# HKUST-Aerial-Robotics/MIND

Hardware: AMD Instinct MI355X
Metric: sim steps/sec (whole node) + scenario-tree nodes expanded/sec, AV2 demo scenes (higher is better)
Workload: dtype f32-class (bf16 hi+mid+lo split operands = 24 significand bits, six products, fp32 accumulate) pair kernel + ActorNet, f32 elsewhere in the predictor, f64 iLQR

## Files before the change

include/mind_hip.h:

```cpp
#ifndef MIND_HIP_H
#define MIND_HIP_H

#include <stddef.h>
#include <stdint.h>

#ifdef __cplusplus
extern "C" {
#endif

#define MIND_OK 0
#define MIND_EINVAL (-1)
#define MIND_ENOMEM (-2)
#define MIND_EHIP (-3)
#define MIND_ESTATE (-4)
#define MIND_ENOTFOUND (-5)

typedef struct mind_ctx mind_ctx;

int mind_ctx_create(int device, void *stream, mind_ctx **out);
int mind_ctx_destroy(mind_ctx *ctx);
const char *mind_last_error_string(mind_ctx *ctx);
int mind_ctx_synchronize(mind_ctx *ctx);

typedef struct {
  const char *name;
  const float *data;
  int64_t numel;
} mind_tensor_desc;

int mind_weights_load(mind_ctx *ctx, const mind_tensor_desc *tensors, int n_tensors);

typedef struct {
  int n_scenes;
  const int32_t *actor_off;
  const int32_t *lane_off;
  const float *actors;
  const float *lanes;
  const float *lane_feat;
  const float *actor_ctrs;
  const float *actor_vecs;
  const float *lane_ctrs;
  const float *lane_vecs;
  const float *const *rpe;
  const float *tgt_nodes;
  const float *tgt_rpe;
} mind_scene_batch;

typedef struct {
  float *cls;
  float *reg;
  float *vel;
  float *lane_feat;
  float *actor_emb;
  float *cls_emb;
} mind_pred_out;

int mind_predict_batch(mind_ctx *ctx, const mind_scene_batch *in, mind_pred_out *out);

int mind_last_fusion_stats(mind_ctx *ctx, int *n_launches, float *total_ms, double *pairs_processed);
int mind_last_actor_stats(mind_ctx *ctx, int *layerwise, int *n_launches, int *n_chunks, float *total_ms);
int mind_last_token_stats(mind_ctx *ctx, int *layerwise, int *n_launches, int *n_chunks, float *total_ms);
int mind_last_token_stage_ms(mind_ctx *ctx, float *out_ms, int cap);
int mind_last_ilqr_stats(mind_ctx *ctx, float *kernel_ms, int *n_trees, int *workgroups_per_tree);
int mind_last_ilqr_profile(mind_ctx *ctx, double *out9);
int mind_last_ilqr_trace(mind_ctx *ctx, int tree, int phase, double *out, int cap_rows, int *n_rows);
int mind_set_profiling(mind_ctx *ctx, int enable);

#define MIND_PAIR_F32 0
#define MIND_PAIR_BF16X3 1
#define MIND_PAIR_BF16 2
#define MIND_PAIR_BF16X6 3
int mind_set_pair_precision(mind_ctx *ctx, int mode);

int mind_set_tuning(mind_ctx *ctx, const char *name, int value);
int mind_get_pair_precision(mind_ctx *ctx);
int mind_debug_pack_bfrag(const float *w, int row_stride, uint32_t *out);

int mind_debug_pair_schedule(const int *scene_tokens, const int *scene_actors, int n_scenes, int n_cu, int last_layer, int *out_jobs, int cap,
                             int *out_info);

int mind_debug_predict_choice(const char *const *knob_names, const int *knob_values, int n_knobs, int pair_prec, int n_cu, int have_side,
                              const int *scene_actors, const int *scene_lanes, int n_scenes, long long *out, int cap);

int mind_debug_ilqr_plan(const char *const *knob_names, const int *knob_values, int n_knobs, int n_cu, int mode, int n_trees, const int *n_nodes,
                         const int32_t *parents, long long *out, int cap, int *bad);

int mind_debug_aime_book(int pred_len, int max_depth, int max_rounds, int n_agents, int world, int rank, int force, int n_rounds, const int *dec_len,
                         const float *dec, int n_tokens, int bytes_per_pair, int plan_chunk_mb, int per_scene, long long *out, int cap, char *msg,
                         int msg_cap);

int mind_debug_actor_lw_plan(int n_actors, int np, int chunk, long long *out_launches, int cap, long long *out_info);

int mind_debug_token_lw_plan(int n_tokens, int mode, int chunk, long long *out_launches, int cap, long long *out_info);

int mind_debug_pack_conv_frag(const float *w, int co, int ci, int ksz, uint32_t *out, size_t cap);

int mind_debug_trig(mind_ctx *ctx, const double *x, int n, double *out);

int mind_debug_set_layers(mind_ctx *ctx, int n);
int64_t mind_debug_read(mind_ctx *ctx, const char *name, float *host, int64_t max_floats);

typedef struct {
  int n_nodes;
  const int32_t *parent;
  const float *prob;
  int n_agents;
  const float *agent_mean;
  const float *agent_cov;
  const double *field;
  const double *node_w;
} mind_cost_tree;

typedef struct {
  double dt, wheelbase;
  double w_des_state[6];
  double w_state_con[6];
  double state_lower[6], state_upper[6];
  double w_ctrl[2];
  double w_tgt, w_ego, w_ego_cov_offset, w_exo, w_exo_cov_offset, w_exo_cost_offset;
  double grid_res; int grid_w, grid_h;
  int max_iter;
} mind_ilqr_cfg;

typedef struct { int iterations; int converged; double J; double mu; } mind_ilqr_stats;

int mind_ilqr_solve_trees(mind_ctx *ctx, const mind_ilqr_cfg *cfg, const mind_cost_tree *trees,
                          int n_trees, const double *x0, const double *target_lane, int n_lane_pts,
                          double target_vel, int use_exo, const double *us_init, double *xs,
                          double *us, mind_ilqr_stats *stats);

int mind_ilqr_contingency(mind_ctx *ctx, const mind_ilqr_cfg *cfg_warm, const mind_ilqr_cfg *cfg_full,
                          const mind_cost_tree *trees, int n_trees, const double *x0,
                          const double *target_lane, int n_lane_pts, double target_vel, double *xs,
                          double *us, mind_ilqr_stats *stats_warm, mind_ilqr_stats *stats_full);
int mind_ilqr_contingency_begin(mind_ctx *ctx, const mind_ilqr_cfg *cfg_warm, const mind_ilqr_cfg *cfg_full,
                                const mind_cost_tree *trees, int n_trees, const double *x0,
                                const double *target_lane, int n_lane_pts, double target_vel, double *xs,
                                double *us, mind_ilqr_stats *stats_warm, mind_ilqr_stats *stats_full);
int mind_ilqr_contingency_begin_plan(mind_ctx *ctx, const mind_ilqr_cfg *cfg_warm, const mind_ilqr_cfg *cfg_full, const double *x0,
                                     const double *target_lane, int n_lane_pts, double target_vel, double *xs, double *us,
                                     mind_ilqr_stats *stats_warm, mind_ilqr_stats *stats_full);
int mind_ilqr_finish(mind_ctx *ctx);

typedef struct {
  int n_scenes;
  const int32_t *actor_off;
  const float *reg, *vel;
  const float *actor_ctrs, *actor_vecs;
  const float *rot, *orig;
  const float *cov_last;
  const int32_t *last;
  const float *target_lane;
  int n_lane_pts;
  const float *cls;
  const float *scen_prob;
  int lane_check;
  float dist_thres;
} mind_world_in;

typedef struct {
  float *world;
  float *topo;
  float *ego_end;
  float *sel, *sel_prob;
} mind_world_out;

int mind_aime_world(mind_ctx *ctx, const mind_world_in *in, const mind_world_out *out);

typedef struct {
  int n_scenes, n_agents, n_lanes;
  const float *pos, *ang, *vel;
  const float *types;
  const float *pad;
  const float *lane_ctrs, *lane_vecs;
  const float *target_lane;
  const float *target_lane_info;
  int n_lane_pts;
  float time_ahead, min_vel;
  const float *rows_dev;
  const int32_t *parent_slot;
  const int32_t *row0;
  const int32_t *dur;
  int prev_gen;
} mind_rebase_in;

typedef struct {
  float *actors;
  float *actor_ctrs, *actor_vecs;
  float *lane_ctrs, *lane_vecs;
  float *tgt_nodes, *tgt_rpe;
  float *frames;
  int32_t *gen;
} mind_rebase_out;

int mind_aime_rebase(mind_ctx *ctx, const mind_rebase_in *in, const mind_rebase_out *out);

typedef struct {
  int n_agents, n_lanes, n_lane_pts;
  const float *actors;
  const float *actor_ctrs, *actor_vecs;
  const float *lanes;
  const float *lane_ctrs, *lane_vecs;
  const float *tgt_nodes, *tgt_rpe;
  const float *rot, *orig, *tgt_pts;
  const float *hist;
  const float *types;
  const float *target_lane;
  const float *target_lane_info;
  float time_ahead, min_vel, dist_thres;
  int max_depth;
  int max_rounds;
  int pred_len;
  const float *raw_pos, *raw_ang, *raw_vel;
  const float *raw_pad;
  const double *lane_pts;
  const int32_t *lane_flags;
  float travel0;
  const float *script_cls, *script_reg, *script_vel;
  float prob_floor;
  const mind_ilqr_cfg *solve_cfg_warm, *solve_cfg_full;
  const double *solve_x0, *solve_lane;
  int solve_n_lane_pts;
  double solve_target_vel;
} mind_aime_plan_in;

#define MIND_AIME_BRANCH 1
#define MIND_AIME_END 2
#define MIND_AIME_TERMINATE 4
typedef struct {
  int round, scene, mode;
  int parent;
  float prob;
  int cur_t, end_t;
  int flags;
  int dur;
  int64_t row_off;
  float tgt_pts[22];
} mind_aime_node;

typedef struct {
  const mind_aime_node *nodes;
  int n_nodes;
  const float *rows;
  int64_t n_row_floats;
  int n_expanded, n_rounds;
  int root_flags;
  int round_scenes[32];
  float pair_ms;
  int pair_launches;
  int n_trees;
// ... 145 lines not shown
```

mind_amd/_lib.py:

```python
import ctypes as C
import os

_HERE = os.path.dirname(os.path.abspath(__file__))
LIB_PATH = os.environ.get("MIND_HIP_LIB", os.path.join(_HERE, "libmind_hip.so"))

MIND_OK = 0
MIND_EINVAL, MIND_ENOMEM, MIND_EHIP, MIND_ESTATE, MIND_ENOTFOUND = -1, -2, -3, -4, -5


class TensorDesc(C.Structure):
    _fields_ = [("name", C.c_char_p), ("data", C.POINTER(C.c_float)), ("numel", C.c_int64)]


class SceneBatch(C.Structure):
    _fields_ = [("n_scenes", C.c_int), ("actor_off", C.POINTER(C.c_int32)), ("lane_off", C.POINTER(C.c_int32)),
                ("actors", C.c_void_p), ("lanes", C.c_void_p), ("lane_feat", C.c_void_p),
                ("actor_ctrs", C.c_void_p), ("actor_vecs", C.c_void_p), ("lane_ctrs", C.c_void_p),
                ("lane_vecs", C.c_void_p), ("rpe", C.POINTER(C.c_void_p)), ("tgt_nodes", C.c_void_p),
                ("tgt_rpe", C.c_void_p)]


class PredOut(C.Structure):
    _fields_ = [("cls", C.c_void_p), ("reg", C.c_void_p), ("vel", C.c_void_p), ("lane_feat", C.c_void_p),
                ("actor_emb", C.c_void_p), ("cls_emb", C.c_void_p)]


class CostTree(C.Structure):
    _fields_ = [("n_nodes", C.c_int), ("parent", C.POINTER(C.c_int32)), ("prob", C.POINTER(C.c_float)),
                ("n_agents", C.c_int), ("agent_mean", C.POINTER(C.c_float)), ("agent_cov", C.POINTER(C.c_float)),
                ("field", C.POINTER(C.c_double)), ("node_w", C.POINTER(C.c_double))]


class FieldGrid(C.Structure):
    _fields_ = [("W", C.c_int), ("H", C.c_int), ("res", C.c_double), ("off_x", C.c_double), ("off_y", C.c_double),
                ("gx", C.POINTER(C.c_double)), ("gy", C.POINTER(C.c_double))]


class WorldIn(C.Structure):
    _fields_ = [("n_scenes", C.c_int), ("actor_off", C.POINTER(C.c_int32)), ("reg", C.c_void_p), ("vel", C.c_void_p),
                ("actor_ctrs", C.c_void_p), ("actor_vecs", C.c_void_p), ("rot", C.POINTER(C.c_float)),
                ("orig", C.POINTER(C.c_float)), ("cov_last", C.POINTER(C.c_float)), ("last", C.POINTER(C.c_int32)),
                ("target_lane", C.POINTER(C.c_float)), ("n_lane_pts", C.c_int), ("cls", C.c_void_p),
                ("scen_prob", C.POINTER(C.c_float)), ("lane_check", C.c_int), ("dist_thres", C.c_float)]


class WorldOut(C.Structure):
    _fields_ = [("world", C.c_void_p), ("topo", C.c_void_p), ("ego_end", C.c_void_p), ("sel", C.c_void_p), ("sel_prob", C.c_void_p)]


class RebaseIn(C.Structure):
    _fields_ = [("n_scenes", C.c_int), ("n_agents", C.c_int), ("n_lanes", C.c_int), ("pos", C.POINTER(C.c_float)),
                ("ang", C.POINTER(C.c_float)), ("vel", C.POINTER(C.c_float)), ("types", C.POINTER(C.c_float)),
                ("pad", C.POINTER(C.c_float)), ("lane_ctrs", C.POINTER(C.c_float)), ("lane_vecs", C.POINTER(C.c_float)),
                ("target_lane", C.POINTER(C.c_float)), ("target_lane_info", C.POINTER(C.c_float)), ("n_lane_pts", C.c_int),
                ("time_ahead", C.c_float), ("min_vel", C.c_float), ("rows_dev", C.c_void_p), ("parent_slot", C.POINTER(C.c_int32)),
                ("row0", C.POINTER(C.c_int32)), ("dur", C.POINTER(C.c_int32)), ("prev_gen", C.c_int)]


class RebaseOut(C.Structure):
    _fields_ = [("actors", C.c_void_p), ("actor_ctrs", C.c_void_p), ("actor_vecs", C.c_void_p), ("lane_ctrs", C.c_void_p),
                ("lane_vecs", C.c_void_p), ("tgt_nodes", C.c_void_p), ("tgt_rpe", C.c_void_p), ("frames", C.c_void_p),
                ("gen", C.POINTER(C.c_int32))]


class AimePlanIn(C.Structure):
    _fields_ = [("n_agents", C.c_int), ("n_lanes", C.c_int), ("n_lane_pts", C.c_int)] + \
               [(k, C.POINTER(C.c_float)) for k in ("actors", "actor_ctrs", "actor_vecs", "lanes", "lane_ctrs", "lane_vecs", "tgt_nodes", "tgt_rpe",
                                                    "rot", "orig", "tgt_pts", "hist", "types", "target_lane", "target_lane_info")] + \
               [("time_ahead", C.c_float), ("min_vel", C.c_float), ("dist_thres", C.c_float), ("max_depth", C.c_int), ("max_rounds", C.c_int), ("pred_len", C.c_int),
                ("raw_pos", C.POINTER(C.c_float)), ("raw_ang", C.POINTER(C.c_float)), ("raw_vel", C.POINTER(C.c_float)), ("raw_pad", C.POINTER(C.c_float)),
                ("lane_pts", C.POINTER(C.c_double)), ("lane_flags", C.POINTER(C.c_int32)), ("travel0", C.c_float),
                ("script_cls", C.c_void_p), ("script_reg", C.c_void_p), ("script_vel", C.c_void_p), ("prob_floor", C.c_float),
                ("solve_cfg_warm", C.c_void_p), ("solve_cfg_full", C.c_void_p), ("solve_x0", C.c_void_p), ("solve_lane", C.c_void_p),
                ("solve_n_lane_pts", C.c_int), ("solve_target_vel", C.c_double)]


class AimeNode(C.Structure):
    _fields_ = [("round", C.c_int), ("scene", C.c_int), ("mode", C.c_int), ("parent", C.c_int), ("prob", C.c_float),
                ("cur_t", C.c_int), ("end_t", C.c_int), ("flags", C.c_int), ("dur", C.c_int), ("row_off", C.c_int64),
                ("tgt_pts", C.c_float * 22)]


class AimePlanOut(C.Structure):
    _fields_ = [("nodes", C.POINTER(AimeNode)), ("n_nodes", C.c_int), ("rows", C.POINTER(C.c_float)), ("n_row_floats", C.c_int64),
                ("n_expanded", C.c_int), ("n_rounds", C.c_int), ("root_flags", C.c_int), ("round_scenes", C.c_int * 32),
                ("pair_ms", C.c_float), ("pair_launches", C.c_int), ("n_trees", C.c_int), ("tree_top", C.POINTER(C.c_int32)),
                ("tree_off", C.POINTER(C.c_int32)), ("flat_parent", C.POINTER(C.c_int32)), ("flat_prob", C.POINTER(C.c_float)),
                ("flat_mean", C.POINTER(C.c_float)), ("flat_cov", C.POINTER(C.c_float)), ("solves_begun", C.c_int)]


class IlqrCfg(C.Structure):
    _fields_ = [("dt", C.c_double), ("wheelbase", C.c_double), ("w_des_state", C.c_double * 6),
                ("w_state_con", C.c_double * 6), ("state_lower", C.c_double * 6), ("state_upper", C.c_double * 6),
                ("w_ctrl", C.c_double * 2), ("w_tgt", C.c_double), ("w_ego", C.c_double),
                ("w_ego_cov_offset", C.c_double), ("w_exo", C.c_double), ("w_exo_cov_offset", C.c_double),
                ("w_exo_cost_offset", C.c_double), ("grid_res", C.c_double), ("grid_w", C.c_int), ("grid_h", C.c_int),
                ("max_iter", C.c_int)]


class IlqrStats(C.Structure):
    _fields_ = [("iterations", C.c_int), ("converged", C.c_int), ("J", C.c_double), ("mu", C.c_double)]


LOOP_TAN_FN = C.CFUNCTYPE(C.c_double, C.c_double)
LOOP_SINCOS_FN = C.CFUNCTYPE(None, C.c_double, C.POINTER(C.c_double))


class LoopDesc(C.Structure):
    _fields_ = [("n_tracks", C.c_int), ("n_steps", C.c_int), ("clamp_last", C.c_int), ("ego_state", C.c_void_p), ("ego_state_is_f32", C.c_int), ("ego_obs", C.c_void_p), ("ego_trig32", C.c_void_p),
                ("tan_fn", C.c_void_p), ("sincos_fn", C.c_void_p), ("exo_obs", C.c_void_p),
                ("exo_valid", C.c_void_p), ("timestep", C.c_void_p), ("type_slot", C.c_void_p),
                ("sim_step", C.c_double), ("plan_step", C.c_double), ("enable_time", C.c_double),
                ("wheelbase", C.c_double), ("max_speed", C.c_double), ("max_steer", C.c_double), ("max_acc", C.c_double), ("max_dec", C.c_double),
                ("n_lanes", C.c_int), ("lane_pts", C.c_void_p), ("lane_flags", C.c_void_p),
                ("n_lane_pts", C.c_int), ("target_lane", C.c_void_p), ("target_lane_info", C.c_void_p),
                ("time_ahead", C.c_double), ("min_vel", C.c_float), ("dist_thres", C.c_float), ("max_depth", C.c_int), ("max_rounds", C.c_int),
                ("pred_len", C.c_int), ("prob_floor", C.c_float),
                ("cfg_warm", C.c_void_p), ("cfg_full", C.c_void_p), ("solve_n_lane_pts", C.c_int), ("solve_lane", C.c_void_p), ("target_vel", C.c_double),
                ("eval_n_lane_pts", C.c_int), ("eval_lane_is_f32", C.c_int), ("eval_lane", C.c_void_p), ("speculative", C.c_int)]


class LoopTotals(C.Structure):
    _fields_ = [("plans", C.c_longlong), ("expansions", C.c_longlong), ("scen_trees", C.c_longlong), ("rounds", C.c_longlong),
                ("aime_s", C.c_double), ("ilqr_s", C.c_double), ("total_s", C.c_double),
                ("iterations", C.c_longlong), ("node_iterations", C.c_longlong), ("node_iterations_exo", C.c_longlong),
                ("warm_speculated", C.c_longlong), ("warm_hits", C.c_longlong),
                ("pair_ms", C.c_double), ("pair_launches", C.c_longlong), ("scene_n2", C.c_double), ("scene_n_a1", C.c_double),
                ("ilqr_ms", C.c_double), ("ilqr_launches", C.c_longlong), ("ilqr_trees", C.c_longlong), ("ilqr_workgroups_per_tree", C.c_int),
                ("ilqr_prof", C.c_double * 9), ("ilqr_node_steps", C.c_double)]


class LoopOut(C.Structure):
    _fields_ = [("planned", C.c_int), ("enabled", C.c_int), ("n_steps", C.c_longlong), ("n_plans", C.c_longlong), ("episode_steps", C.c_longlong),
                ("sim_time", C.c_double), ("last_trigger", C.c_double), ("state", C.c_double * 4), ("ctrl", C.c_double * 2),
                ("n_agents", C.c_int), ("n_trees", C.c_int), ("best", C.c_int), ("n_expanded", C.c_int), ("n_rounds", C.c_int), ("n_traj_nodes", C.c_int),
                ("costs", C.POINTER(C.c_double)), ("aime_s", C.c_double), ("ilqr_s", C.c_double), ("total_s", C.c_double),
                ("tot", LoopTotals)]


PLANNER_EGO_KEY = -(1 << 63)


class PlannerDesc(C.Structure):
    _fields_ = [("time_ahead", C.c_double), ("min_vel", C.c_float), ("dist_thres", C.c_float), ("max_depth", C.c_int), ("max_rounds", C.c_int),
                ("pred_len", C.c_int), ("prob_floor", C.c_float), ("cfg_warm", C.c_void_p), ("cfg_full", C.c_void_p), ("speculative", C.c_int),
                ("ego_type_slot", C.c_int)]


class PlannerOut(C.Structure):
    _fields_ = [("n_plans", C.c_longlong),
                ("n_agents", C.c_int), ("n_trees", C.c_int), ("best", C.c_int), ("n_expanded", C.c_int), ("n_rounds", C.c_int), ("n_traj_nodes", C.c_int),
                ("costs", C.POINTER(C.c_double)), ("ctrl", C.c_double * 2), ("aime_s", C.c_double), ("ilqr_s", C.c_double), ("total_s", C.c_double),
                ("tot", LoopTotals)]


EXPORTS = ["mind_ctx_create", "mind_ctx_destroy", "mind_last_error_string", "mind_ctx_synchronize",
           "mind_weights_load", "mind_predict_batch", "mind_last_fusion_stats", "mind_last_actor_stats", "mind_debug_actor_lw_plan", "mind_last_token_stats", "mind_last_token_stage_ms", "mind_debug_token_lw_plan", "mind_set_profiling",
           "mind_ilqr_solve_trees", "mind_ilqr_contingency", "mind_ilqr_solve_fields", "mind_cost_eval", "mind_lane_dist_field", "mind_aime_world", "mind_aime_rebase", "mind_debug_set_layers",
           "mind_debug_read", "mind_set_pair_precision", "mind_get_pair_precision", "mind_debug_pack_bfrag", "mind_debug_pack_conv_frag", "mind_debug_pair_schedule", "mind_debug_predict_choice", "mind_debug_ilqr_plan", "mind_debug_aime_book", "mind_set_tuning", "mind_last_ilqr_stats", "mind_aime_plan", "mind_last_ilqr_profile", "mind_eval_traj_trees", "mind_last_ilqr_trace", "mind_ilqr_contingency_begin", "mind_ilqr_finish", "mind_fill_tracks", "mind_ilqr_contingency_begin_plan", "mind_debug_trig", "mind_aime_plan_begin", "mind_aime_plan_poll", "mind_aime_plan_finish", "mind_ctx_busy", "mind_ilqr_finish_plan",
           "mind_set_exchange", "mind_last_exchange_stats",
           "mind_loop_create", "mind_loop_destroy", "mind_loop_reset", "mind_loop_advance", "mind_loop_state", "mind_loop_last_plan", "mind_loop_export",
           "mind_planner_create", "mind_planner_destroy", "mind_planner_reset", "mind_planner_observe", "mind_planner_set_lanes", "mind_planner_set_target_lane",
           "mind_planner_set_solve_lane", "mind_planner_set_eval_lane", "mind_planner_plan", "mind_planner_last_plan", "mind_planner_export"]

EXCHANGE_FN = C.CFUNCTYPE(C.c_int, C.c_void_p, C.c_int, C.c_void_p, C.c_void_p, C.c_int64)
XCHG_ALLGATHER, XCHG_ALLREDUCE, XCHG_ALLTOALLV = 0, 1, 2

_lib = None


def load():
    global _lib
    if _lib is not None:
        return _lib
    if not os.path.exists(LIB_PATH):
        raise ImportError(f"{LIB_PATH} is missing: the HIP extension must be built (hipcc --offload-arch=gfx950); "
                          "there is no CPU fallback for the product path")
    lib = C.CDLL(LIB_PATH)
    lib.mind_ctx_create.argtypes = [C.c_int, C.c_void_p, C.POINTER(C.c_void_p)]
    lib.mind_ctx_destroy.argtypes = [C.c_void_p]
    lib.mind_last_error_string.argtypes = [C.c_void_p]
    lib.mind_last_error_string.restype = C.c_char_p
    lib.mind_ctx_synchronize.argtypes = [C.c_void_p]
    lib.mind_weights_load.argtypes = [C.c_void_p, C.POINTER(TensorDesc), C.c_int]
    lib.mind_predict_batch.argtypes = [C.c_void_p, C.POINTER(SceneBatch), C.POINTER(PredOut)]
    lib.mind_last_fusion_stats.argtypes = [C.c_void_p, C.POINTER(C.c_int), C.POINTER(C.c_float), C.POINTER(C.c_double)]
    lib.mind_last_actor_stats.argtypes = [C.c_void_p, C.POINTER(C.c_int), C.POINTER(C.c_int), C.POINTER(C.c_int), C.POINTER(C.c_float)]
    lib.mind_debug_actor_lw_plan.argtypes = [C.c_int, C.c_int, C.c_int, C.POINTER(C.c_longlong), C.c_int, C.POINTER(C.c_longlong)]
    lib.mind_last_token_stats.argtypes = [C.c_void_p, C.POINTER(C.c_int), C.POINTER(C.c_int), C.POINTER(C.c_int), C.POINTER(C.c_float)]
    lib.mind_last_token_stage_ms.argtypes = [C.c_void_p, C.POINTER(C.c_float), C.c_int]
    lib.mind_debug_token_lw_plan.argtypes = [C.c_int, C.c_int, C.c_int, C.POINTER(C.c_longlong), C.c_int, C.POINTER(C.c_longlong)]
    lib.mind_set_profiling.argtypes = [C.c_void_p, C.c_int]
    lib.mind_ilqr_solve_trees.argtypes = [C.c_void_p, C.POINTER(IlqrCfg), C.POINTER(CostTree), C.c_int,
                                          C.POINTER(C.c_double), C.POINTER(C.c_double), C.c_int, C.c_double, C.c_int,
                                          C.POINTER(C.c_double), C.POINTER(C.c_double), C.POINTER(C.c_double),
                                          C.POINTER(IlqrStats)]
    lib.mind_ilqr_contingency.argtypes = [C.c_void_p, C.POINTER(IlqrCfg), C.POINTER(IlqrCfg), C.POINTER(CostTree), C.c_int,
                                          C.POINTER(C.c_double), C.POINTER(C.c_double), C.c_int, C.c_double,
                                          C.POINTER(C.c_double), C.POINTER(C.c_double), C.POINTER(IlqrStats), C.POINTER(IlqrStats)]
    lib.mind_ilqr_contingency_begin.argtypes = [C.c_void_p, C.POINTER(IlqrCfg), C.POINTER(IlqrCfg), C.POINTER(CostTree), C.c_int,
                                          C.POINTER(C.c_double), C.POINTER(C.c_double), C.c_int, C.c_double,
                                          C.POINTER(C.c_double), C.POINTER(C.c_double), C.POINTER(IlqrStats), C.POINTER(IlqrStats)]
    lib.mind_ilqr_finish.argtypes = [C.c_void_p]
    lib.mind_ilqr_contingency_begin_plan.argtypes = [C.c_void_p, C.POINTER(IlqrCfg), C.POINTER(IlqrCfg), C.c_void_p, C.c_void_p, C.c_int, C.c_double,
                                                     C.c_void_p, C.c_void_p, C.c_void_p, C.c_void_p]
    lib.mind_fill_tracks.argtypes = [C.c_void_p, C.c_int, C.c_int, C.c_void_p, C.c_void_p, C.c_void_p, C.c_void_p, C.c_void_p, C.c_void_p]
    lib.mind_ilqr_solve_fields.argtypes = [C.c_void_p, C.POINTER(IlqrCfg), C.POINTER(FieldGrid), C.POINTER(CostTree), C.c_int,
                                           C.POINTER(C.c_double), C.POINTER(C.c_double), C.POINTER(C.c_double),
                                           C.POINTER(C.c_double), C.POINTER(IlqrStats)]
    lib.mind_cost_eval.argtypes = [C.c_void_p, C.POINTER(IlqrCfg), C.POINTER(FieldGrid), C.POINTER(CostTree),
                                   C.POINTER(C.c_double), C.POINTER(C.c_double), C.c_int, C.c_double, C.c_int, C.c_int,
                                   C.POINTER(C.c_int32), C.POINTER(C.c_double), C.POINTER(C.c_double), C.POINTER(C.c_double)]
    lib.mind_lane_dist_field.argtypes = [C.c_void_p, C.POINTER(C.c_double), C.POINTER(C.c_double), C.c_int, C.c_int, C.c_int,
                                         C.c_double] + [C.POINTER(C.c_double)] * 4
    lib.mind_aime_world.argtypes = [C.c_void_p, C.POINTER(WorldIn), C.POINTER(WorldOut)]
    lib.mind_aime_rebase.argtypes = [C.c_void_p, C.POINTER(RebaseIn), C.POINTER(RebaseOut)]
    lib.mind_aime_plan.argtypes = [C.c_void_p, C.POINTER(AimePlanIn), C.POINTER(AimePlanOut)]
    lib.mind_aime_plan_begin.argtypes = [C.c_void_p, C.POINTER(AimePlanIn)]
    lib.mind_aime_plan_poll.argtypes = [C.c_void_p]
    lib.mind_aime_plan_finish.argtypes = [C.c_void_p, C.POINTER(AimePlanOut)]
    lib.mind_ctx_busy.argtypes = [C.c_void_p]
    lib.mind_ilqr_finish_plan.argtypes = [C.c_void_p, C.c_int, C.c_int, C.c_void_p, C.c_void_p, C.c_void_p, C.c_void_p]
    lib.mind_set_pair_precision.argtypes = [C.c_void_p, C.c_int]
    lib.mind_set_tuning.argtypes = [C.c_void_p, C.c_char_p, C.c_int]
    lib.mind_last_ilqr_stats.argtypes = [C.c_void_p, C.POINTER(C.c_float), C.POINTER(C.c_int), C.POINTER(C.c_int)]
    lib.mind_last_ilqr_profile.argtypes = [C.c_void_p, C.POINTER(C.c_double)]
    lib.mind_last_ilqr_trace.argtypes = [C.c_void_p, C.c_int, C.c_int, C.POINTER(C.c_double), C.c_int, C.POINTER(C.c_int)]
    lib.mind_eval_traj_trees.argtypes = [C.POINTER(C.c_double), C.POINTER(C.c_double), C.POINTER(C.c_int32), C.c_int, C.c_void_p, C.c_int, C.c_int,
                                         C.c_double, C.POINTER(C.c_double)]
    lib.mind_get_pair_precision.argtypes = [C.c_void_p]
    lib.mind_debug_pack_bfrag.argtypes = [C.POINTER(C.c_float), C.c_int, C.POINTER(C.c_uint32)]
    lib.mind_debug_pair_schedule.argtypes = [C.POINTER(C.c_int), C.POINTER(C.c_int), C.c_int, C.c_int, C.c_int, C.POINTER(C.c_int), C.c_int, C.POINTER(C.c_int)]
    lib.mind_debug_predict_choice.argtypes = [C.POINTER(C.c_char_p), C.POINTER(C.c_int), C.c_int, C.c_int, C.c_int, C.c_int, C.POINTER(C.c_int), C.POINTER(C.c_int),
                                              C.c_int, C.POINTER(C.c_longlong), C.c_int]
    lib.mind_debug_ilqr_plan.argtypes = [C.POINTER(C.c_char_p), C.POINTER(C.c_int), C.c_int, C.c_int, C.c_int, C.c_int, C.POINTER(C.c_int), C.POINTER(C.c_int32),
                                         C.POINTER(C.c_longlong), C.c_int, C.POINTER(C.c_int)]
    lib.mind_debug_aime_book.argtypes = [C.c_int] * 8 + [C.POINTER(C.c_int), C.POINTER(C.c_float)] + [C.c_int] * 4 + [C.POINTER(C.c_longlong), C.c_int, C.c_char_p, C.c_int]
    lib.mind_debug_trig.argtypes = [C.c_void_p, C.POINTER(C.c_double), C.c_int, C.POINTER(C.c_double)]
    lib.mind_debug_pack_conv_frag.argtypes = [C.POINTER(C.c_float), C.c_int, C.c_int, C.c_int, C.POINTER(C.c_uint32), C.c_size_t]
    lib.mind_debug_set_layers.argtypes = [C.c_void_p, C.c_int]
    lib.mind_debug_read.argtypes = [C.c_void_p, C.c_char_p, C.POINTER(C.c_float), C.c_int64]
    lib.mind_set_exchange.argtypes = [C.c_void_p, C.c_int, C.c_int, EXCHANGE_FN, C.c_void_p, C.c_int]
    lib.mind_last_exchange_stats.argtypes = [C.c_void_p, C.POINTER(C.c_longlong), C.POINTER(C.c_longlong)]
    lib.mind_loop_create.argtypes = [C.c_void_p, C.POINTER(LoopDesc), C.POINTER(C.c_void_p)]
    lib.mind_loop_destroy.argtypes = [C.c_void_p]
    lib.mind_loop_reset.argtypes = [C.c_void_p]
    lib.mind_loop_advance.argtypes = [C.c_void_p, C.c_int, C.c_double, C.c_longlong, C.POINTER(LoopOut)]
    lib.mind_loop_state.argtypes = [C.c_void_p, C.POINTER(LoopOut)]
    lib.mind_loop_last_plan.argtypes = [C.c_void_p, C.POINTER(AimePlanOut)] + [C.POINTER(C.c_void_p)] * 6 + [C.c_void_p]
    lib.mind_loop_export.argtypes = [C.c_void_p, C.c_int, C.POINTER(C.c_int), C.c_void_p, C.c_void_p, C.c_void_p]
    lib.mind_planner_create.argtypes = [C.c_void_p, C.POINTER(PlannerDesc), C.POINTER(C.c_void_p)]
    lib.mind_planner_destroy.argtypes = [C.c_void_p]
    lib.mind_planner_reset.argtypes = [C.c_void_p]
    lib.mind_planner_observe.argtypes = [C.c_void_p, C.c_int, C.c_void_p, C.c_int, C.c_void_p, C.c_void_p, C.c_void_p]
    lib.mind_planner_set_lanes.argtypes = [C.c_void_p, C.c_int, C.c_void_p, C.c_void_p]
    lib.mind_planner_set_target_lane.argtypes = [C.c_void_p, C.c_int, C.c_void_p, C.c_void_p]
    lib.mind_planner_set_solve_lane.argtypes = [C.c_void_p, C.c_int, C.c_void_p, C.c_double]
    lib.mind_planner_set_eval_lane.argtypes = [C.c_void_p, C.c_int, C.c_void_p, C.c_int]
    lib.mind_planner_plan.argtypes = [C.c_void_p, C.c_void_p, C.c_void_p, C.POINTER(PlannerOut)]
    lib.mind_planner_last_plan.argtypes = [C.c_void_p, C.POINTER(AimePlanOut)] + [C.POINTER(C.c_void_p)] * 6 + [C.c_void_p]
    lib.mind_planner_export.argtypes = [C.c_void_p, C.c_int, C.POINTER(C.c_int), C.c_void_p, C.c_void_p, C.c_void_p]
    for n in EXPORTS:
        getattr(lib, n)
        if n not in ("mind_last_error_string", "mind_debug_read"):
            getattr(lib, n).restype = C.c_int
    lib.mind_debug_read.restype = C.c_int64
    _lib = lib
    return lib


PRED_CHOICE_FIELDS = ("header", "n_runs", "np", "actor_form", "actor_arg", "actor_grid", "actor_chunk", "actor_chunks", "actor_launches", "qsplit", "qk_stride",
                      "tiled", "edge_bf16", "edge_pair_bytes", "tok_chunk", "tok_lw", "tok_chunks", "pair_family", "pair_np", "l5_jobs5", "xcd_lanes",
                      "xcd_lanes5", "dec_actor", "dec_np", "fp32_dec", "split_dec", "want_mw", "mw_blocks", "cls_on_side", "tgt_wait_first")
PAIR_PREC = ("f32", "bf16x3", "bf16", "bf16x6")


def predict_choice(knobs, prec, scenes, n_cu=256, have_side=True):
    lib = load()
    names = (C.c_char_p * max(1, len(knobs)))(*[k.encode() for k in knobs])
    vals = (C.c_int * max(1, len(knobs)))(*[int(v) for v in knobs.values()])
    sa = (C.c_int * len(scenes))(*[a for a, _ in scenes])
    sl = (C.c_int * len(scenes))(*[l for _, l in scenes])
    cap = 32 + 6 * len(scenes)
    out = (C.c_longlong * cap)()
    n = lib.mind_debug_predict_choice(names, vals, len(knobs), PAIR_PREC.index(prec) if isinstance(prec, str) else prec, n_cu, int(have_side),
                                      sa, sl, len(scenes), out, cap)
    if n == MIND_EINVAL:
        return None
    assert 0 < n <= cap and out[0] == 32 and n == 32 + 6 * out[1], n
    d = dict(zip(PRED_CHOICE_FIELDS, out[:30]))
    d["runs"] = [tuple(out[32 + 6 * i:38 + 6 * i]) for i in range(out[1])]
    return d


ILQR_PLAN_FIELDS = ("header", "n_trees", "form", "G", "GS", "spec", "nslot", "grid", "workgroups_per_tree", "host_out", "early", "starve_followers")
ILQR_TREE_FIELDS = ("M", "nl", "nseg", "nsl", "maxls", "nfs")
ILQR_TREE_TABLES = ("level_start", "level_nodes", "child_start", "child_list", "seg_start", "seg_nodes", "slevel_start", "slevel_segs", "seg_rec",
                    "fstep_start", "fstep_items", "fstep_q1", "fstep_nstart", "fstep_nodes")


def ilqr_plan(knobs, parents, n_cu=256, generic=False, evaluate=False, two_fits=False):
    lib = load()
    names = (C.c_char_p * max(1, len(knobs)))(*[k.encode() for k in knobs])
    vals = (C.c_int * max(1, len(knobs)))(*[int(v) for v in knobs.values()])
    nn = (C.c_int * len(parents))(*[len(p) for p in parents])
    flat = [int(v) for p in parents for v in p]
    par = (C.c_int32 * max(1, len(flat)))(*flat)
    bad = (C.c_int * 2)()
    mode = int(generic) | int(evaluate) << 1 | int(two_fits) << 2
    n = lib.mind_debug_ilqr_plan(names, vals, len(knobs), n_cu, mode, len(parents), nn, par, None, 0, bad)
    if n == MIND_EINVAL:
        return {"bad": (bad[0], bad[1])} if bad[0] >= 0 else None
    out = (C.c_longlong * n)()
    assert lib.mind_debug_ilqr_plan(names, vals, len(knobs), n_cu, mode, len(parents), nn, par, out, n, bad) == n and out[0] == 16
    d = dict(zip(ILQR_PLAN_FIELDS, out[:12]))
    d["trees"], o = [], 16
    for _ in parents:
        tr = dict(zip(ILQR_TREE_FIELDS, out[o:o + 6]))
        lens, o = out[o + 6:o + 20], o + 20
        for name, ln in zip(ILQR_TREE_TABLES, lens):
            tr[name], o = list(out[o:o + ln]), o + ln
        d["trees"].append(tr)
    assert o == n
    return d


AIME_ROUND_FIELDS = ("B", "lo", "hi", "Bmax", "chunk", "S", "s0", "Sm", "any")
AIME_NODE_FIELDS = ("round", "scene", "mode", "parent", "prob", "cur_t", "end_t", "flags", "dur", "row_off", "owner", "lscene")


def aime_book(pred_len, max_depth, n_agents, rounds, world=1, rank=0, force=False, max_rounds=32, n_tokens=0, bytes_per_pair=512, plan_chunk_mb=96 * 1024,
              per_scene=1):
    import numpy as np
    lib = load()
    arrs = [np.ascontiguousarray(r, np.float32).ravel() for r in rounds]
    lens = (C.c_int * max(1, len(arrs)))(*[a.size for a in arrs])
    dec = np.concatenate(arrs + [np.zeros(1, np.float32)])
    msg = C.create_string_buffer(256)
    args = [pred_len, max_depth, max_rounds, n_agents, world, rank, int(force), len(arrs), lens, dec.ctypes.data_as(C.POINTER(C.c_float)), n_tokens,
            bytes_per_pair, plan_chunk_mb, per_scene]
    n = lib.mind_debug_aime_book(*args, None, 0, msg, 256)
    if n == MIND_EINVAL:
        return None
    out = (C.c_longlong * n)()
    assert lib.mind_debug_aime_book(*args, out, n, msg, 256) == n and out[0] == 16
    o, take = [16], lambda k: (list(out[o[0]:o[0] + k]), o.__setitem__(0, o[0] + k))[0]
    d = dict(code=out[1], error=msg.value.decode() if out[1] else None, args=(out[2], out[3]), n_rows=out[8], root_flags=out[9], rounds=[])
    for _ in range(out[4]):
        r = dict(zip(AIME_ROUND_FIELDS, take(9)))
        for k, ln in (("todo", r["S"]), ("cnt_r", world), ("s0_r", world + 1), ("win", 3 * r["Sm"]), ("tab", 2 * world), ("snd", 2 * world), ("rcv", 2 * world)):
            r[k] = take(ln)
        d["rounds"].append(r)
    if not out[1]:
        d["nodes"] = [dict(zip(AIME_NODE_FIELDS, take(12))) for _ in range(out[5])]
        for name in ("gather", "flat"):
            nj, nb, nbytes = take(3)
            d[name] = dict(jobs=[tuple(take(5)) for _ in range(nj)], job_of_block=take(nb), agent_of_block=take(nb), bytes=nbytes)
        d["tree_top"], d["tree_off"], d["flat_parent"], d["flat_prob"] = take(out[6]), take(out[6] + 1), take(out[7]), take(out[7])
    assert o[0] == n
    return d


class MindError(RuntimeError):
    pass


def check(lib, ctx, rc, what):
    if rc != MIND_OK:
        msg = lib.mind_last_error_string(ctx) if ctx else b""
        raise MindError(f"{what} failed with code {rc}: {msg.decode() if msg else ''}")
```

mind_amd/csrc/encdec_kernels.hip:

```cpp
#include <hip/hip_runtime.h>
#include <stdint.h>

typedef float f32x4 __attribute__((ext_vector_type(4)));

#define NT 256

__device__ __forceinline__ float wave_sum(float v) {
  v += __shfl_xor(v, 32, 64);
  v += __shfl_xor(v, 16, 64);
  v += __shfl_xor(v, 8, 64);
  v += __shfl_xor(v, 4, 64);
  v += __shfl_xor(v, 2, 64);
  v += __shfl_xor(v, 1, 64);
  return v;
}

__device__ __forceinline__ float block_sum(float v, float *red) {
  v = wave_sum(v);
  __syncthreads();
  if ((threadIdx.x & 63) == 0) red[threadIdx.x >> 6] = v;
  __syncthreads();
  return red[0] + red[1] + red[2] + red[3];
}

#ifndef DB
#define DB 16
#endif
#define DENSE_ROW_FENCE() __builtin_amdgcn_sched_barrier(0)
#define DBQ 8
template <int R>
__device__ __forceinline__ void dense_quads(const float *in, int ldi, int K, const float *__restrict__ WT,
                                            const float *__restrict__ b, int NOUT, float *out, int ldo,
                                            float *part, int part_floats) {
  const int nthr = blockDim.x;
  const int NQ = NOUT >> 2;
  int KP = 1;
  while (KP * 2 * NQ <= nthr && KP * 2 * R * NOUT <= part_floats && KP * 2 <= (K >> 2)) KP *= 2;
  const int Kc = ((K / 4 + KP - 1) / KP) * 4;
  for (int item = threadIdx.x; item < KP * NQ; item += nthr) {
    const int kp = item / NQ, o = (item % NQ) * 4;
    float acc[R][4];
#pragma unroll
    for (int r = 0; r < R; ++r)
#pragma unroll
      for (int c = 0; c < 4; ++c) acc[r][c] = (KP == 1 && b) ? b[o + c] : 0.f;
    const int k0 = kp * Kc, k1 = min(K, k0 + Kc);
    int k = k0;
    for (; k + DBQ <= k1; k += DBQ) {
      f32x4 w[DBQ];
#pragma unroll
      for (int q = 0; q < DBQ; ++q) w[q] = *(const f32x4 *)(WT + (size_t)(k + q) * NOUT + o);
#pragma unroll
      for (int r = 0; r < R; ++r) {
#pragma unroll
        for (int q4 = 0; q4 < DBQ / 4; ++q4) {
          const f32x4 x = *(const f32x4 *)(in + r * ldi + k + 4 * q4);
#pragma unroll
          for (int j = 0; j < 4; ++j)
#pragma unroll
            for (int c = 0; c < 4; ++c) acc[r][c] = fmaf(w[4 * q4 + j][c], x[j], acc[r][c]);
        }
        DENSE_ROW_FENCE();
      }
    }
    for (; k < k1; k += 4) {
#pragma unroll
      for (int j = 0; j < 4; ++j) {
        const f32x4 w = *(const f32x4 *)(WT + (size_t)(k + j) * NOUT + o);
#pragma unroll
        for (int r = 0; r < R; ++r) {
          const float x = in[r * ldi + k + j];
#pragma unroll
          for (int c = 0; c < 4; ++c) acc[r][c] = fmaf(w[c], x, acc[r][c]);
        }
      }
    }
#pragma unroll
    for (int r = 0; r < R; ++r)
#pragma unroll
      for (int c = 0; c < 4; ++c) {
        if (KP == 1) out[r * ldo + o + c] = acc[r][c];
        else part[(kp * R + r) * NOUT + o + c] = acc[r][c];
      }
  }
  if (KP == 1) return;
  __syncthreads();
  for (int i = threadIdx.x; i < R * NOUT; i += nthr) {
    const int r = i / NOUT, oo = i % NOUT;
    float v = b ? b[oo] : 0.f;
    for (int q = 0; q < KP; ++q) v += part[(q * R + r) * NOUT + oo];
    out[r * ldo + oo] = v;
  }
}

#ifndef DT
#define DT 1024
#endif
template <int R>
__device__ __forceinline__ void dense_quads_part(const float *in, int ldi, int K, const float *__restrict__ WT, const float *__restrict__ b, int NOUT,
                                                 float *out, int ldo, float *part, int part_floats, int wg, int G) {
  const int nthr = blockDim.x;
  const int NQ = NOUT >> 2;
  int KP = 1;
  while (KP * 2 * NQ <= DT && KP * 2 * R * NOUT <= part_floats && KP * 2 <= (K >> 2)) KP *= 2;
  const int Kc = ((K / 4 + KP - 1) / KP) * 4;
  const int q_lo = NQ * wg / G, q_hi = NQ * (wg + 1) / G, NQg = q_hi - q_lo;
  for (int item = threadIdx.x; item < KP * NQg; item += nthr) {
    const int kp = item / NQg, o = (q_lo + item % NQg) * 4;
    float acc[R][4];
#pragma unroll
    for (int r = 0; r < R; ++r)
#pragma unroll
      for (int c = 0; c < 4; ++c) acc[r][c] = (KP == 1 && b) ? b[o + c] : 0.f;
    const int k0 = kp * Kc, k1 = min(K, k0 + Kc);
    int k = k0;
    for (; k + DBQ <= k1; k += DBQ) {
      f32x4 w[DBQ];
#pragma unroll
      for (int q = 0; q < DBQ; ++q) w[q] = *(const f32x4 *)(WT + (size_t)(k + q) * NOUT + o);
#pragma unroll
      for (int r = 0; r < R; ++r) {
#pragma unroll
        for (int q4 = 0; q4 < DBQ / 4; ++q4) {
          const f32x4 x = *(const f32x4 *)(in + r * ldi + k + 4 * q4);
#pragma unroll
          for (int j = 0; j < 4; ++j)
#pragma unroll
            for (int c = 0; c < 4; ++c) acc[r][c] = fmaf(w[4 * q4 + j][c], x[j], acc[r][c]);
        }
        DENSE_ROW_FENCE();
      }
    }
    for (; k < k1; k += 4) {
#pragma unroll
      for (int j = 0; j < 4; ++j) {
        const f32x4 w = *(const f32x4 *)(WT + (size_t)(k + j) * NOUT + o);
#pragma unroll
        for (int r = 0; r < R; ++r) {
          const float x = in[r * ldi + k + j];
#pragma unroll
          for (int c = 0; c < 4; ++c) acc[r][c] = fmaf(w[c], x, acc[r][c]);
        }
      }
    }
#pragma unroll
    for (int r = 0; r < R; ++r)
#pragma unroll
      for (int c = 0; c < 4; ++c) {
        if (KP == 1) out[r * ldo + o + c] = acc[r][c];
        else part[(kp * R + r) * NOUT + o + c] = acc[r][c];
      }
  }
  if (KP == 1) return;
  __syncthreads();
  const int o_lo = q_lo * 4, no = NQg * 4;
  for (int i = threadIdx.x; i < R * no; i += nthr) {
    const int r = i / no, oo = o_lo + i % no;
    float v = b ? b[oo] : 0.f;
    for (int q = 0; q < KP; ++q) v += part[(q * R + r) * NOUT + oo];
    out[r * ldo + oo] = v;
  }
}

#define DEC_SYNC_SPINS (1u << 22)
__device__ __forceinline__ bool dec_grid_sync(unsigned *bar, int G, unsigned *abort_word) {
  __shared__ int sh_ab;
  __syncthreads();
  if (threadIdx.x == 0) {
// ... 558 lines not shown
  const int PF = DEC_SCENE_PART;
  const int tid = threadIdx.x;
  int xstage = 0;
  float *xb0 = xbuf, *xb1 = xbuf + 6 * 1536;
#ifdef MIND_DEC_TRACE
  if (blockIdx.x == 0 && tid == 0) dec_trn_ = 0;
#endif
  DEC_MARK();
  if (PART == 2) {
    for (int i = tid; i < 768; i += blockDim.x) C[i / 128][i % 128] = Cout[(size_t)b * 768 + i];
    __syncthreads();
  }
  if (PART != 2) {
  if (tid < 128) v0[0][tid] = x[(size_t)cls_row[b] * 128 + tid];
  __syncthreads();
  dense<1>(&v0[0][0], 256, 128, W.c0W, W.c0b, 384, &v1[0][0], 768, part, PF);
  DEC_MARK();
  __syncthreads();
  ln_rows(&v1[0][0], 768, 1, 384, W.c0g, W.c0be, true);
  DEC_MARK();
  __syncthreads();
  if (MW) {
    dense_quads_part<1>(&v1[0][0], 768, 384, W.c3W, W.c3b, 768, &ff[0][0], 1536, part, PF, wg, G);
    if (dec_exchange<1>(&ff[0][0], 1536, 768, wg, G, (xstage++ & 1) ? xb1 : xb0, bar, abort_word)) return;
  } else
    dense<1>(&v1[0][0], 768, 384, W.c3W, W.c3b, 768, &ff[0][0], 1536, part, PF);
  DEC_MARK();
  __syncthreads();
  ln_rows(&ff[0][0], 1536, 1, 768, W.c3g, W.c3be, true);
  DEC_MARK();
  __syncthreads();
  for (int i = tid; i < 768; i += blockDim.x) C[i / 128][i % 128] = ff[0][i];
  __syncthreads();
  for (int L = 0; L < 2; ++L) {
    dense<6>(&C[0][0], 128, 128, W.inW[L], W.inb[L], 384, &qkv[0][0], 384, part, PF);
  DEC_MARK();
    __syncthreads();
    if (tid < 4 * 36) {
      const int hd = tid / 36, s = (tid % 36) / 6, t = tid % 6;
      float d = 0.f;
      for (int k = 0; k < 32; ++k) d = fmaf(qkv[s][hd * 32 + k], qkv[t][128 + hd * 32 + k], d);
      sc[hd][s][t] = d / sqrtf(32.0f);
    }
    __syncthreads();
    if (tid < 24) {
      const int hd = tid / 6, s = tid % 6;
      float m = -INFINITY;
      for (int t = 0; t < 6; ++t) m = fmaxf(m, sc[hd][s][t]);
      float e[6], sum = 0.f;
      for (int t = 0; t < 6; ++t) { e[t] = expf(sc[hd][s][t] - m); sum += e[t]; }
      for (int t = 0; t < 6; ++t) sc[hd][s][t] = e[t] / sum;
    }
    __syncthreads();
    for (int i = tid; i < 6 * 128; i += blockDim.x) {
      const int s = i / 128, c = i % 128, hd = c / 32;
      float o = 0.f;
      for (int t = 0; t < 6; ++t) o = fmaf(sc[hd][s][t], qkv[t][256 + c], o);
      att[s][c] = o;
    }
    __syncthreads();
    dense<6>(&att[0][0], 128, 128, W.outW[L], W.outb[L], 128, &t2[0][0], 128, part, PF);
  DEC_MARK();
    __syncthreads();
    for (int i = tid; i < 768; i += blockDim.x) C[i / 128][i % 128] += t2[i / 128][i % 128];
    __syncthreads();
    ln_rows(&C[0][0], 128, 6, 128, W.n1g[L], W.n1b[L], false);
  DEC_MARK();
    __syncthreads();
    if (MW) {
      dense_quads_part<6>(&C[0][0], 128, 128, W.l1W[L], W.l1b[L], 1536, &ff[0][0], 1536, part, PF, wg, G);
      if (dec_exchange<6>(&ff[0][0], 1536, 1536, wg, G, (xstage++ & 1) ? xb1 : xb0, bar, abort_word)) return;
    } else
      dense<6>(&C[0][0], 128, 128, W.l1W[L], W.l1b[L], 1536, &ff[0][0], 1536, part, PF);
  DEC_MARK();
    __syncthreads();
    for (int i = tid; i < 6 * 1536; i += blockDim.x) ff[i / 1536][i % 1536] = fmaxf(ff[i / 1536][i % 1536], 0.f);
    __syncthreads();
    if (MW) {
      dense_quads_part<6>(&ff[0][0], 1536, 1536, W.l2W[L], W.l2b[L], 128, &t2[0][0], 128, part, PF, wg, G);
      if (dec_exchange<6>(&t2[0][0], 128, 128, wg, G, (xstage++ & 1) ? xb1 : xb0, bar, abort_word)) return;
    } else
      dense<6>(&ff[0][0], 1536, 1536, W.l2W[L], W.l2b[L], 128, &t2[0][0], 128, part, PF);
  DEC_MARK();
    __syncthreads();
    for (int i = tid; i < 768; i += blockDim.x) C[i / 128][i % 128] += t2[i / 128][i % 128];
    __syncthreads();
    ln_rows(&C[0][0], 128, 6, 128, W.n2g[L], W.n2b[L], false);
  DEC_MARK();
    __syncthreads();
  }
  if (!MW || wg == 0)
    for (int i = tid; i < 768; i += blockDim.x) Cout[(size_t)b * 768 + i] = C[i / 128][i % 128];
  }
  if (PART == 1) return;
  dense<6>(&C[0][0], 128, 128, W.k0W, W.k0b, 128, &att[0][0], 128, part, PF);
  DEC_MARK();
  __syncthreads();
  ln_rows(&att[0][0], 128, 6, 128, W.k0g, W.k0be, true);
  DEC_MARK();
  __syncthreads();
  dense<6>(&att[0][0], 128, 128, W.k3W, W.k3b, 128, &t2[0][0], 128, part, PF);
  DEC_MARK();
  __syncthreads();
  ln_rows(&t2[0][0], 128, 6, 128, W.k3g, W.k3be, true);
  DEC_MARK();
  __syncthreads();
  for (int k = tid >> 6; k < 6; k += (int)(blockDim.x >> 6)) {
    const int lane = tid & 63;
    float s = t2[k][lane] * W.k6W[lane] + t2[k][lane + 64] * W.k6W[lane + 64];
    s = wave_sum(s);
    if (lane == 0) sc[0][0][k] = s + W.k6b[0];
  }
  __syncthreads();
  if (tid == 0 && (!MW || wg == 0)) {
    float m = -INFINITY;
    for (int k = 0; k < 6; ++k) m = fmaxf(m, sc[0][0][k]);
    float e[6], sum = 0.f;
    for (int k = 0; k < 6; ++k) { e[k] = expf(sc[0][0][k] - m); sum += e[k]; }
    for (int k = 0; k < 6; ++k) cls_out[(size_t)b * 6 + k] = e[k] / sum;
  }
  DEC_MARK();
#ifdef MIND_DEC_TRACE
  if (blockIdx.x == 0 && tid == 0) {
    printf("[k_dec_scene] cycles between marks (dense / LayerNorm stages in program order):");
    for (int q = 1; q < dec_trn_ && q < 64; ++q) printf(" %lld", dec_tr_[q] - dec_tr_[q - 1]);
    printf("\n");
  }
#endif
}

__global__ __launch_bounds__(DT) void k_dec_scene(const float *__restrict__ x, const int *__restrict__ cls_row, float *__restrict__ Cout,
                                                  float *__restrict__ cls_out, DecW W) {
  k_dec_scene_body<false>(x, cls_row, Cout, cls_out, W, (int)blockIdx.x, 0, 1, nullptr, nullptr, nullptr);
}
__global__ __launch_bounds__(DT) void k_dec_scene_c(const float *__restrict__ x, const int *__restrict__ cls_row, float *__restrict__ Cout, DecW W) {
  k_dec_scene_body<false, 1>(x, cls_row, Cout, nullptr, W, (int)blockIdx.x, 0, 1, nullptr, nullptr, nullptr);
}
__global__ __launch_bounds__(DT) void k_dec_cls(float *__restrict__ Cout, float *__restrict__ cls_out, DecW W) {
  k_dec_scene_body<false, 2>(nullptr, nullptr, Cout, cls_out, W, (int)blockIdx.x, 0, 1, nullptr, nullptr, nullptr);
}
#define DEC_MW_G 8
__global__ __launch_bounds__(DT) void k_dec_scene_mw(const float *__restrict__ x, const int *__restrict__ cls_row, float *__restrict__ Cout,
                                                     float *__restrict__ cls_out, DecW W, int n_scenes, float *__restrict__ xbuf,
                                                     unsigned *__restrict__ bars, unsigned *abort_word) {
  const int r = (int)blockIdx.x % (8 * DEC_MW_G);
  const int b = 8 * ((int)blockIdx.x / (8 * DEC_MW_G)) + (r & 7), wg = r >> 3;
  if (b >= n_scenes) return;
  k_dec_scene_body<true>(x, cls_row, Cout, cls_out, W, b, wg, DEC_MW_G, xbuf + (size_t)b * 2 * 6 * 1536, bars + 4 * (size_t)b, abort_word);
}

#define RA 4
#define DEC_ACTOR_LDS_FLOATS (512 + 1536 + 3072 + 3072 + 3072 + 960 + 6144)
template <int PART>
__global__ __launch_bounds__(DT) void k_dec_actor(const float *__restrict__ x ,
                                                  const int *__restrict__ actor_row ,
                                                  const int *__restrict__ actor_scene , int n_actors,
                                                  const float *__restrict__ Cmode ,
                                                  const float *__restrict__ tgt ,
                                                  float *__restrict__ reg, float *__restrict__ vel, DecW W, float *__restrict__ h2g) {
  extern __shared__ __attribute__((aligned(16))) float dsm[];
  float (*xin)[128] = (float (*)[128])(dsm);
  float (*h1)[384] = (float (*)[384])(dsm + 512);
  float (*h2)[768] = (float (*)[768])(dsm + 2048);
  float (*E)[128] = (float (*)[128])(dsm + 5120);
  float (*t1)[128] = (float (*)[128])(dsm + 8192);
  float (*prm)[40] = (float (*)[40])(dsm + 11264);
  float *part = dsm + 12224;
  const int PF = 6144;
  const int tid = threadIdx.x;
  const int a0 = blockIdx.x * RA;
  if (PART != 2) {
    for (int i = tid; i < RA * 128; i += blockDim.x) {
      const int r = i / 128, a = a0 + r;
      xin[r][i % 128] = a < n_actors ? x[(size_t)actor_row[a] * 128 + i % 128] : 0.f;
    }
    __syncthreads();
    dense<RA>(&xin[0][0], 128, 128, W.a0W, W.a0b, 384, &h1[0][0], 384, part, PF);
    __syncthreads();
    ln_rows(&h1[0][0], 384, RA, 384, W.a0g, W.a0be, true);
    __syncthreads();
    dense<RA>(&h1[0][0], 384, 384, W.a3W, W.a3b, 768, &h2[0][0], 768, part, PF);
    __syncthreads();
    ln_rows(&h2[0][0], 768, RA, 768, W.a3g, W.a3be, true);
    __syncthreads();
    if (PART == 1) {
      for (int i = tid; i < RA * 768; i += blockDim.x) {
        const int r = i / 768, a = a0 + r;
        if (a < n_actors) h2g[(size_t)a * 768 + i % 768] = h2[r][i % 768];
      }
      return;
    }
  } else {
    for (int i = tid; i < RA * 768; i += blockDim.x) {
      const int r = i / 768, a = a0 + r;
      h2[r][i % 768] = a < n_actors ? h2g[(size_t)a * 768 + i % 768] : 0.f;
    }
    __syncthreads();
  }
  for (int i = tid; i < RA * 768; i += blockDim.x) {
    const int r = i / 768, k = (i % 768) / 128, c = i % 128;
    const int a = a0 + r;
    float v = 0.f;
    if (a < n_actors) {
      const int sc = actor_scene[a];
      v = h2[r][k * 128 + c] + Cmode[((size_t)sc * 6 + k) * 128 + c];
      if (k == 0) v += tgt[(size_t)sc * 128 + c];
    }
    E[r * 6 + k][c] = v;
  }
  __syncthreads();
  dense<RA * 6>(&E[0][0], 128, 128, W.r0W, W.r0b, 128, &t1[0][0], 128, part, PF);
  __syncthreads();
  ln_rows(&t1[0][0], 128, RA * 6, 128, W.r0g, W.r0be, true);
  __syncthreads();
  dense<RA * 6>(&t1[0][0], 128, 128, W.r3W, W.r3b, 128, &E[0][0], 128, part, PF);
  __syncthreads();
  ln_rows(&E[0][0], 128, RA * 6, 128, W.r3g, W.r3be, true);
  __syncthreads();
  for (int i = tid; i < RA * 6 * 40; i += blockDim.x) {
    const int r = i / 40, o = i % 40;
    float acc = W.r6b[o];
    for (int k = 0; k < 128; ++k) acc = fmaf(W.r6W[k * 40 + o], E[r][k], acc);
    prm[r][o] = acc;
  }
  __syncthreads();
  for (int i = tid; i < RA * 6 * 60; i += blockDim.x) {
    const int r = i / 60, t = i % 60;
    const int a = a0 + r / 6, k = r % 6;
    if (a >= n_actors) continue;
    float o5[5] = {0.f, 0.f, 0.f, 0.f, 0.f};
    for (int c = 0; c < 8; ++c) {
      const float tv = W.T[t * 8 + c];
#pragma unroll
      for (int d = 0; d < 5; ++d) o5[d] = fmaf(tv, prm[r][c * 5 + d], o5[d]);
    }
    float v2[2] = {0.f, 0.f};
    for (int c = 0; c < 7; ++c) {
      const float tv = W.Tp[t * 7 + c];
      v2[0] = fmaf(tv, prm[r][(c + 1) * 5 + 0] - prm[r][c * 5 + 0], v2[0]);
      v2[1] = fmaf(tv, prm[r][(c + 1) * 5 + 1] - prm[r][c * 5 + 1], v2[1]);
    }
    float *ro = reg + (((size_t)a * 6 + k) * 60 + t) * 5;
    ro[0] = o5[0]; ro[1] = o5[1]; ro[2] = expf(o5[2]); ro[3] = expf(o5[3]); ro[4] = expf(o5[4]);
    float *vo = vel + (((size_t)a * 6 + k) * 60 + t) * 2;
    vo[0] = v2[0] / 6.0f; vo[1] = v2[1] / 6.0f;
  }
}

extern "C" size_t mind_dec_scene_lds_bytes() { return (size_t)DEC_SCENE_LDS_FLOATS * sizeof(float); }
extern "C" size_t mind_dec_actor_lds_bytes() { return (size_t)DEC_ACTOR_LDS_FLOATS * sizeof(float); }
```

mind_amd/csrc/fusion_kernels.hip:

```cpp
#include <hip/hip_runtime.h>
#include <stdint.h>

typedef float f32x4 __attribute__((ext_vector_type(4)));
typedef float f32x16 __attribute__((ext_vector_type(16)));

typedef unsigned int u32;
typedef u32 u32x4 __attribute__((ext_vector_type(4)));
typedef __bf16 bf16x8 __attribute__((ext_vector_type(8)));
typedef __bf16 bf16x2_t __attribute__((ext_vector_type(2)));
typedef float f32x2_t __attribute__((ext_vector_type(2)));

__device__ __forceinline__ u32 pk_bf16(float a, float b) {
  f32x2_t v = {a, b};
  return __builtin_bit_cast(u32, __builtin_convertvector(v, bf16x2_t));
}
__device__ __forceinline__ float bf_lo_f32(u32 pk) { return __builtin_bit_cast(float, pk << 16); }
__device__ __forceinline__ float bf_hi_f32(u32 pk) { return __builtin_bit_cast(float, pk & 0xffff0000u); }

#define D_ 128
#define PART_STRIDE 1040

struct PairJob {
  long long edge_base;
  int N;
  int j;
  int t0, t1;
  int tok_base;
  int slot;
  int flags;
  int scene;
  long long edge_base_t;
};

#define VT_GM 0
#define VT_BM 128
#define VT_BP 256
#define VT_GP 384
#define VT_BEP 512
#define VT_GE 640
#define VT_BE 768
#define VT_SIZE 896

#define PAIR_WAVES 8
#define PAIR_THREADS (PAIR_WAVES * 64)
#define STAGE_FLOATS 512
#define LDS_WAE 0
#define LDS_WAP 16384
#define LDS_STAGE 32768
#define LDS_PTAB (LDS_STAGE + PAIR_WAVES * STAGE_FLOATS)
#define LDS_SVEC (LDS_PTAB + PAIR_WAVES * 128)
#define LDS_VT (LDS_SVEC + PAIR_WAVES * 136)
#define LDS_RT (LDS_VT + VT_SIZE)
#define LDS_TOTAL (LDS_RT + 1024)

#define LDS_FENCE() asm volatile("s_waitcnt lgkmcnt(0)" ::: "memory")
#define SCHED_FENCE() __builtin_amdgcn_sched_barrier(0)
#define OPAQUE(x) asm volatile("" : "+v"(x))

typedef f32x4 frag8[8];

__device__ __forceinline__ float red_quad(float v) {
  v += __shfl_xor(v, 16, 64);
  v += __shfl_xor(v, 32, 64);
  return v;
}
__device__ __forceinline__ float red_max16(float v) {
  v = fmaxf(v, __shfl_xor(v, 8, 64));
  v = fmaxf(v, __shfl_xor(v, 4, 64));
  v = fmaxf(v, __shfl_xor(v, 2, 64));
  v = fmaxf(v, __shfl_xor(v, 1, 64));
  return v;
}
__device__ __forceinline__ float red_sum16(float v) {
  v += __shfl_xor(v, 8, 64);
  v += __shfl_xor(v, 4, 64);
  v += __shfl_xor(v, 2, 64);
  v += __shfl_xor(v, 1, 64);
  return v;
}

__device__ __forceinline__ void ln_pairs(frag8 &a, const float *vtq, int off_g, int off_b, bool relu) {
  float s = 0.f;
#pragma unroll
  for (int b = 0; b < 8; ++b)
#pragma unroll
    for (int w = 0; w < 4; ++w) s += a[b][w];
  s = red_quad(s);
  const float mean = s * (1.0f / 128.0f);
  float v = 0.f;
#pragma unroll
  for (int b = 0; b < 8; ++b)
#pragma unroll
    for (int w = 0; w < 4; ++w) {
      const float d = a[b][w] - mean;
      v = fmaf(d, d, v);
    }
  v = red_quad(v);
  const float rstd = 1.0f / sqrtf(v * (1.0f / 128.0f) + 1e-5f);
#pragma unroll
  for (int b = 0; b < 8; ++b) {
    const f32x4 gm = *(const f32x4 *)(vtq + off_g + 16 * b);
    const f32x4 bt = *(const f32x4 *)(vtq + off_b + 16 * b);
#pragma unroll
    for (int w = 0; w < 4; ++w) {
      float y = (a[b][w] - mean) * rstd * gm[w] + bt[w];
      if (relu) y = fmaxf(y, 0.f);
      a[b][w] = y;
    }
    if (b & 1) SCHED_FENCE();
  }
}

__device__ __forceinline__ void gemm128(frag8 &acc, const float *wa, const frag8 &bsrc, int lane) {
  int lo = lane * 4;
  OPAQUE(lo);
  const float *wl = wa + lo;
  f32x4 c0 = *(const f32x4 *)(wl + (0 * 8 + 0) * 256);
  f32x4 c1 = *(const f32x4 *)(wl + (1 * 8 + 0) * 256);
#pragma unroll
  for (int st = 0; st < 32; ++st) {
    const int s4 = st >> 2, ob = (st & 3) * 2;
    f32x4 n0 = c0, n1 = c1;
    if (st < 31) {
      const int s4n = (st + 1) >> 2, obn = ((st + 1) & 3) * 2;
      n0 = *(const f32x4 *)(wl + (obn * 8 + s4n) * 256);
      n1 = *(const f32x4 *)(wl + ((obn + 1) * 8 + s4n) * 256);
    }
#pragma unroll
    for (int w = 0; w < 4; ++w) {
      const float bv = bsrc[s4][w];
      acc[ob] = __builtin_amdgcn_mfma_f32_16x16x4f32(c0[w], bv, acc[ob], 0, 0, 0);
      acc[ob + 1] = __builtin_amdgcn_mfma_f32_16x16x4f32(c1[w], bv, acc[ob + 1], 0, 0, 0);
    }
    c0 = n0; c1 = n1;
    SCHED_FENCE();
  }
}

__device__ __forceinline__ int sw_pos(int r, int c) { return (r * 8 + (c ^ ((r >> 1) & 7))) * 4; }

#ifdef MIND_PAIR_TRACE
#define PT_DECL long long pt_[12] = {0, 0, 0, 0, 0, 0, 0, 0, 0, 0, 0, 0}; long long pt_t = clock64();
#define PT_DRAIN() asm volatile("s_waitcnt vmcnt(0)" ::: "memory")
#define PT(i) do { long long n_ = clock64(); pt_[i] += n_ - pt_t; pt_t = n_; } while (0)
#else
#define PT_DECL
#define PT_DRAIN()
#define PT(i)
#endif

template <int MODE>
__global__ __launch_bounds__(PAIR_THREADS, 1) void k_pair(const PairJob *__restrict__ jobs, int n_jobs,
                                                 float *__restrict__ edge, const float *__restrict__ ST,
                                                 const float *__restrict__ QK, float *__restrict__ part,
// ... 262 lines not shown
        LDS_FENCE();
        const bool mine = (ll >> 5) == (qt & 1);
        const int fq = ll & 31;
#pragma unroll
        for (int t = 0; t < 16; ++t) {
          float val = stage[sw_pos(t, fq >> 2) + (fq & 3)];
          val = mine ? val : 0.f;
          const f32x4 pa = *(const f32x4 *)(ptab + t * 8);
          const f32x4 pb = *(const f32x4 *)(ptab + t * 8 + 4);
#pragma unroll
          for (int k = 0; k < 4; ++k) {
            mbar[hf][k] = fmaf(pa[k], val, mbar[hf][k]);
            mbar[hf][k + 4] = fmaf(pb[k], val, mbar[hf][k + 4]);
          }
          if ((t & 3) == 3) SCHED_FENCE();
        }
        LDS_FENCE();
      }

      PT(7);
    }

    float *po = part + (size_t)J.slot * PART_STRIDE;
#pragma unroll
    for (int r = 0; r < 4; ++r) {
      const float l = red_sum16(l_part[r]);
      if (p == 0 && q < 2) { po[4 * q + r] = m_run[r]; po[8 + 4 * q + r] = l; }
    }
#pragma unroll
    for (int hf = 0; hf < 2; ++hf)
#pragma unroll
      for (int hd = 0; hd < 8; ++hd) po[16 + hd * 128 + hf * 64 + lane] = mbar[hf][hd];
  }
#ifdef MIND_PAIR_TRACE
  if (blockIdx.x == 0 && tid == 0)
    printf("[k_pair<%d> um=%d] cycles: load %lld gemm1 %lld T+LN1 %lld scores %lld softmax %lld mbar %lld gemm2 %lld LN23+store %lld\n", MODE,
           update_mode, pt_[0], pt_[1], pt_[2], pt_[3], pt_[4], pt_[5], pt_[6], pt_[7]);
#endif
}

template __global__ void k_pair<0>(const PairJob *, int, float *, const float *, const float *, float *,
                                   const float *, const float *, const float *, const float *,
                                   const float *, const float *const *, int);
template __global__ void k_pair<1>(const PairJob *, int, float *, const float *, const float *, float *,
                                   const float *, const float *, const float *, const float *,
                                   const float *, const float *const *, int);

extern "C" size_t mind_pair_lds_bytes() { return (size_t)LDS_TOTAL * sizeof(float); }

#define TOK_TPW_BIG 8
#define TOK_TPW_SMALL 4

struct TokMeta {
  int type;
  int src;
  int slot0;
  int nsplit;
  int flags;
  int pad0, pad1, pad2;
};

struct TokWeights {
  const float *WvT, *bv, *WoT, *bo, *g2, *b2, *W1T, *b1, *W2T, *bb2, *g3, *b3;
  const float *WsT, *WtT, *bm, *WqT, *bq, *Wk;
  const float *WpaT, *bpa, *gpa, *bepa, *WplT, *bpl, *gpl, *bepl;
};

#define TKG 4
#define TT_THREADS (TKG * 128)

template <int K, int TP>
__device__ __forceinline__ void matvec_part(float (&acc)[TP], const float *__restrict__ WT, int ldo, int col,
                                            const float *xin, int ldx, int kg) {
  constexpr int KQ = K / TKG;
  const int k0 = kg * KQ;
  float w[KQ];
#pragma unroll
  for (int k = 0; k < KQ; ++k) w[k] = WT[(size_t)(k0 + k) * ldo + col];
#pragma unroll
  for (int t = 0; t < TP; ++t) acc[t] = 0.f;
#pragma unroll
  for (int k = 0; k < KQ; k += 4)
#pragma unroll
    for (int t = 0; t < TP; ++t) {
      const float4 xv = *reinterpret_cast<const float4 *>(xin + t * ldx + k0 + k);
      acc[t] = fmaf(w[k], xv.x, acc[t]);
      acc[t] = fmaf(w[k + 1], xv.y, acc[t]);
      acc[t] = fmaf(w[k + 2], xv.z, acc[t]);
      acc[t] = fmaf(w[k + 3], xv.w, acc[t]);
    }
}

template <int K>
__device__ __forceinline__ void mv_load(float (&w)[K / TKG], const float *__restrict__ WT, int ldo, int col, int kg) {
  constexpr int KQ = K / TKG;
  const int k0 = kg * KQ;
#pragma unroll
  for (int k = 0; k < KQ; ++k) w[k] = WT[(size_t)(k0 + k) * ldo + col];
}
template <int K, int TP>
__device__ __forceinline__ void mv_fma(float (&acc)[TP], const float (&w)[K / TKG], const float *xin, int ldx, int kg) {
  constexpr int KQ = K / TKG;
  const int k0 = kg * KQ;
#pragma unroll
  for (int t = 0; t < TP; ++t) acc[t] = 0.f;
#pragma unroll
  for (int k = 0; k < KQ; k += 4)
#pragma unroll
    for (int t = 0; t < TP; ++t) {
      const float4 xv = *reinterpret_cast<const float4 *>(xin + t * ldx + k0 + k);
      acc[t] = fmaf(w[k], xv.x, acc[t]);
      acc[t] = fmaf(w[k + 1], xv.y, acc[t]);
      acc[t] = fmaf(w[k + 2], xv.z, acc[t]);
      acc[t] = fmaf(w[k + 3], xv.w, acc[t]);
    }
}
template <int TP, int N>
__device__ __forceinline__ void ksum_n(const float (&acc)[N][TP], const float (&bias)[N], float *rk, int kg, int col, float (&r0)[N], float (&r1)[N]) {
  constexpr int TPW = TP, ST = TKG * TP * 128;
  __syncthreads();
#pragma unroll
  for (int n = 0; n < N; ++n)
#pragma unroll
    for (int t = 0; t < TPW; ++t) rk[n * ST + (kg * TPW + t) * 128 + col] = acc[n][t];
  __syncthreads();
  const int t0 = (TP / TKG) * kg;
#pragma unroll
  for (int n = 0; n < N; ++n) {
    const float *q = rk + n * ST;
    r0[n] = ((q[(0 * TPW + t0) * 128 + col] + q[(1 * TPW + t0) * 128 + col]) + (q[(2 * TPW + t0) * 128 + col] + q[(3 * TPW + t0) * 128 + col])) + bias[n];
    r1[n] = 0.f;
    if (TP / TKG == 2)
      r1[n] = ((q[(0 * TPW + t0 + 1) * 128 + col] + q[(1 * TPW + t0 + 1) * 128 + col]) + (q[(2 * TPW + t0 + 1) * 128 + col] + q[(3 * TPW + t0 + 1) * 128 + col])) + bias[n];
  }
}

template <int TP>
__device__ __forceinline__ void ksum(const float (&acc)[TP], float bias, float *rk, int kg, int col, float &r0, float &r1) {
  constexpr int TPW = TP;
  __syncthreads();
#pragma unroll
  for (int t = 0; t < TPW; ++t) rk[(kg * TPW + t) * 128 + col] = acc[t];
  __syncthreads();
  const int t0 = (TP / TKG) * kg;
  r0 = ((rk[(0 * TPW + t0) * 128 + col] + rk[(1 * TPW + t0) * 128 + col]) +
        (rk[(2 * TPW + t0) * 128 + col] + rk[(3 * TPW + t0) * 128 + col])) + bias;
  r1 = 0.f;
  if (TP / TKG == 2)
    r1 = ((rk[(0 * TPW + t0 + 1) * 128 + col] + rk[(1 * TPW + t0 + 1) * 128 + col]) +
          (rk[(2 * TPW + t0 + 1) * 128 + col] + rk[(3 * TPW + t0 + 1) * 128 + col])) + bias;
}

__device__ __forceinline__ void gsum2(float &a, float &b, float *rd, int kg, int tid) {
#pragma unroll
  for (int o = 32; o > 0; o >>= 1) { a += __shfl_xor(a, o, 64); b += __shfl_xor(b, o, 64); }
  const int wv = (tid >> 6) & 1;
  __syncthreads();
  if ((tid & 63) == 0) { rd[(kg * 2 + wv) * 2] = a; rd[(kg * 2 + wv) * 2 + 1] = b; }
  __syncthreads();
  a = rd[(kg * 2) * 2] + rd[(kg * 2 + 1) * 2];
  b = rd[(kg * 2) * 2 + 1] + rd[(kg * 2 + 1) * 2 + 1];
}

__device__ __forceinline__ void ln2tok(float &p0, float &p1, float g, float be, float *rd, int kg, int tid) {
  float s0 = p0, s1 = p1;
  gsum2(s0, s1, rd, kg, tid);
  const float d0 = p0 - s0 * (1.0f / 128.0f), d1 = p1 - s1 * (1.0f / 128.0f);
  s0 = d0 * d0; s1 = d1 * d1;
  gsum2(s0, s1, rd, kg, tid);
  p0 = d0 * (1.0f / sqrtf(s0 * (1.0f / 128.0f) + 1e-5f)) * g + be;
  p1 = d1 * (1.0f / sqrtf(s1 * (1.0f / 128.0f) + 1e-5f)) * g + be;
}

template <int TPW, bool MG>
__device__ __forceinline__ void k_token_body(const TokMeta *__restrict__ meta, int n_tok, int mode,
                                             const float *__restrict__ actor_feat,
                                             const float *__restrict__ lane_feat, float *__restrict__ x,
                                             const float *__restrict__ part, float *__restrict__ ST,
                                             float *__restrict__ QK, const TokWeights &W) {
  __shared__ __attribute__((aligned(16))) float xs[TPW][132];
  __shared__ __attribute__((aligned(16))) float tmp[TPW][260];
  __shared__ __attribute__((aligned(16))) float mb[TPW][8][132];
  __shared__ float rk[(MG ? 3 : 1) * TKG * TPW * 128];
  __shared__ float rd[TKG * 2 * 2];
  __shared__ float cw[TPW][8][8];
  const int tid = threadIdx.x, kg = tid >> 7, col = tid & 127;
  const int tok0 = blockIdx.x * TPW;
  const int nt = min(TPW, n_tok - tok0);
  constexpr bool TWO = TPW / TKG == 2;
  const int ta = (TPW / TKG) * kg, tb = TWO ? ta + 1 : ta;
  const bool va = ta < nt, vb = TWO && tb < nt;
#ifdef MIND_TOKEN_TRACE
  long long tt_[10] = {0, 0, 0, 0, 0, 0, 0, 0, 0, 0}, tq_ = clock64();
#define TT(i) do { const long long n_ = clock64(); tt_[i] += n_ - tq_; tq_ = n_; } while (0)
#else
#define TT(i) do {} while (0)
#endif

  if (mode & 1) {
    int tya = 2, tyb = 2;
    float fa = 0.f, fb = 0.f;
    if (va) {
      const TokMeta m = meta[tok0 + ta];
      tya = m.type;
      if (m.type == 0) fa = actor_feat[(size_t)m.src * 128 + col];
      else if (m.type == 1) fa = lane_feat[(size_t)m.src * 128 + col];
    }
    if (vb) {
      const TokMeta m = meta[tok0 + tb];
      tyb = m.type;
      if (m.type == 0) fb = actor_feat[(size_t)m.src * 128 + col];
      else if (m.type == 1) fb = lane_feat[(size_t)m.src * 128 + col];
    }
    tmp[ta][col] = fa; if (TWO) tmp[tb][col] = fb;
    __syncthreads();
    float acc[TPW], a0, a1, l0, l1;
    matvec_part<128, TPW>(acc, W.WpaT, 128, col, &tmp[0][0], 260, kg);
    ksum<TPW>(acc, W.bpa[col], rk, kg, col, a0, a1);
    matvec_part<128, TPW>(acc, W.WplT, 128, col, &tmp[0][0], 260, kg);
    ksum<TPW>(acc, W.bpl[col], rk, kg, col, l0, l1);
    float p0 = tya == 0 ? a0 : l0, p1 = tyb == 0 ? a1 : l1;
    {
      float s0 = p0, s1 = p1;
      gsum2(s0, s1, rd, kg, tid);
      const float d0 = p0 - s0 * (1.0f / 128.0f), d1 = p1 - s1 * (1.0f / 128.0f);
      s0 = d0 * d0; s1 = d1 * d1;
      gsum2(s0, s1, rd, kg, tid);
      const float ga = W.gpa[col], gl = W.gpl[col], ba = W.bepa[col], bl = W.bepl[col];
      p0 = fmaxf(d0 * (1.0f / sqrtf(s0 * (1.0f / 128.0f) + 1e-5f)) * (tya == 0 ? ga : gl) + (tya == 0 ? ba : bl), 0.f);
      p1 = fmaxf(d1 * (1.0f / sqrtf(s1 * (1.0f / 128.0f) + 1e-5f)) * (tyb == 0 ? ga : gl) + (tyb == 0 ? ba : bl), 0.f);
      if (tya == 2) p0 = 0.f;
      if (tyb == 2) p1 = 0.f;
    }
    xs[ta][col] = p0; if (TWO) xs[tb][col] = p1;
    __syncthreads();
  } else {
    xs[ta][col] = va ? x[(size_t)(tok0 + ta) * 128 + col] : 0.f;
    if (TWO) xs[tb][col] = vb ? x[(size_t)(tok0 + tb) * 128 + col] : 0.f;
    __syncthreads();
  }
  TT(0);
  if (mode & 2) {
    if (tid < TPW * 8) {
      const int t = tid >> 3, hd = tid & 7;
      float wgt[8];
#pragma unroll
      for (int s = 0; s < 8; ++s) wgt[s] = 0.f;
      if (t < nt) {
        const TokMeta m = meta[tok0 + t];
        if (!((mode & 8) && !(m.flags & 1))) {
          float M = -INFINITY;
          for (int s = 0; s < m.nsplit; ++s) M = fmaxf(M, part[(size_t)(m.slot0 + s) * PART_STRIDE + hd]);
          float L = 0.f;
          for (int s = 0; s < m.nsplit; ++s) {
            const float *ps = part + (size_t)(m.slot0 + s) * PART_STRIDE;
            const float e = expf(ps[hd] - M);
            wgt[s] = e;
            L += e * ps[8 + hd];
          }
          const float inv = 1.0f / L;
          for (int s = 0; s < m.nsplit; ++s) wgt[s] *= inv;
        }
      }
#pragma unroll
      for (int s = 0; s < 8; ++s) cw[t][hd][s] = wgt[s];
    }
    __syncthreads();
    TT(1);
#pragma unroll
    for (int q = 0; q < TPW / TKG; ++q) {
      const int t = ta + q;
      int ns = 0, slot0 = 0;
      if (t < nt) {
        const TokMeta m = meta[tok0 + t];
        ns = ((mode & 8) && !(m.flags & 1)) ? 0 : m.nsplit;
        slot0 = m.slot0;
      }
      float v[8];
#pragma unroll
      for (int hd = 0; hd < 8; ++hd) v[hd] = 0.f;
      int s = 0;
      for (; s + 2 <= ns; s += 2) {
        const float *ps = part + (size_t)(slot0 + s) * PART_STRIDE + 16 + col;
        float pv[8], pw[8];
#pragma unroll
        for (int hd = 0; hd < 8; ++hd) { pv[hd] = ps[hd * 128]; pw[hd] = ps[PART_STRIDE + hd * 128]; }
#pragma unroll
        for (int hd = 0; hd < 8; ++hd) v[hd] = fmaf(cw[t][hd][s], pv[hd], v[hd]);
#pragma unroll
        for (int hd = 0; hd < 8; ++hd) v[hd] = fmaf(cw[t][hd][s + 1], pw[hd], v[hd]);
      }
      if (s < ns) {
        const float *ps = part + (size_t)(slot0 + s) * PART_STRIDE + 16 + col;
        float pv[8];
#pragma unroll
        for (int hd = 0; hd < 8; ++hd) pv[hd] = ps[hd * 128];
#pragma unroll
        for (int hd = 0; hd < 8; ++hd) v[hd] = fmaf(cw[t][hd][s], pv[hd], v[hd]);
      }
#pragma unroll
      for (int hd = 0; hd < 8; ++hd) mb[t][hd][col] = v[hd];
    }
    __syncthreads();
    TT(2);
    {
      float acc[TPW], o0, o1;
      matvec_part<128, TPW>(acc, W.WvT, 128, col, &mb[0][col >> 4][0], 8 * 132, kg);
      ksum<TPW>(acc, W.bv[col], rk, kg, col, o0, o1);
// ... 141 lines not shown
```

mind_amd/csrc/mind_hip.hip:

```cpp
#include <hip/hip_runtime.h>

#include <cmath>
#include <cstdarg>
#include <cstdio>
#include <cstdlib>
#include <algorithm>
#include <cstring>
#include <map>
#include <string>
#include <thread>
#include <atomic>
#include <functional>
#include <vector>

#include "../../include/mind_hip.h"
#include "encdec_kernels.hip"
#include "fusion_kernels.hip"
#include "pair_bf16_kernels.hip"
#include "pair_tile_kernels.hip"
#include "pair_tile6_kernels.hip"
#include "token_mfma_kernels.hip"
#include "actor_mfma_kernels.hip"
#include "actor_lw_kernels.hip"
#include "token_lw_kernels.hip"
// ... 121 lines not shown
  std::atomic<int> pa_state{0};
  mind_aime_plan_in pa_in;
  mind_aime_plan_out pa_out;
  int pa_rc = 0;
  struct Plan {
    AimeBook book;
    int agents = 0;
    long long gen = 0;
    const float *rows_p = nullptr, *fmean_p = nullptr, *fcov_p = nullptr;
    const float *dev_fmean = nullptr, *dev_fcov = nullptr;
  } plan;
  DevBuf pl_flat;
  DevBuf dec_xbuf, dec_bars;
  unsigned *dec_abort = nullptr;
  int rb_cur = 0, rb_gen = 0;
  size_t rb_S = 0, rb_a = 0;
  bool profiling = false;
  hipEvent_t ev_il0 = nullptr, ev_il1 = nullptr;
  float ilqr_ms = 0.f;
  int ilqr_multi = 0, ilqr_trees = 0;
  std::function<int()> il_finish;
  bool il_finish_owned = false;
  hipEvent_t ev_rows = nullptr;
  std::vector<const double *> il_trace_dev;
  std::vector<int> il_trace_its;
  int il_trace_cap = 0, il_trace_phases = 0;
  double il_prof[9] = {0, 0, 0, 0, 0, 0, 0, 0, 0};
  long long n_ilqr_fallbacks = 0;
  int n_pair_launch = 0;
  float pair_ms = 0.f;
  double pairs_done = 0.0;
  std::vector<hipEvent_t> ev;
  bool ev_defer = false;
  std::vector<hipEvent_t> ev_pool;
  size_t ev_pool_used = 0;
  std::vector<size_t> ev_pending;
  int n_cu = 256;
  int debug_layers = 6;
  int last_ntok = 0;
  size_t il_dbg[6] = {0, 0, 0, 0, 0, 0};
  long long last_edge_pairs = 0;
  int last_slots = 0, last_A = 0, last_B = 0;
};

static int fail(mind_ctx *c, int code, const char *fmt, ...) {
  char buf[512];
  va_list ap;
  va_start(ap, fmt);
  vsnprintf(buf, sizeof(buf), fmt, ap);
  va_end(ap);
  if (c) c->err = buf;
  return code;
}

#define HIPCHK(c, call)                                                                        \
  do {                                                                                         \
    hipError_t e_ = (call);                                                                    \
    if (e_ != hipSuccess)                                                                      \
      return fail(c, MIND_EHIP, "%s failed: %s (%s:%d)", #call, hipGetErrorString(e_), __FILE__, __LINE__); \
  } while (0)

static int ensure(mind_ctx *c, DevBuf &b, size_t bytes) {
  if (bytes <= b.cap) return MIND_OK;
  if (b.p) (void)hipFree(b.p);
  b.p = nullptr;
  b.cap = 0;
  size_t want = bytes < ((size_t)64 << 20) ? std::max<size_t>(2 * bytes, (size_t)1 << 20) : bytes + bytes / 4 + 4096;
  hipError_t e = hipMalloc(&b.p, want);
  if (e != hipSuccess) {
    e = hipMalloc(&b.p, bytes);
    want = bytes;
    if (e != hipSuccess) return fail(c, MIND_ENOMEM, "hipMalloc(%zu) failed: %s", bytes, hipGetErrorString(e));
  }
  b.cap = want;
  return MIND_OK;
}

static int ensure_exact(mind_ctx *c, DevBuf &b, size_t bytes, const char *what) {
  if (bytes <= b.cap) return MIND_OK;
  HIPCHK(c, hipStreamSynchronize(c->stream));
  if (b.p) (void)hipFree(b.p);
  b.p = nullptr;
  b.cap = 0;
  if (hipMalloc(&b.p, bytes) != hipSuccess) return fail(c, MIND_ENOMEM, "hipMalloc(%zu) for %s failed", bytes, what);
  b.cap = bytes;
  return MIND_OK;
}

extern "C" int mind_ctx_create(int device, void *stream, mind_ctx **out) {
  if (!out) return MIND_EINVAL;
  *out = nullptr;
  int n = 0;
  if (hipGetDeviceCount(&n) != hipSuccess || n <= 0) return MIND_EHIP;
  if (device < 0 || device >= n) return MIND_EINVAL;
  mind_ctx *c = new mind_ctx();
  c->device = device;
  if (hipSetDevice(device) != hipSuccess) { delete c; return MIND_EHIP; }
  c->stream = (hipStream_t)stream;
  if (hipStreamCreateWithFlags(&c->side, hipStreamNonBlocking) != hipSuccess) c->side = nullptr;
  if (c->side && hipEventCreateWithFlags(&c->ev_side, hipEventDisableTiming) != hipSuccess) { (void)hipStreamDestroy(c->side); c->side = nullptr; }
  if (c->side && hipEventCreateWithFlags(&c->ev_main, hipEventDisableTiming) != hipSuccess) { (void)hipStreamDestroy(c->side); c->side = nullptr; }
  if (c->side && hipEventCreateWithFlags(&c->ev_tgt, hipEventDisableTiming) != hipSuccess) { (void)hipStreamDestroy(c->side); c->side = nullptr; }
  if (hipEventCreateWithFlags(&c->ev_stage, hipEventDisableTiming) != hipSuccess) { *out = nullptr; delete c; return MIND_EHIP; }
  hipDeviceProp_t prop;
  if (hipGetDeviceProperties(&prop, device) == hipSuccess) c->n_cu = prop.multiProcessorCount;
  (void)hipFuncSetAttribute((const void *)k_pair<0>, hipFuncAttributeMaxDynamicSharedMemorySize, (int)mind_pair_lds_bytes());
  (void)hipFuncSetAttribute((const void *)k_pair<1>, hipFuncAttributeMaxDynamicSharedMemorySize, (int)mind_pair_lds_bytes());
  (void)hipFuncSetAttribute((const void *)k_pair_bf<0, 3>, hipFuncAttributeMaxDynamicSharedMemorySize, (int)mind_pair_bf_lds_bytes());
  (void)hipFuncSetAttribute((const void *)k_pair_bf<1, 3>, hipFuncAttributeMaxDynamicSharedMemorySize, (int)mind_pair_bf_lds_bytes());
  (void)hipFuncSetAttribute((const void *)k_pair_bf<0, 1>, hipFuncAttributeMaxDynamicSharedMemorySize, (int)mind_pair_bf_lds_bytes());
  (void)hipFuncSetAttribute((const void *)k_pair_bf<1, 1>, hipFuncAttributeMaxDynamicSharedMemorySize, (int)mind_pair_bf_lds_bytes());
  (void)hipFuncSetAttribute((const void *)k_pair_t<0, 3>, hipFuncAttributeMaxDynamicSharedMemorySize, (int)mind_pair_bf_lds_bytes());
  (void)hipFuncSetAttribute((const void *)k_pair_t<1, 3>, hipFuncAttributeMaxDynamicSharedMemorySize, (int)mind_pair_bf_lds_bytes());
  (void)hipFuncSetAttribute((const void *)k_pair_t<0, 1>, hipFuncAttributeMaxDynamicSharedMemorySize, (int)mind_pair_bf_lds_bytes());
  (void)hipFuncSetAttribute((const void *)k_pair_t<1, 1>, hipFuncAttributeMaxDynamicSharedMemorySize, (int)mind_pair_bf_lds_bytes());
  (void)hipFuncSetAttribute((const void *)k_pair_t6<0>, hipFuncAttributeMaxDynamicSharedMemorySize, (int)mind_pair_bf_lds_bytes());
  (void)hipFuncSetAttribute((const void *)k_pair_t6<1>, hipFuncAttributeMaxDynamicSharedMemorySize, (int)mind_pair_bf_lds_bytes());
  if (const char *te = getenv("MIND_PAIR_TILE")) c->pt.pair_tile = !(te[0] == '0');
  if (const char *xe = getenv("MIND_XCD_ORDER")) c->pt.xcd_order = !(xe[0] == '0');

  if (const char *pe = getenv("MIND_PAIR_PREC")) {
    const std::string v = pe;
    if (v == "f32" || v == "0") c->pair_prec = 0;
    else if (v == "bf16x3" || v == "1") c->pair_prec = 1;
    else if (v == "bf16" || v == "2") c->pair_prec = 2;
    else if (v == "bf16x6" || v == "3") c->pair_prec = 3;
  }
  (void)hipFuncSetAttribute((const void *)k_actor_net, hipFuncAttributeMaxDynamicSharedMemorySize, (int)mind_actor_lds_bytes());
  (void)hipFuncSetAttribute((const void *)k_actor_mfma<3>, hipFuncAttributeMaxDynamicSharedMemorySize, (int)mind_actor_mfma_lds_bytes());
  (void)hipFuncSetAttribute((const void *)k_actor_mfma<6>, hipFuncAttributeMaxDynamicSharedMemorySize, (int)mind_actor_mfma_lds_bytes());
  (void)hipFuncSetAttribute((const void *)k_dec_actor_mfma<1>, hipFuncAttributeMaxDynamicSharedMemorySize, (int)mind_dec_actor_mfma_lds_bytes());
  (void)hipFuncSetAttribute((const void *)k_dec_actor_mfma<3>, hipFuncAttributeMaxDynamicSharedMemorySize, (int)mind_dec_actor_mfma_lds_bytes());
  (void)hipFuncSetAttribute((const void *)k_dec_actor_mfma<6>, hipFuncAttributeMaxDynamicSharedMemorySize, (int)mind_dec_actor_mfma_lds_bytes());
  if (const char *se = getenv("MIND_ACTOR_SPLIT")) c->pt.actor_np = atoi(se) == 3 ? 3 : 6;
  (void)hipFuncSetAttribute((const void *)k_actor_mfma<1>, hipFuncAttributeMaxDynamicSharedMemorySize, (int)mind_actor_mfma_lds_bytes());
  if (const char *me = getenv("MIND_ENC_MFMA")) c->pt.enc_mfma = !(me[0] == '0');
  if (const char *me = getenv("MIND_ACTOR_F32")) c->pt.actor_f32 = !(me[0] == '0');
  if (const char *me = getenv("MIND_ACTOR_F32_MIN")) c->pt.actor_f32_min = atoi(me);
  if (const char *me = getenv("MIND_ACTOR_LW_MIN")) c->pt.actor_lw_min = atoi(me);
  lw_set_attributes();
  (void)hipFuncSetAttribute((const void *)k_actor_f32<1>, hipFuncAttributeMaxDynamicSharedMemorySize, (int)mind_actor_f32_lds_bytes(1));
  (void)hipFuncSetAttribute((const void *)k_actor_f32<2>, hipFuncAttributeMaxDynamicSharedMemorySize, (int)mind_actor_f32_lds_bytes(2));
  if (const char *de = getenv("MIND_DEC_MFMA_MIN")) c->pt.dec_mfma_min = atoi(de);
  if (const char *oe = getenv("MIND_DEC_OVERLAP")) c->pt.dec_overlap = !(oe[0] == '0');
  (void)hipFuncSetAttribute((const void *)k_ilqr<true, 0>, hipFuncAttributeMaxDynamicSharedMemorySize, (int)il_lds_bytes(0));
  (void)hipFuncSetAttribute((const void *)k_ilqr<false, 1>, hipFuncAttributeMaxDynamicSharedMemorySize, (int)il_lds_bytes(0));
  (void)hipFuncSetAttribute((const void *)k_ilqr<false, 0>, hipFuncAttributeMaxDynamicSharedMemorySize, (int)il_lds_bytes(0));
  (void)hipFuncSetAttribute((const void *)k_ilqr<false, 2>, hipFuncAttributeMaxDynamicSharedMemorySize, (int)il_lds_bytes(0));
  if (const char *te = getenv("MIND_TOK_MFMA")) c->pt.tok_mfma = !(te[0] == '0');
  if (const char *te = getenv("MIND_TOK_SMALL_MAX")) c->pt.tok_small_max = atoi(te);
  if (const char *te = getenv("MIND_TOK_MERGE")) c->pt.tok_merge = !(te[0] == '0');
  if (const char *te = getenv("MIND_DEC_MW")) c->pt.dec_mw = !(te[0] == '0');
  if (const char *te = getenv("MIND_DEC_CLS_SIDE")) c->pt.dec_cls_side = !(te[0] == '0');
  if (const char *te = getenv("MIND_TOK_BF_MIN_N")) c->pt.tok_bf_min_n = atoi(te);
  if (const char *te = getenv("MIND_TOK_LW_MIN_N")) c->pt.tok_lw_min_n = atoi(te);
  if (const char *te = getenv("MIND_TOK_LW_MIN")) c->pt.tok_lw_min = atoi(te);
  if (const char *te = getenv("MIND_TGT_SIDE")) c->pt.tgt_side = !(te[0] == '0');
  if (const char *te = getenv("MIND_PL_TAB_SIDE")) c->pl_tab_side = !(te[0] == '0');
  (void)hipFuncSetAttribute((const void *)k_token_mfma<0>, hipFuncAttributeMaxDynamicSharedMemorySize, (int)mind_token_mfma_lds_bytes());
  (void)hipFuncSetAttribute((const void *)k_token_mfma<1>, hipFuncAttributeMaxDynamicSharedMemorySize, (int)mind_token_mfma_lds_bytes());
  if (const char *ce = getenv("MIND_PLAN_CHUNK_MB")) { const long v = atol(ce); if (v > 0) c->plan_chunk_mb = v; }
  if (const char *we = getenv("MIND_TAB_SMALL")) c->tab_small = atoi(we) != 0;
  if (const char *we = getenv("MIND_TAB_HOST_MAX")) c->tab_host_max = std::max(0, atoi(we));
  if (const char *we = getenv("MIND_EARLY_EVAL")) c->early_eval = atoi(we) != 0;
  if (const char *we = getenv("MIND_GLUE_FUSED")) c->glue_fused = atoi(we) != 0;
  if (const char *we = getenv("MIND_DEC_MIRROR")) c->dec_mirror = atoi(we) != 0;
  if (const char *we = getenv("MIND_UPLOAD_KERNEL_MAX")) c->upload_kernel_max = std::max(0, atoi(we));
  const char *const il_env[][2] = {{"MIND_ILQR_CHUNK", "ilqr_chunk"}, {"MIND_ILQR_WGS", "ilqr_wgs"}, {"MIND_ILQR_SPEC_DERIV", "ilqr_spec_deriv"},
                                   {"MIND_ILQR_HOST_OUT_MAX", "ilqr_host_out_max"}, {"MIND_ILQR_SLOTS", "ilqr_slots"}};
  for (const auto &e : il_env)
    if (const char *we = getenv(e[0])) (void)ilqr_tuning_set(c->it, e[1], atoi(we));
  (void)hipFuncSetAttribute((const void *)k_dec_scene, hipFuncAttributeMaxDynamicSharedMemorySize, (int)mind_dec_scene_lds_bytes());
  (void)hipFuncSetAttribute((const void *)k_dec_scene_mw, hipFuncAttributeMaxDynamicSharedMemorySize, (int)mind_dec_scene_lds_bytes());
  (void)hipFuncSetAttribute((const void *)k_dec_scene_c, hipFuncAttributeMaxDynamicSharedMemorySize, (int)mind_dec_scene_lds_bytes());
  (void)hipFuncSetAttribute((const void *)k_dec_cls, hipFuncAttributeMaxDynamicSharedMemorySize, (int)mind_dec_scene_lds_bytes());
  (void)hipFuncSetAttribute((const void *)k_dec_tgt, hipFuncAttributeMaxDynamicSharedMemorySize, (int)mind_dec_scene_lds_bytes());
  (void)hipFuncSetAttribute((const void *)k_dec_actor<0>, hipFuncAttributeMaxDynamicSharedMemorySize, (int)mind_dec_actor_lds_bytes());
  (void)hipFuncSetAttribute((const void *)k_dec_actor<1>, hipFuncAttributeMaxDynamicSharedMemorySize, (int)mind_dec_actor_lds_bytes());
  (void)hipFuncSetAttribute((const void *)k_dec_actor<2>, hipFuncAttributeMaxDynamicSharedMemorySize, (int)mind_dec_actor_lds_bytes());
  *out = c;
  return MIND_OK;
}

extern "C" int mind_ctx_destroy(mind_ctx *c) {
  if (!c) return MIND_EINVAL;
  if (c->pa_thread.joinable()) c->pa_thread.join();
  (void)hipSetDevice(c->device);
  (void)hipStreamSynchronize(c->stream);
  DevBuf *bufs[] = {&c->edge, &c->x, &c->ST, &c->QK, &c->part, &c->tokpos, &c->meta, &c->jobs, &c->actor_feat,
                    &c->lane_feat, &c->tgt_feat, &c->cmode, &c->tgt_emb, &c->rows, &c->rpe_ptrs, &c->ilqr_dev, &c->aime_dev, &c->rebase_dev2[0], &c->rebase_dev2[1], &c->dec_h2};
  for (DevBuf *b : bufs)
    if (b->p) (void)hipFree(b->p);
  for (TableSet &t : c->tabs)
    for (DevBuf *b : {&t.meta, &t.jobs, &t.jobs5, &t.rows})
      if (b->p) (void)hipFree(b->p);
  if (c->wdev) (void)hipFree(c->wdev);
  for (DevBuf *b : {&c->dec_xbuf, &c->dec_bars})
    if (b->p) (void)hipFree(b->p);
  if (c->dec_abort) (void)hipHostFree(c->dec_abort);
  for (DevBuf *b : {&c->pl_root, &c->pl_in[0], &c->pl_in[1], &c->pl_lf, &c->pl_lrep, &c->pl_pred, &c->pl_small, &c->pl_tab[0], &c->pl_tab[1], &c->pl_win[0],
                    &c->pl_win[1], &c->pl_flat, &c->x_send, &c->x_recv, &c->x_seg})
    if (b->p) (void)hipFree(b->p);
  for (DevBuf &b : c->pl_world)
    if (b.p) (void)hipFree(b.p);
  for (void *q : c->pl_pin)
    if (q) (void)hipHostFree(q);
  if (c->ev_pl) (void)hipEventDestroy(c->ev_pl);
  if (c->ev_root) (void)hipEventDestroy(c->ev_root);
  if (c->ev_field) (void)hipEventDestroy(c->ev_field);
  if (c->il_field.p) (void)hipFree(c->il_field.p);
  if (c->il_field_pin) (void)hipHostFree(c->il_field_pin);
  if (c->ev_tab) (void)hipEventDestroy(c->ev_tab);
  if (c->ev_rows) (void)hipEventDestroy(c->ev_rows);
  if (c->pl_copy) (void)hipStreamDestroy(c->pl_copy);
  for (hipEvent_t e : c->ev) (void)hipEventDestroy(e);
  for (hipEvent_t e : c->ev_pool) (void)hipEventDestroy(e);
  if (c->ev_side) (void)hipEventDestroy(c->ev_side);
  if (c->ev_main) (void)hipEventDestroy(c->ev_main);
  if (c->ev_tgt) (void)hipEventDestroy(c->ev_tgt);
  if (c->ev_stage) (void)hipEventDestroy(c->ev_stage);
  if (c->ev_cls) (void)hipEventDestroy(c->ev_cls);
  if (c->actor_lw_arena.p) (void)hipFree(c->actor_lw_arena.p);
  if (c->tok_lw_arena.p) (void)hipFree(c->tok_lw_arena.p);
  for (hipEvent_t e : c->ev_tok) (void)hipEventDestroy(e);
  if (c->ev_act0) (void)hipEventDestroy(c->ev_act0);
  if (c->ev_act1) (void)hipEventDestroy(c->ev_act1);
  if (c->ev_il0) (void)hipEventDestroy(c->ev_il0);
  if (c->ev_il1) (void)hipEventDestroy(c->ev_il1);
  if (c->side) { (void)hipStreamSynchronize(c->side); (void)hipStreamDestroy(c->side); }
  if (c->own_stream) (void)hipStreamDestroy(c->stream);
  delete c;
  return MIND_OK;
}

extern "C" const char *mind_last_error_string(mind_ctx *c) { return c ? c->err.c_str() : "null context"; }

extern "C" int mind_ctx_synchronize(mind_ctx *c) {
  if (!c) return MIND_EINVAL;
  HIPCHK(c, hipStreamSynchronize(c->stream));
  return MIND_OK;
}

extern "C" int mind_set_tuning(mind_ctx *c, const char *name, int value) {
  if (!c || !name) return MIND_EINVAL;
  const std::string n = name;
  if (pred_tuning_set(c->pt, name, value)) return MIND_OK;
  if (ilqr_tuning_set(c->it, name, value)) return MIND_OK;
  if (n == "plan_chunk_mb") c->plan_chunk_mb = value < 1 ? 1 : value;
  else if (n == "pl_tab_side") c->pl_tab_side = value != 0;
  else if (n == "tab_small") c->tab_small = value != 0;
  else if (n == "tab_host_max") c->tab_host_max = value < 0 ? 0 : value;
  else if (n == "early_eval") c->early_eval = value != 0;
  else if (n == "glue_fused") c->glue_fused = value != 0;
  else if (n == "dec_mirror") c->dec_mirror = value != 0;
  else if (n == "upload_kernel_max") c->upload_kernel_max = value < 0 ? 0 : value;
  else return fail(c, MIND_EINVAL, "mind_set_tuning: unknown knob '%s'", name);
  return MIND_OK;
}

extern "C" int mind_set_exchange(mind_ctx *c, int rank, int world, mind_exchange_fn fn, void *user, int force) {
  if (!c) return MIND_EINVAL;
  if (fn && (world < 1 || rank < 0 || rank >= world)) return fail(c, MIND_EINVAL, "mind_set_exchange: rank %d of %d", rank, world);
  c->xfn = fn; c->xuser = user;
  c->xr = fn ? rank : 0; c->xw = fn ? world : 1; c->xforce = fn && force != 0;
  return MIND_OK;
}

extern "C" int mind_last_exchange_stats(mind_ctx *c, long long *collectives, long long *bytes) {
  if (!c) return MIND_EINVAL;
  if (collectives) *collectives = c->x_collectives;
  if (bytes) *bytes = c->x_bytes;
  return MIND_OK;
}

extern "C" int mind_set_pair_precision(mind_ctx *c, int mode) {
  if (!c || mode < 0 || mode > 3) return MIND_EINVAL;
  c->pair_prec = mode;
  return MIND_OK;
}

extern "C" int mind_get_pair_precision(mind_ctx *c) { return c ? c->pair_prec : MIND_EINVAL; }

namespace { std::vector<float> pack_bfrag(const std::vector<float> &w, int row_stride); }
extern "C" int mind_debug_pack_bfrag(const float *w, int row_stride, uint32_t *out) {
  if (!w || !out || row_stride < 128) return MIND_EINVAL;
  std::vector<float> v(w, w + (size_t)127 * row_stride + 128);
  v.resize((size_t)128 * row_stride, 0.f);
  const std::vector<float> t = pack_bfrag(v, row_stride);
  memcpy(out, t.data(), 16384 * sizeof(uint32_t));
  return MIND_OK;
}

extern "C" int mind_set_profiling(mind_ctx *c, int enable) {
  if (!c) return MIND_EINVAL;
  c->profiling = enable != 0;
  return MIND_OK;
}

extern "C" int mind_last_ilqr_stats(mind_ctx *c, float *kernel_ms, int *n_trees, int *workgroups_per_tree) {
  if (!c) return MIND_EINVAL;
  if (kernel_ms) *kernel_ms = c->ilqr_ms;
  if (n_trees) *n_trees = c->ilqr_trees;
  if (workgroups_per_tree) *workgroups_per_tree = c->ilqr_multi;
  return MIND_OK;
}

extern "C" int mind_last_ilqr_trace(mind_ctx *c, int tree, int phase, double *out, int cap_rows, int *n_rows) {
  if (!c || !n_rows || (cap_rows > 0 && !out)) return MIND_EINVAL;
  if (tree < 0 || tree >= (int)c->il_trace_dev.size() || phase < 0 || phase >= c->il_trace_phases || !c->il_trace_dev[tree])
    return fail(c, MIND_ESTATE, "mind_last_ilqr_trace: no trace for tree %d phase %d (the last tree-iLQR call had %d trees, %d phases)", tree, phase,
                (int)c->il_trace_dev.size(), c->il_trace_phases);
  const int rows = std::min(c->il_trace_its[2 * tree + phase], c->il_trace_cap);
  *n_rows = rows;
  const int take = std::min(rows, cap_rows);
  if (take > 0) {
    HIPCHK(c, hipMemcpyAsync(out, c->il_trace_dev[tree] + (size_t)phase * c->il_trace_cap * IL_TRACE_W, (size_t)take * IL_TRACE_W * sizeof(double),
                             hipMemcpyDeviceToHost, c->stream));
    HIPCHK(c, hipStreamSynchronize(c->stream));
  }
  return MIND_OK;
}

extern "C" int mind_last_ilqr_profile(mind_ctx *c, double *out9) {
  if (!c || !out9) return MIND_EINVAL;
  memcpy(out9, c->il_prof, sizeof(c->il_prof));
  return MIND_OK;
}

static int mind_pair_events_resolve(mind_ctx *c, float *total_ms) {
  float sum = 0.f;
  for (size_t base : c->ev_pending)
    for (int L = 0; L < c->debug_layers; ++L) {
// ... 794 lines not shown
    for (i = 8; i < n - (n % 8); i += 8)
      for (int j = 0; j < 8; ++j) r[j] += a[i + j];
    double res = ((r[0] + r[1]) + (r[2] + r[3])) + ((r[4] + r[5]) + (r[6] + r[7]));
    for (; i < n; ++i) res += a[i];
    return res;
  }
  long n2 = n / 2;
  n2 -= n2 % 8;
  return np_pairwise(a, n2) + np_pairwise(a + n2, n - n2);
}
template <class T>
void eval_nodes(const double *st, const double *ct, long N, const T *lane, int P, double tv, double *per_node) {
  const int S = P - 1;
  std::vector<T> dx(S), dy(S), l2(S);
  for (int q = 0; q < S; ++q) {
    dx[q] = lane[2 * q + 2] - lane[2 * q];
    dy[q] = lane[2 * q + 3] - lane[2 * q + 1];
    l2[q] = dx[q] * dx[q] + dy[q] * dy[q];
  }
  constexpr int BS = 8;
  const int NB = (S + BS - 1) / BS;
  std::vector<double> sx_(S), sy_(S), sr_(S), bx(NB), by(NB), br(NB);
  for (int q = 0; q < S; ++q) {
    const double ax = (double)lane[2 * q], ay = (double)lane[2 * q + 1], ex = (double)lane[2 * q + 2], ey = (double)lane[2 * q + 3];
    sx_[q] = 0.5 * (ax + ex); sy_[q] = 0.5 * (ay + ey);
    sr_[q] = 0.5 * sqrt((ex - ax) * (ex - ax) + (ey - ay) * (ey - ay)) * (1.0 + 1e-9) + 1e-9;
  }
  for (int b = 0; b < NB; ++b) {
    const int q0 = b * BS, q1 = std::min(S, q0 + BS);
    double cx = 0.0, cy = 0.0;
    for (int q = q0; q < q1; ++q) { cx += sx_[q]; cy += sy_[q]; }
    cx /= (double)(q1 - q0); cy /= (double)(q1 - q0);
    double r = 0.0;
    for (int q = q0; q < q1; ++q) r = std::max(r, sqrt((sx_[q] - cx) * (sx_[q] - cx) + (sy_[q] - cy) * (sy_[q] - cy)) + sr_[q]);
    bx[b] = cx; by[b] = cy; br[b] = r * (1.0 + 1e-9) + 1e-9;
  }
  int b_prev = 0;
  for (long i = 0; i < N; ++i) {
    const double px = st[6 * i], py = st[6 * i + 1];
    double emin = INFINITY, rmin = INFINITY;
    bool saw_nan = false;
    int b_best = b_prev;
    auto price_block = [&](int b) {
      const int q0 = b * BS, q1 = std::min(S, q0 + BS);
      for (int q = q0; q < q1; ++q) {
        if (emin < INFINITY) {
          const double cxq = px - sx_[q], cyq = py - sy_[q], lim = rmin + sr_[q];
          if (cxq * cxq + cyq * cyq > lim * lim) continue;
        }
        const double sx = (double)lane[2 * q], sy = (double)lane[2 * q + 1], ddx = (double)dx[q], ddy = (double)dy[q];
        double t = ((px - sx) * ddx + (py - sy) * ddy) / (double)l2[q];
        t = t < 0.0 ? 0.0 : (t > 1.0 ? 1.0 : t);
        const double ex = px - (sx + t * ddx), ey = py - (sy + t * ddy);
        const double e = ex * ex + ey * ey;
        if (e < emin) { emin = e; rmin = sqrt(e) * (1.0 + 1e-9) + 1e-9; b_best = b; }
        else if (e != e) saw_nan = true;
      }
    };
    price_block(b_prev);
    for (int b = 0; b < NB; ++b) {
      if (b == b_prev) continue;
      if (emin < INFINITY) {
        const double cxb = px - bx[b], cyb = py - by[b], lim = rmin + br[b];
        if (cxb * cxb + cyb * cyb > lim * lim) continue;
      }
      price_block(b);
    }
    b_prev = b_best;
    const double dmin = saw_nan ? (double)NAN : sqrt(emin);
    const double c0 = ct[2 * i], c1 = ct[2 * i + 1], dv = tv - st[6 * i + 2];
    per_node[i] = ((0.1 * (c0 * c0) + 5.0 * (c1 * c1)) + 0.01 * (dv * dv)) + 0.01 * dmin;
  }
}
}

extern "C" int mind_fill_tracks(const double *raw , int a, int T, const int32_t *slot ,
                                float *pos , float *ang , float *vel , int16_t *typ ,
                                int16_t *have ) {
  if (!raw || !slot || !pos || !ang || !vel || !typ || !have || a < 0 || T <= 0) return MIND_EINVAL;
  for (int i = 0; i < a; ++i) {
    const double *r = raw + (size_t)i * T * 6;
    int first = 0;
    for (int t = 0; t < T; ++t)
      if (r[t * 6] != 0.0) { first = t; break; }
    int src = -1;
    for (int t = 0; t < T; ++t) {
      const bool h = r[t * 6] != 0.0;
      if (h) src = t;
      const int f = src < 0 ? first : src;
      const bool hf = r[f * 6] != 0.0;
      const size_t o = (size_t)i * T + t;
      pos[2 * o] = hf ? (float)r[f * 6 + 1] : 0.f;
      pos[2 * o + 1] = hf ? (float)r[f * 6 + 2] : 0.f;
      ang[o] = hf ? (float)r[f * 6 + 3] : 0.f;
      vel[2 * o] = h ? (float)r[t * 6 + 4] : 0.f;
      vel[2 * o + 1] = h ? (float)r[t * 6 + 5] : 0.f;
      have[o] = h ? 1 : 0;
      for (int k = 0; k < 7; ++k) typ[o * 7 + k] = (h && k == slot[i]) ? 1 : 0;
    }
  }
  return MIND_OK;
}

extern "C" int mind_eval_traj_trees(const double *states, const double *ctrls, const int32_t *counts, int n_trees, const void *lane,
                                    int lane_is_f32, int n_lane_pts, double target_vel, double *out) {
  if (!states || !ctrls || !counts || n_trees <= 0 || !lane || n_lane_pts < 2 || !out) return MIND_EINVAL;
  long N = 0;
  for (int t = 0; t < n_trees; ++t) { if (counts[t] <= 0) return MIND_EINVAL; N += counts[t]; }
  std::vector<double> per(N);
  auto run = [&](long lo, long hi) {
    if (lane_is_f32) eval_nodes<float>(states + 6 * lo, ctrls + 2 * lo, hi - lo, (const float *)lane, n_lane_pts, target_vel, per.data() + lo);
    else eval_nodes<double>(states + 6 * lo, ctrls + 2 * lo, hi - lo, (const double *)lane, n_lane_pts, target_vel, per.data() + lo);
  };
  const long nth = std::min<long>(std::min<long>(8, (long)std::max(1u, std::thread::hardware_concurrency())), N / 8192);
  if (nth <= 1) run(0, N);
  else {
    std::vector<std::thread> th;
    for (long k = 0; k < nth; ++k) th.emplace_back(run, N * k / nth, N * (k + 1) / nth);
    for (std::thread &t : th) t.join();
  }
  long o = 0;
  for (int t = 0; t < n_trees; ++t) {
    const long n = counts[t];
    out[t] = (n > 1 ? per[o] + np_pairwise(per.data() + o + 1, n - 1) : per[o]) / (double)n;
    o += n;
  }
  return MIND_OK;
}

__global__ void k_debug_trig(const double *__restrict__ x, int n, double *__restrict__ out) {
  const int i = blockIdx.x * blockDim.x + threadIdx.x;
  const double v = i < n ? x[i] : 0.0;
  double s, c, t, c2;
  mind_sincos(v, &s, &c);
  mind_tan_cos(v, &t, &c2);
  if (i < n) { out[4 * i] = s; out[4 * i + 1] = c; out[4 * i + 2] = t; out[4 * i + 3] = c2; }
}
extern "C" int mind_debug_trig(mind_ctx *c, const double *x, int n, double *out) {
  if (!c || !x || !out || n <= 0) return MIND_EINVAL;
  HIPCHK(c, hipSetDevice(c->device));
  double *d = nullptr;
  HIPCHK(c, hipMalloc((void **)&d, (size_t)n * 5 * sizeof(double)));
  hipError_t e = hipMemcpy(d, x, (size_t)n * sizeof(double), hipMemcpyHostToDevice);
  if (e == hipSuccess) {
    hipLaunchKernelGGL(k_debug_trig, dim3((n + 63) / 64), dim3(64), 0, c->stream, d, n, d + n);
    e = hipStreamSynchronize(c->stream);
  }
  if (e == hipSuccess) e = hipMemcpy(out, d + n, (size_t)n * 4 * sizeof(double), hipMemcpyDeviceToHost);
  (void)hipFree(d);
  if (e != hipSuccess) return fail(c, MIND_EHIP, "mind_debug_trig: %s", hipGetErrorString(e));
  return MIND_OK;
}

extern "C" int mind_debug_set_layers(mind_ctx *c, int n) {
  if (!c || n < 0 || n > 6) return MIND_EINVAL;
  c->debug_layers = n;
  return MIND_OK;
}
extern "C" int64_t mind_debug_read(mind_ctx *c, const char *name, float *host, int64_t max_floats) {
  if (!c || !name) return MIND_EINVAL;
  const void *src = nullptr;
  int64_t n = 0;
  std::string k = name;
  if (k == "x") { src = c->x.p; n = (int64_t)c->last_ntok * 128; }
  else if (k == "ST") { src = c->ST.p; n = (int64_t)c->last_ntok * 256; }
  else if (k == "QK") { src = c->QK.p; n = (int64_t)c->last_ntok * 1024; }
  else if (k == "edge") { src = c->edge.p; n = c->last_edge_pairs * 128; }
  else if (k == "part") { src = c->part.p; n = (int64_t)c->last_slots * PART_STRIDE; }
  else if (k == "actor_feat") { src = c->actor_feat.p; n = (int64_t)c->last_A * 128; }
  else if (k == "tokpos") { src = c->tokpos.p; n = (int64_t)c->last_ntok * 4; }
  else if (k == "cmode") { src = c->cmode.p; n = (int64_t)c->last_B * 768; }
  else if (k == "tgt_emb") { src = c->tgt_emb.p; n = (int64_t)c->last_B * 128; }
  else if (k == "tgt_feat") { src = c->tgt_feat.p; n = (int64_t)c->last_B * 128; }
  else if (k == "il_spec") {
    if (!host) return 2;
    if (max_floats < 2) return MIND_EINVAL;
    host[0] = (float)c->il_spec_req; host[1] = (float)c->il_spec_hit;
    return 2;
  }
  else if (k.rfind("il_", 0) == 0 && c->il_dbg[5]) {
    const size_t M = c->il_dbg[5];
    int w = -1; size_t per = 0;
    if (k == "il_L") { w = 0; per = 1; } else if (k == "il_Lx") { w = 1; per = 6; } else if (k == "il_Lxx") { w = 2; per = 36; }
    else if (k == "il_Fx") { w = 3; per = 36; } else if (k == "il_xs") { w = 4; per = 6; }
    if (w < 0) return MIND_EINVAL;
    src = (const char *)c->ilqr_dev.p + c->il_dbg[w];
    n = (int64_t)(M * per * 2);
  }
  else return MIND_EINVAL;
  if (!host) return n;
  if (n > max_floats) n = max_floats;
  if (hipStreamSynchronize(c->stream) != hipSuccess) return MIND_EHIP;
  if (k == "edge" && c->last_edge_tiled) {
    long long pt = 0;
    for (int N : c->last_scene_n) pt += (long long)N * (((N + 15) / 16) * 16);
    const bool eb = c->last_edge_bf16;
    std::vector<float> raw((size_t)pt * (eb ? 64 : 128));
    if (hipMemcpy(raw.data(), src, raw.size() * sizeof(float), hipMemcpyDeviceToHost) != hipSuccess) return MIND_EHIP;
    int64_t o = 0;
    size_t sb = 0;
    for (int N : c->last_scene_n) {
      const int rows = ((N + 15) / 16) * 16;
      for (int j = 0; j < N; ++j)
        for (int i = 0; i < N; ++i)
          for (int f = 0; f < 128 && o < n; ++f, ++o) {
            const int t = i >> 4, pp = i & 15, b = f >> 4, qq = (f >> 2) & 3, r = f & 3;
            const size_t tile0 = sb + (size_t)j * rows + (size_t)t * 16;
            if (!eb) host[o] = raw[tile0 * 128 + ((b * 64 + qq * 16 + pp) * 4 + r)];
            else {
              uint32_t w;
              memcpy(&w, &raw[tile0 * 64 + (((b >> 1) * 64 + qq * 16 + pp) * 4 + 2 * (b & 1) + (r >> 1))], 4);
              w = (r & 1) ? (w & 0xffff0000u) : (w << 16);
              memcpy(&host[o], &w, 4);
            }
          }
      sb += (size_t)N * rows;
    }
    return n;
  }
  if (hipMemcpy(host, src, (size_t)n * sizeof(float), hipMemcpyDeviceToHost) != hipSuccess) return MIND_EHIP;
  return n;
}

#include "loop.hip"
```

mind_amd/csrc/pred_choice.h:

```cpp
#pragma once
#include <cstring>
#include <vector>

struct PredTuning {
  bool pair_tile = true;
  bool xcd_order = true;
  bool enc_mfma = true;
  int actor_np = 6;
  bool actor_f32 = true;
  int actor_f32_min = 1 << 30, actor_f32_pair_min = 1 << 30;
  int actor_lw_min = 1 << 30, actor_lw_chunk = 0;
  bool tok_mfma = false;
  int tok_bf_min_n = 0;
  int tok_lw_min_n = 1 << 30, tok_lw_min = 1 << 30, tok_lw_chunk = 0;
  bool tok_merge = true;
  int tok_small_max = 2048;
  int dec_mfma_min = 1 << 30;
  bool dec_overlap = true;
  bool dec_mw = false;
  bool dec_cls_side = false;
  bool tgt_side = true;
};

static bool pred_tuning_set(PredTuning &t, const char *name, int value) {
  const auto is = [name](const char *k) { return strcmp(name, k) == 0; };
  if (is("dec_mfma_min")) t.dec_mfma_min = value;
  else if (is("enc_mfma")) t.enc_mfma = value != 0;
  else if (is("actor_f32")) t.actor_f32 = value != 0;
  else if (is("actor_f32_min")) t.actor_f32_min = value;
  else if (is("actor_f32_pair_min")) t.actor_f32_pair_min = value;
  else if (is("actor_lw_min")) t.actor_lw_min = value;
  else if (is("actor_lw_chunk")) t.actor_lw_chunk = value < 0 ? 0 : value;
  else if (is("actor_split")) t.actor_np = value == 3 ? 3 : 6;
  else if (is("xcd_order")) t.xcd_order = value != 0;
  else if (is("pair_tile")) t.pair_tile = value != 0;
  else if (is("dec_overlap")) t.dec_overlap = value != 0;
  else if (is("tok_mfma")) t.tok_mfma = value != 0;
  else if (is("tok_small_max")) t.tok_small_max = value;
  else if (is("tok_merge")) t.tok_merge = value != 0;
  else if (is("dec_mw")) t.dec_mw = value != 0;
  else if (is("dec_cls_side")) t.dec_cls_side = value != 0;
  else if (is("tok_bf_min_n")) t.tok_bf_min_n = value;
  else if (is("tok_lw_min_n")) t.tok_lw_min_n = value;
  else if (is("tok_lw_min")) t.tok_lw_min = value;
  else if (is("tok_lw_chunk")) t.tok_lw_chunk = value < 0 ? 0 : value;
  else if (is("tgt_side")) t.tgt_side = value != 0;
  else return false;
  return true;
}

static inline int pred_mfma_parts(const PredTuning &t, int pair_prec) {
  return (pair_prec == 3 || (pair_prec == 1 && t.actor_np == 6)) ? 6 : (pair_prec == 1 ? 3 : 1);
}

static inline bool pred_edge_tiled(const PredTuning &t, int pair_prec) { return pair_prec == 3 || (pair_prec != 0 && t.pair_tile); }

static inline int pred_edge_pair_bytes(const PredTuning &t, int pair_prec) { return pred_edge_tiled(t, pair_prec) && pair_prec == 2 ? 256 : 512; }

enum PredActorForm { PRED_ACTOR_VALU = 0, PRED_ACTOR_F32 = 1, PRED_ACTOR_MFMA = 2, PRED_ACTOR_LW = 3 };
enum PredPairFamily { PRED_PAIR_F32 = 0, PRED_PAIR_BF = 1, PRED_PAIR_T = 2, PRED_PAIR_T6 = 3 };
enum PredDecActor { PRED_DEC_ONE = 0, PRED_DEC_SPLIT = 1, PRED_DEC_MFMA = 2 };

struct PredTokRun {
  int t0, n, kind;
  bool layerwise;
  bool small, merged;
};

struct PredChoice {
  int np = 1;
  int actor_form = PRED_ACTOR_VALU, actor_arg = 0, actor_grid = 0, actor_chunk = 0, actor_chunks = 1, actor_launches = 1;
  int qsplit = 0, qk_stride = 1024;
  bool tiled = false, edge_bf16 = false;
  std::vector<PredTokRun> tok_runs;
  int tok_chunk = 0;
  bool tok_lw = false;
  int last_tok_chunks = 0;
  int pair_family = PRED_PAIR_F32, pair_np = 0;
  bool l5_jobs5 = false;
  int xcd_lanes = 1, xcd_lanes5 = 1;
  int dec_actor = PRED_DEC_ONE;
  bool fp32_dec = true, split_dec = false, want_mw = false, cls_side = false;
  int mw_blocks = 0;
  bool tgt_wait_first = false;
};

static PredChoice pred_choose(const PredTuning &t, int pair_prec, int n_cu, bool have_side, int n_scenes, const int *scene_actors, const int *scene_lanes) {
  PredChoice ch;
  int A = 0;
  for (int b = 0; b < n_scenes; ++b) A += scene_actors[b];
  ch.np = pred_mfma_parts(t, pair_prec);

  ch.actor_grid = A;
  if (t.actor_f32 && A >= (pair_prec == 0 ? t.actor_f32_pair_min : t.actor_f32_min)) {
    ch.actor_form = PRED_ACTOR_F32; ch.actor_arg = 2; ch.actor_grid = (A + 1) / 2;
  } else if (pair_prec == 0 && t.actor_f32 && t.enc_mfma) {
    ch.actor_form = PRED_ACTOR_F32; ch.actor_arg = 1;
  } else if (pair_prec == 0 || !t.enc_mfma) {
    ch.actor_form = PRED_ACTOR_VALU;
  } else if (A >= t.actor_lw_min) {
    ch.actor_form = PRED_ACTOR_LW; ch.actor_arg = ch.np;
    ch.actor_chunk = t.actor_lw_chunk > 0 ? t.actor_lw_chunk : LW_CHUNK;
    ch.actor_chunks = (A + ch.actor_chunk - 1) / ch.actor_chunk;
    ch.actor_grid = ch.actor_chunks;
    ch.actor_launches = ch.actor_chunks * (1 + 2 * LW_NSTAGE);
  } else {
    ch.actor_form = PRED_ACTOR_MFMA; ch.actor_arg = ch.np;
  }

  ch.qsplit = pair_prec == 3 ? 48 : pair_prec != 0 ? 16 : 0;
  ch.qk_stride = pair_prec == 3 ? P6_QK_STRIDE : 1024;
  ch.tiled = pred_edge_tiled(t, pair_prec);
  ch.edge_bf16 = pred_edge_pair_bytes(t, pair_prec) == 256;

  ch.tok_chunk = t.tok_lw_chunk > 0 ? t.tok_lw_chunk : TL_CHUNK;
  long long njobs = 0, njobs5 = 0;
  int t0 = 0;
  for (int b = 0; b < n_scenes; ++b) {
    const int N = scene_actors[b] + scene_lanes[b] + 1;
    const int kind = t.tok_mfma ? 1 : (pair_prec != 0 && pair_prec != 3 && t.tok_bf_min_n > 0 && N >= t.tok_bf_min_n) ? 2 : N >= t.tok_lw_min_n ? 1 : 0;
    if (!ch.tok_runs.empty() && ch.tok_runs.back().kind == kind) ch.tok_runs.back().n += N;
    else ch.tok_runs.push_back({t0, N, kind, false, false, false});
    t0 += N;
    njobs += (long long)N * pair_column_splits(N);
    njobs5 += (long long)(scene_actors[b] + 1) * pair_column_splits(N);
  }
  for (PredTokRun &r : ch.tok_runs) {
    r.layerwise = r.kind == 1 && r.n >= t.tok_lw_min;
    r.small = r.kind == 0 && r.n <= t.tok_small_max;
    r.merged = r.small && t.tok_merge;
    if (r.layerwise) {
      ch.tok_lw = true;
      ch.last_tok_chunks += (r.n + ch.tok_chunk - 1) / ch.tok_chunk;
    }
  }

  ch.pair_family = pair_prec == 0 ? PRED_PAIR_F32 : pair_prec == 3 ? PRED_PAIR_T6 : ch.tiled ? PRED_PAIR_T : PRED_PAIR_BF;
  ch.pair_np = (ch.pair_family == PRED_PAIR_T || ch.pair_family == PRED_PAIR_BF) ? (pair_prec == 1 ? 3 : 1) : 0;
  ch.l5_jobs5 = ch.tiled;
  ch.xcd_lanes = pair_xcd_lanes(t.xcd_order, n_scenes, pair_grid(njobs, n_cu));
  ch.xcd_lanes5 = pair_xcd_lanes(t.xcd_order, n_scenes, pair_grid(njobs5, n_cu));

  ch.fp32_dec = pair_prec == 0 || !t.enc_mfma || A < t.dec_mfma_min;
  ch.split_dec = ch.fp32_dec && have_side && t.dec_overlap;
  ch.dec_actor = ch.split_dec ? PRED_DEC_SPLIT : ch.fp32_dec ? PRED_DEC_ONE : PRED_DEC_MFMA;
  ch.mw_blocks = ((n_scenes + 7) / 8) * 8 * DEC_MW_G;
  ch.want_mw = t.dec_mw && ch.mw_blocks <= n_cu;
  ch.cls_side = ch.split_dec && t.dec_cls_side;
  ch.tgt_wait_first = have_side && !t.tgt_side;
  return ch;
}
```

mind_amd/csrc/predict.hip:

```cpp
__global__ void k_tokpos(const TokMeta *__restrict__ meta, int n_tok, const float *__restrict__ actr,
                         const float *__restrict__ avec, const float *__restrict__ lctr,
                         const float *__restrict__ lvec, float *__restrict__ tokpos) {
  const int t = blockIdx.x * blockDim.x + threadIdx.x;
  if (t >= n_tok) return;
  const TokMeta m = meta[t];
  float4 o = make_float4(0.f, 0.f, 0.f, 0.f);
  if (m.type == 0 && actr) o = make_float4(actr[m.src * 2], actr[m.src * 2 + 1], avec[m.src * 2], avec[m.src * 2 + 1]);
  if (m.type == 1 && lctr) o = make_float4(lctr[m.src * 2], lctr[m.src * 2 + 1], lvec[m.src * 2], lvec[m.src * 2 + 1]);
  ((float4 *)tokpos)[t] = o;
}

struct PairTables {
  std::vector<TokMeta> meta;
  std::vector<PairJob> jobs, jobs5;
  std::vector<int> actor_row, actor_scene, cls_row, scene_n;
  long long edge_pairs = 0, edge_pairs_t = 0;
  int ntok = 0, slot = 0;
  double pairs_full = 0, pairs_l5 = 0;
};

static void pair_tables_build(int Bn, const int *scene_actors, const int *scene_lanes, bool xcd_order, int n_cu, PairTables &T) {
  int A = 0;
  for (int b = 0; b < Bn; ++b) A += scene_actors[b];
  T.actor_row.assign(A, 0); T.actor_scene.assign(A, 0); T.cls_row.assign(Bn, 0); T.scene_n.assign(Bn, 0);
  int a0 = 0, l0 = 0;
  for (int b = 0; b < Bn; ++b) {
    const int a = scene_actors[b], l = scene_lanes[b];
    const int N = a + l + 1;
    const int tiles = (N + 15) / 16;
    const int ns = pair_column_splits(N);
    for (int j = 0; j < N; ++j) {
      TokMeta m;
      memset(&m, 0, sizeof(m));
      m.type = j < a ? 0 : (j < a + l ? 1 : 2);
      m.src = j < a ? a0 + j : (j < a + l ? l0 + (j - a) : 0);
      m.slot0 = T.slot;
      m.nsplit = ns;
      m.flags = (j < a || j == N - 1) ? 1 : 0;
      T.meta.push_back(m);
      for (int s_ = 0; s_ < ns; ++s_) {
        PairJob J;
        memset(&J, 0, sizeof(J));
        J.edge_base = T.edge_pairs;
        J.edge_base_t = T.edge_pairs_t;
        J.N = N;
        J.j = j;
        pair_job_range(tiles, ns, s_, &J.t0, &J.t1);
        J.tok_base = T.ntok;
        J.slot = T.slot++;
        J.flags = m.flags;
        J.scene = b;
        T.jobs.push_back(J);
      }
      if (j < a) { T.actor_row[a0 + j] = T.ntok + j; T.actor_scene[a0 + j] = b; }
    }
    T.cls_row[b] = T.ntok + N - 1;
    T.scene_n[b] = N;
    T.ntok += N;
    T.edge_pairs += (long long)N * N;
    T.edge_pairs_t += (long long)N * tiles * 16;
    T.pairs_full += (double)N * N;
    T.pairs_l5 += (double)N * (a + 1);
    a0 += a; l0 += l;
  }
  for (const PairJob &J : T.jobs)
    if (J.flags & 1) T.jobs5.push_back(J);
  for (std::vector<PairJob> *jl : {&T.jobs, &T.jobs5}) {
    const int grid = pair_grid((long long)jl->size(), n_cu);
    pair_jobs_deal(*jl, grid, PAIR_WAVES, pair_xcd_lanes(xcd_order, Bn, grid));
  }
}

extern "C" int mind_debug_pair_schedule(const int *scene_tokens, const int *scene_actors, int n_scenes, int n_cu, int last_layer, int *out_jobs, int cap,
                                        int *out_info) {
  if (!scene_tokens || !scene_actors || n_scenes <= 0 || n_cu <= 0 || !out_jobs || !out_info) return MIND_EINVAL;
  std::vector<int> lanes(n_scenes);
  for (int b = 0; b < n_scenes; ++b) {
    const int N = scene_tokens[b], a = scene_actors[b];
    if (N <= 0 || a < 0 || a >= N) return MIND_EINVAL;
    lanes[b] = N - a - 1;
  }
  PairTables T;
  pair_tables_build(n_scenes, scene_actors, lanes.data(), true, n_cu, T);
  const std::vector<PairJob> &jl = last_layer ? T.jobs5 : T.jobs;
  const int grid = pair_grid((long long)jl.size(), n_cu);
  const int stride = grid * PAIR_WAVES;
  int n = 0;
  for (size_t i = 0; i < jl.size(); ++i) {
    const PairJob &J = jl[i];
    if (J.t1 <= J.t0) continue;
    if (n < cap) {
      int *o = out_jobs + (size_t)6 * n;
      o[0] = J.scene; o[1] = J.j; o[2] = J.t0; o[3] = J.t1; o[4] = J.slot; o[5] = (int)(i % stride);
    }
    ++n;
  }
  out_info[0] = pair_column_splits(scene_tokens[0]); out_info[1] = grid; out_info[2] = (int)jl.size(); out_info[3] = n;
  return n;
}

#define PRED_CHOICE_HEADER 32
extern "C" int mind_debug_predict_choice(const char *const *knob_names, const int *knob_values, int n_knobs, int pair_prec, int n_cu, int have_side,
                                         const int *scene_actors, const int *scene_lanes, int n_scenes, long long *out, int cap) {
  if (n_knobs < 0 || (n_knobs > 0 && (!knob_names || !knob_values)) || pair_prec < 0 || pair_prec > 3 || n_cu <= 0 || !scene_actors || !scene_lanes ||
      n_scenes <= 0 || cap < 0 || (cap > 0 && !out))
    return MIND_EINVAL;
  PredTuning t;
  for (int k = 0; k < n_knobs; ++k)
    if (!knob_names[k] || !pred_tuning_set(t, knob_names[k], knob_values[k])) return MIND_EINVAL;
  for (int b = 0; b < n_scenes; ++b)
    if (scene_actors[b] <= 0 || scene_lanes[b] < 0) return MIND_EINVAL;
  const PredChoice ch = pred_choose(t, pair_prec, n_cu, have_side != 0, n_scenes, scene_actors, scene_lanes);
  const bool mfma_dec = ch.dec_actor == PRED_DEC_MFMA;
  const long long head[PRED_CHOICE_HEADER] = {
      PRED_CHOICE_HEADER, (long long)ch.tok_runs.size(), ch.np, ch.actor_form, ch.actor_arg, ch.actor_grid, ch.actor_chunk, ch.actor_chunks,
      ch.actor_launches, ch.qsplit, ch.qk_stride, ch.tiled, ch.edge_bf16, pred_edge_pair_bytes(t, pair_prec), ch.tok_chunk, ch.tok_lw,
      ch.last_tok_chunks, ch.pair_family, ch.pair_np, ch.l5_jobs5, ch.xcd_lanes, ch.xcd_lanes5, ch.dec_actor, mfma_dec ? ch.np : 0,
      ch.fp32_dec, ch.split_dec, ch.want_mw, ch.mw_blocks, ch.cls_side && !ch.want_mw, ch.tgt_wait_first, 0, 0};
  std::vector<long long> rec(head, head + PRED_CHOICE_HEADER);
  for (const PredTokRun &r : ch.tok_runs) rec.insert(rec.end(), {r.t0, r.n, r.kind, r.layerwise, r.small, r.merged});
  for (size_t i = 0; i < rec.size() && (int)i < cap; ++i) out[i] = rec[i];
  return (int)rec.size();
}

struct PredCall {
  mind_ctx *c;
  const mind_scene_batch *in;
  mind_pred_out *out;
  const PredChoice &ch;
  int Bn, A, Ltot;
  hipStream_t st, ss;
  TableSet *ts = nullptr;
  const float *lane_feat = nullptr;
  const float *const *rpe_dev = nullptr;
  hipEvent_t *evs = nullptr;
  bool tok_timed = false;
  size_t ev_tok_used = 0;
  float *x() const { return (float *)c->x.p; }
  const int *rows() const { return (const int *)ts->rows.p; }
};

static int pred_tables(PredCall &p, const int *scene_actors, const int *scene_lanes) {
  mind_ctx *c = p.c;
  const int Bn = p.Bn, A = p.A;
  std::vector<int> key;
  key.reserve(2 * Bn + 3);
  key.push_back(Bn);
  for (int b = 0; b <= Bn; ++b) key.push_back(p.in->actor_off[b]);
  for (int b = 0; b <= Bn; ++b) key.push_back(p.in->lane_off[b]);
  TableSet *ts = nullptr;
  for (TableSet &t : c->tabs)
    if (t.key == key) ts = &t;
  const bool tab_hit = ts != nullptr;
  if (!ts) {
    ts = &c->tabs[0];
    for (TableSet &t : c->tabs)
      if (t.stamp < ts->stamp) ts = &t;
  }
  ts->stamp = ++c->tab_clock;
  p.ts = ts;
  if (tab_hit) {
    c->n_table_hits++;
    return MIND_OK;
  }
  PairTables T;
  pair_tables_build(Bn, scene_actors, scene_lanes, c->pt.xcd_order, c->n_cu, T);
  int rc;
  ts->key.clear();
  if ((rc = ensure(c, ts->meta, T.meta.size() * sizeof(TokMeta)))) return rc;
  if ((rc = ensure(c, ts->jobs, T.jobs.size() * sizeof(PairJob)))) return rc;
  if ((rc = ensure(c, ts->jobs5, T.jobs5.size() * sizeof(PairJob)))) return rc;
  if ((rc = ensure(c, ts->rows, (size_t)(2 * A + Bn) * sizeof(int)))) return rc;
  HIPCHK(c, hipMemcpyAsync(ts->meta.p, T.meta.data(), T.meta.size() * sizeof(TokMeta), hipMemcpyHostToDevice, p.st));
  HIPCHK(c, hipMemcpyAsync(ts->jobs.p, T.jobs.data(), T.jobs.size() * sizeof(PairJob), hipMemcpyHostToDevice, p.st));
  HIPCHK(c, hipMemcpyAsync(ts->jobs5.p, T.jobs5.data(), T.jobs5.size() * sizeof(PairJob), hipMemcpyHostToDevice, p.st));
  std::vector<int> rows(2 * A + Bn);
  memcpy(rows.data(), T.actor_row.data(), A * sizeof(int));
  memcpy(rows.data() + A, T.actor_scene.data(), A * sizeof(int));
  memcpy(rows.data() + 2 * A, T.cls_row.data(), Bn * sizeof(int));
  HIPCHK(c, hipMemcpyAsync(ts->rows.p, rows.data(), rows.size() * sizeof(int), hipMemcpyHostToDevice, p.st));
  HIPCHK(c, hipStreamSynchronize(p.st));
  ts->actor_row.swap(T.actor_row);
  ts->cls_row.swap(T.cls_row);
  ts->scene_n.swap(T.scene_n);
  ts->edge_pairs = T.edge_pairs; ts->edge_pairs_t = T.edge_pairs_t; ts->ntok = T.ntok; ts->slot = T.slot; ts->njobs = (int)T.jobs.size();
  ts->njobs5 = (int)T.jobs5.size();
  ts->pairs_full = T.pairs_full; ts->pairs_l5 = T.pairs_l5;
  ts->key.swap(key);
  return MIND_OK;
}

static int pred_workspaces(PredCall &p) {
  mind_ctx *c = p.c;
  const TableSet *ts = p.ts;
  const int ntok = ts->ntok, Bn = p.Bn;
  int rc;
  if ((rc = ensure(c, c->edge, (size_t)(p.ch.tiled ? ts->edge_pairs_t : ts->edge_pairs) * 128 * sizeof(float)))) return rc;
  if ((rc = ensure(c, c->x, (size_t)ntok * 128 * sizeof(float)))) return rc;
  if ((rc = ensure(c, c->ST, (size_t)ntok * 256 * sizeof(float)))) return rc;
  if ((rc = ensure(c, c->QK, (size_t)(ntok + 1) * p.ch.qk_stride * sizeof(float)))) return rc;
  if ((rc = ensure(c, c->part, (size_t)ts->slot * PART_STRIDE * sizeof(float)))) return rc;
  if ((rc = ensure(c, c->tokpos, (size_t)ntok * 4 * sizeof(float)))) return rc;
  if ((rc = ensure(c, c->actor_feat, (size_t)p.A * 128 * sizeof(float)))) return rc;
  if ((rc = ensure(c, c->lane_feat, (size_t)(p.Ltot > 0 ? p.Ltot : 1) * 128 * sizeof(float)))) return rc;
  if ((rc = ensure(c, c->tgt_feat, (size_t)Bn * 128 * sizeof(float)))) return rc;
  if ((rc = ensure(c, c->cmode, (size_t)Bn * 768 * sizeof(float)))) return rc;
  if ((rc = ensure(c, c->tgt_emb, (size_t)Bn * 128 * sizeof(float)))) return rc;
  if (p.in->rpe) {
    if ((rc = ensure(c, c->rpe_ptrs, (size_t)Bn * sizeof(float *)))) return rc;
    HIPCHK(c, hipMemcpyAsync(c->rpe_ptrs.p, p.in->rpe, (size_t)Bn * sizeof(float *), hipMemcpyHostToDevice, p.st));
    HIPCHK(c, hipStreamSynchronize(p.st));
    p.rpe_dev = (const float *const *)c->rpe_ptrs.p;
  }
  return MIND_OK;
}

static int pred_actor_net(PredCall &p) {
  mind_ctx *c = p.c;
  const PredChoice &ch = p.ch;
  const float *actors = p.in->actors;
  float *actor_feat = (float *)c->actor_feat.p;
  const int A = p.A;
  const dim3 grid(ch.actor_grid);
  switch (ch.actor_form) {
  case PRED_ACTOR_F32:
    if (ch.actor_arg == 2) hipLaunchKernelGGL(k_actor_f32<2>, grid, dim3(AF_T), mind_actor_f32_lds_bytes(2), p.st, actors, A, actor_feat, c->actorFW);
    else hipLaunchKernelGGL(k_actor_f32<1>, grid, dim3(AF_T), mind_actor_f32_lds_bytes(1), p.st, actors, A, actor_feat, c->actorFW);
    break;
  case PRED_ACTOR_VALU:
    hipLaunchKernelGGL(k_actor_net, grid, dim3(AT), mind_actor_lds_bytes(), p.st, actors, A, actor_feat, c->actorW);
    break;
  case PRED_ACTOR_LW: {
    int rc;
    if ((rc = ensure_exact(c, c->actor_lw_arena, lw_arena_bytes(ch.actor_chunk), "the layer-wise ActorNet's arena"))) return rc;
    lw_build_plan(A, ch.actor_chunk, c->actor_lw_plan);
    u32 *arena = (u32 *)c->actor_lw_arena.p;
    const int nl = ch.np == 6 ? lw_run<6>(c->actor_lw_plan, p.st, arena, actors, actor_feat, c->actorBW)
                 : ch.np == 3 ? lw_run<3>(c->actor_lw_plan, p.st, arena, actors, actor_feat, c->actorBW)
                              : lw_run<1>(c->actor_lw_plan, p.st, arena, actors, actor_feat, c->actorBW);
    if (nl < 0) return fail(c, MIND_ESTATE, "layer-wise ActorNet: a stage has no kernel");
    c->last_actor_lw = 1; c->last_actor_launches = nl; c->last_actor_chunks = ch.actor_chunks;
    break;
  }
  default:
    if (ch.np == 6) hipLaunchKernelGGL(k_actor_mfma<6>, grid, dim3(AM_T), mind_actor_mfma_lds_bytes(), p.st, actors, A, actor_feat, c->actorBW);
    else if (ch.np == 3) hipLaunchKernelGGL(k_actor_mfma<3>, grid, dim3(AM_T), mind_actor_mfma_lds_bytes(), p.st, actors, A, actor_feat, c->actorBW);
    else hipLaunchKernelGGL(k_actor_mfma<1>, grid, dim3(AM_T), mind_actor_mfma_lds_bytes(), p.st, actors, A, actor_feat, c->actorBW);
  }
  return MIND_OK;
}

static int pred_encoders(PredCall &p) {
  mind_ctx *c = p.c;
  const mind_scene_batch *in = p.in;
  hipStream_t st = p.st, ss = p.ss;
  const int Bn = p.Bn, Ltot = p.Ltot, ntok = p.ts->ntok;
  if (c->side) {
    HIPCHK(c, hipEventRecord(c->ev_main, st));
    HIPCHK(c, hipStreamWaitEvent(c->side, c->ev_main, 0));
  }
  const bool act_timed = c->profiling && !c->ev_defer;
  if (act_timed && !c->ev_act0) {
    HIPCHK(c, hipEventCreate(&c->ev_act0));
    HIPCHK(c, hipEventCreate(&c->ev_act1));
  }
  c->last_actor_lw = 0; c->last_actor_launches = 1; c->last_actor_chunks = 1; c->actor_ms = 0.f;
  if (act_timed) HIPCHK(c, hipEventRecord(c->ev_act0, st));
  int rc;
  if ((rc = pred_actor_net(p))) return rc;
  if (act_timed) HIPCHK(c, hipEventRecord(c->ev_act1, st));
  p.lane_feat = in->lane_feat;
// ... 14 lines not shown
  hipLaunchKernelGGL(k_lane_net, dim3((Bn + PL - 1) / PL), dim3(DT), 0, ss, in->tgt_nodes, Bn, (float *)c->tgt_feat.p, c->laneW);
  hipLaunchKernelGGL(k_dec_tgt, dim3(Bn), dim3(DT), mind_dec_scene_lds_bytes(), ss, (const float *)c->tgt_feat.p, in->tgt_rpe, (float *)c->tgt_emb.p,
                     c->decW);
  if (c->side) HIPCHK(c, hipEventRecord(c->ev_tgt, c->side));
  if (p.ch.tgt_wait_first) HIPCHK(c, hipStreamWaitEvent(st, c->ev_tgt, 0));
  return MIND_OK;
}

static hipError_t pred_tok_mark(PredCall &p, int tag) {
  mind_ctx *c = p.c;
  if (!p.tok_timed) return hipSuccess;
  if (p.ev_tok_used == c->ev_tok.size()) {
    hipEvent_t e;
    const hipError_t rc_ = hipEventCreate(&e);
    if (rc_ != hipSuccess) return rc_;
    c->ev_tok.push_back(e);
    c->ev_tok_tag.push_back(0);
  }
  c->ev_tok_tag[p.ev_tok_used] = tag;
  return hipEventRecord(c->ev_tok[p.ev_tok_used++], p.st);
}

static int pred_token_step(PredCall &p, int mode, int Lw) {
  mind_ctx *c = p.c;
  hipStream_t st = p.st;
  const size_t qk_stride = p.ch.qk_stride, tokm_lds = mind_token_mfma_lds_bytes();
  const float *actor_feat = (const float *)c->actor_feat.p, *lane_feat = p.lane_feat;
  float *part = (float *)c->part.p;
  HIPCHK(c, pred_tok_mark(p, -1));
  for (const PredTokRun &r : p.ch.tok_runs) {
    const TokMeta *m_ = (const TokMeta *)p.ts->meta.p + r.t0;
    float *x_ = p.x() + (size_t)r.t0 * 128, *ST_ = (float *)c->ST.p + (size_t)r.t0 * 256, *QK_ = (float *)c->QK.p + (size_t)r.t0 * qk_stride;
    if (r.layerwise) {
      tl_build_plan(r.n, mode, p.ch.tok_chunk, c->n_cu, c->tok_lw_plan);
      for (const TlLaunch &L : c->tok_lw_plan) {
        if (tl_launch(L, st, mode, m_, actor_feat, lane_feat, x_, part, ST_, QK_, qk_stride, c->tokW[Lw], c->tokWM[Lw], (float *)c->tok_lw_arena.p, p.ch.tok_chunk))
          return fail(c, MIND_ESTATE, "layer-wise token stage: a stage has no kernel");
        HIPCHK(c, pred_tok_mark(p, L.stage));
      }
      c->last_tok_launches += (int)c->tok_lw_plan.size();
      continue;
    }
    c->last_tok_launches++;
    if (r.kind == 0) {
      const int tpw = r.small ? TOK_TPW_SMALL : TOK_TPW_BIG;
      hipLaunchKernelGGL(r.small ? (r.merged ? k_token_m : k_token<TOK_TPW_SMALL>) : k_token<TOK_TPW_BIG>, dim3((r.n + tpw - 1) / tpw), dim3(TT_THREADS), 0,
                         st, m_, r.n, mode, actor_feat, lane_feat, x_, part, ST_, QK_, c->tokW[Lw]);
    } else if (r.kind == 1) {
      hipLaunchKernelGGL(k_token_mfma<0>, dim3((r.n + TM_TOK - 1) / TM_TOK), dim3(TM_THREADS), tokm_lds, st, m_, r.n, mode, actor_feat, lane_feat, x_,
                         part, ST_, QK_, c->tokW[Lw], c->tokWM[Lw]);
    } else {
      hipLaunchKernelGGL(k_token_mfma<1>, dim3((r.n + TM_TOK - 1) / TM_TOK), dim3(TM_THREADS), tokm_lds, st, m_, r.n, mode, actor_feat, lane_feat, x_,
                         part, ST_, QK_, c->tokW[Lw], c->tokWB[Lw]);
    }
    HIPCHK(c, pred_tok_mark(p, TL_NSTAGE));
  }
  return MIND_OK;
}

static int pred_pair_layer(PredCall &p, int L) {
  mind_ctx *c = p.c;
  const PredChoice &ch = p.ch;
  const TableSet *ts = p.ts;
  const bool last = L == 5, own5 = last && ch.l5_jobs5;
  const int um = L < 4 ? 0 : (L == 4 ? 1 : 2);
  const PairJob *jl = (const PairJob *)(own5 ? ts->jobs5.p : ts->jobs.p);
  const int nj = own5 ? ts->njobs5 : ts->njobs;
  const dim3 grid(pair_grid(nj, c->n_cu)), block(PAIR_THREADS);
  float *edge = (float *)c->edge.p, *ST = (float *)c->ST.p, *QK = (float *)c->QK.p, *part = (float *)c->part.p, *tokpos = (float *)c->tokpos.p;
  const size_t ldsb = mind_pair_bf_lds_bytes();
  const u32 *we = c->WBe[L], *wp = last ? c->WBe[L] : c->WBp[L];
  if (c->profiling) HIPCHK(c, hipEventRecord(p.evs[2 * L], p.st));
#define PAIR_GO(K0, K1, LDS, ...)                                                                                                             \
  do {                                                                                                                                        \
    if (L == 0) hipLaunchKernelGGL(K0, grid, block, LDS, p.st, jl, nj, edge, ST, QK, part, __VA_ARGS__, c->vtab[L], c->rtab, tokpos, p.rpe_dev, um); \
    else hipLaunchKernelGGL(K1, grid, block, LDS, p.st, jl, nj, edge, ST, QK, part, __VA_ARGS__, c->vtab[L], c->rtab, tokpos, p.rpe_dev, um);        \
  } while (0)
  switch (ch.pair_family) {
  case PRED_PAIR_F32: PAIR_GO((k_pair<0>), (k_pair<1>), mind_pair_lds_bytes(), c->WAe[L], last ? c->WAe[L] : c->WAp[L]); break;
  case PRED_PAIR_T6: PAIR_GO((k_pair_t6<0>), (k_pair_t6<1>), ldsb, we, wp, c->WLe[L], last ? c->WLe[L] : c->WLp[L]); break;
  case PRED_PAIR_T:
    if (ch.pair_np == 3) PAIR_GO((k_pair_t<0, 3>), (k_pair_t<1, 3>), ldsb, we, wp);
    else PAIR_GO((k_pair_t<0, 1>), (k_pair_t<1, 1>), ldsb, we, wp);
    break;
  default:
    if (ch.pair_np == 3) PAIR_GO((k_pair_bf<0, 3>), (k_pair_bf<1, 3>), ldsb, we, wp);
    else PAIR_GO((k_pair_bf<0, 1>), (k_pair_bf<1, 1>), ldsb, we, wp);
  }
#undef PAIR_GO
  if (c->profiling) HIPCHK(c, hipEventRecord(p.evs[2 * L + 1], p.st));
  c->n_pair_launch++;
  c->pairs_done += last ? ts->pairs_l5 : ts->pairs_full;
  return MIND_OK;
}

static int pred_fusion(PredCall &p) {
  mind_ctx *c = p.c;
  const PredChoice &ch = p.ch;
  const TableSet *ts = p.ts;
  int rc;
  c->last_tok_lw = ch.tok_lw; c->last_tok_launches = 0; c->last_tok_chunks = ch.last_tok_chunks; c->tok_ms = 0.f;
  for (float &v : c->tok_stage_ms) v = 0.f;
  if (ch.tok_lw && (rc = ensure_exact(c, c->tok_lw_arena, tl_arena_bytes(ch.tok_chunk), "the layer-wise token stage's arena"))) return rc;
  p.tok_timed = c->profiling && !c->ev_defer;
  if ((rc = pred_token_step(p, 1 | 4 | ch.qsplit, 0))) return rc;
  c->n_pair_launch = 0;
  c->pairs_done = 0;
  if (c->profiling && c->ev.size() < 12) {
    while (c->ev.size() < 12) {
      hipEvent_t e;
      HIPCHK(c, hipEventCreate(&e));
      c->ev.push_back(e);
    }
  }
  p.evs = c->ev.data();
  if (c->profiling && c->ev_defer) {
    while (c->ev_pool.size() < c->ev_pool_used + 12) {
      hipEvent_t e;
      HIPCHK(c, hipEventCreate(&e));
      c->ev_pool.push_back(e);
    }
    p.evs = c->ev_pool.data() + c->ev_pool_used;
    c->ev_pending.push_back(c->ev_pool_used);
    c->ev_pool_used += 12;
  }
  c->last_ntok = ts->ntok; c->last_edge_pairs = ts->edge_pairs; c->last_slots = ts->slot; c->last_A = p.A; c->last_B = p.Bn;
  c->last_scene_n = ts->scene_n; c->last_edge_tiled = ch.tiled; c->last_edge_bf16 = ch.edge_bf16;
  for (int L = 0; L < c->debug_layers; ++L) {
    if ((rc = pred_pair_layer(p, L))) return rc;
    if ((rc = pred_token_step(p, 2 | (L < 5 ? 4 : 8) | ch.qsplit, L + 1))) return rc;
  }
  return MIND_OK;
}

static int pred_decoder(PredCall &p) {
  mind_ctx *c = p.c;
  const PredChoice &ch = p.ch;
  mind_pred_out *out = p.out;
  hipStream_t st = p.st;
  const int A = p.A, Bn = p.Bn;
  const float *x = p.x();
  const int *d_actor_row = p.rows(), *d_actor_scene = d_actor_row + A, *d_cls_row = d_actor_row + 2 * A;
  const float *cmode = (const float *)c->cmode.p, *tgt_emb = (const float *)c->tgt_emb.p;
  const dim3 agrid((A + RA - 1) / RA), mgrid((A + DM_RA - 1) / DM_RA);
  int rc;
  if (ch.split_dec) {
    if ((rc = ensure(c, c->dec_h2, (size_t)A * 768 * sizeof(float)))) return rc;
    HIPCHK(c, hipEventRecord(c->ev_main, st));
    HIPCHK(c, hipStreamWaitEvent(c->side, c->ev_main, 0));
    hipLaunchKernelGGL(k_dec_actor<1>, agrid, dim3(DT), mind_dec_actor_lds_bytes(), c->side, x, d_actor_row, d_actor_scene, A,
                       (const float *)nullptr, (const float *)nullptr, (float *)nullptr, (float *)nullptr, c->decW, (float *)c->dec_h2.p);
    HIPCHK(c, hipEventRecord(c->ev_side, c->side));
  }
  bool cls_on_side = false;
  bool mw = ch.want_mw;
  if (mw) {
    if (c->dec_abort && *(volatile unsigned *)c->dec_abort) return fail(c, MIND_EHIP, "k_dec_scene_mw: a barrier of an earlier launch timed out (launch not resident)");
    if (!c->dec_abort) {
      if (hipHostMalloc((void **)&c->dec_abort, 64, hipHostMallocMapped) != hipSuccess) { c->dec_abort = nullptr; mw = false; }
      else *c->dec_abort = 0u;
    }
    const size_t need_x = (size_t)(c->n_cu / DEC_MW_G) * 2 * 6 * 1536 * sizeof(float), need_b = (size_t)(c->n_cu / DEC_MW_G) * 4 * sizeof(unsigned);
    if (mw && c->dec_xbuf.cap < need_x) {
      if ((rc = ensure(c, c->dec_xbuf, need_x))) return rc;
    }
    if (mw && c->dec_bars.cap < need_b) {
      if ((rc = ensure(c, c->dec_bars, need_b))) return rc;
      HIPCHK(c, hipMemsetAsync(c->dec_bars.p, 0, c->dec_bars.cap, st));
    }
  }
  if (mw)
    hipLaunchKernelGGL(k_dec_scene_mw, dim3(ch.mw_blocks), dim3(DT), mind_dec_scene_lds_bytes(), st, x, d_cls_row, (float *)c->cmode.p, out->cls, c->decW, Bn,
                       (float *)c->dec_xbuf.p, (unsigned *)c->dec_bars.p, c->dec_abort);
  else if (ch.cls_side) {
    hipLaunchKernelGGL(k_dec_scene_c, dim3(Bn), dim3(DT), mind_dec_scene_lds_bytes(), st, x, d_cls_row, (float *)c->cmode.p, c->decW);
    HIPCHK(c, hipEventRecord(c->ev_main, st));
    HIPCHK(c, hipStreamWaitEvent(c->side, c->ev_main, 0));
    hipLaunchKernelGGL(k_dec_cls, dim3(Bn), dim3(DT), mind_dec_scene_lds_bytes(), c->side, (float *)c->cmode.p, out->cls, c->decW);
    if (!c->ev_cls) HIPCHK(c, hipEventCreateWithFlags(&c->ev_cls, hipEventDisableTiming));
    HIPCHK(c, hipEventRecord(c->ev_cls, c->side));
    cls_on_side = true;
  } else
    hipLaunchKernelGGL(k_dec_scene, dim3(Bn), dim3(DT), mind_dec_scene_lds_bytes(), st, x, d_cls_row, (float *)c->cmode.p, out->cls, c->decW);
  if (c->side) HIPCHK(c, hipStreamWaitEvent(st, c->ev_tgt, 0));
  switch (ch.dec_actor) {
  case PRED_DEC_SPLIT:
    HIPCHK(c, hipStreamWaitEvent(st, c->ev_side, 0));
    hipLaunchKernelGGL(k_dec_actor<2>, agrid, dim3(DT), mind_dec_actor_lds_bytes(), st, x, d_actor_row, d_actor_scene, A, cmode, tgt_emb, out->reg,
                       out->vel, c->decW, (float *)c->dec_h2.p);
    break;
  case PRED_DEC_ONE:
    hipLaunchKernelGGL(k_dec_actor<0>, agrid, dim3(DT), mind_dec_actor_lds_bytes(), st, x, d_actor_row, d_actor_scene, A, cmode, tgt_emb, out->reg,
                       out->vel, c->decW, (float *)nullptr);
    break;
  default: {
#define DEC_MFMA(NPV)                                                                                                                     \
  hipLaunchKernelGGL(k_dec_actor_mfma<NPV>, mgrid, dim3(DM_T), mind_dec_actor_mfma_lds_bytes(), st, x, d_actor_row, d_actor_scene, A, cmode, \
                     tgt_emb, out->reg, out->vel, c->decBW)
    if (ch.np == 6) DEC_MFMA(6);
    else if (ch.np == 3) DEC_MFMA(3);
    else DEC_MFMA(1);
#undef DEC_MFMA
  }
  }
  if (cls_on_side) HIPCHK(c, hipStreamWaitEvent(st, c->ev_cls, 0));
  return MIND_OK;
}

static int pred_finish(PredCall &p) {
  mind_ctx *c = p.c;
  mind_pred_out *out = p.out;
  const float *x = p.x();
  for (int a = 0; a < p.A && out->actor_emb; ++a)
    HIPCHK(c, hipMemcpyAsync(out->actor_emb + (size_t)a * 128, x + (size_t)p.ts->actor_row[a] * 128, 128 * sizeof(float), hipMemcpyDeviceToDevice, p.st));
  for (int b = 0; b < p.Bn && out->cls_emb; ++b)
    HIPCHK(c, hipMemcpyAsync(out->cls_emb + (size_t)b * 128, x + (size_t)p.ts->cls_row[b] * 128, 128 * sizeof(float), hipMemcpyDeviceToDevice, p.st));
  HIPCHK(c, hipGetLastError());
  if (c->profiling && c->ev_defer) {
    c->pair_ms = 0.f;
  } else if (c->profiling) {
    HIPCHK(c, hipStreamSynchronize(p.st));
    c->pair_ms = 0.f;
    for (int L = 0; L < c->debug_layers; ++L) {
      float ms = 0.f;
      HIPCHK(c, hipEventElapsedTime(&ms, c->ev[2 * L], c->ev[2 * L + 1]));
      c->pair_ms += ms;
    }
    if (c->ev_act0) HIPCHK(c, hipEventElapsedTime(&c->actor_ms, c->ev_act0, c->ev_act1));
    for (size_t i = 1; i < p.ev_tok_used; ++i) {
      if (c->ev_tok_tag[i] < 0) continue;
      float ms = 0.f;
      HIPCHK(c, hipEventElapsedTime(&ms, c->ev_tok[i - 1], c->ev_tok[i]));
      c->tok_stage_ms[c->ev_tok_tag[i]] += ms;
      c->tok_ms += ms;
    }
  }
  return MIND_OK;
}

extern "C" int mind_predict_batch(mind_ctx *c, const mind_scene_batch *in, mind_pred_out *out) {
  if (!c || !in || !out) return MIND_EINVAL;
  if (!c->have_weights) return fail(c, MIND_ESTATE, "weights not loaded");
  const int Bn = in->n_scenes;
  if (Bn <= 0 || !in->actor_off || !in->lane_off || !in->actors || !in->tgt_nodes || !in->tgt_rpe || !out->cls ||
      !out->reg || !out->vel)
    return fail(c, MIND_EINVAL, "null input/output pointer");
  if (!in->lanes && !in->lane_feat) return fail(c, MIND_EINVAL, "need lanes or lane_feat");
  if (!in->rpe && !(in->actor_ctrs && in->actor_vecs && in->lane_ctrs && in->lane_vecs))
    return fail(c, MIND_EINVAL, "need rpe or ctrs/vecs");
  HIPCHK(c, hipSetDevice(c->device));
  const int A = in->actor_off[Bn], Ltot = in->lane_off[Bn];
  if (A <= 0 || Ltot < 0) return fail(c, MIND_EINVAL, "empty batch");
  std::vector<int> sa(Bn), sl(Bn);
  for (int b = 0; b < Bn; ++b) {
    sa[b] = in->actor_off[b + 1] - in->actor_off[b]; sl[b] = in->lane_off[b + 1] - in->lane_off[b];
    if (sa[b] <= 0 || sl[b] < 0) return fail(c, MIND_EINVAL, "scene %d has %d agents, %d lanes", b, sa[b], sl[b]);
  }
  const PredChoice ch = pred_choose(c->pt, c->pair_prec, c->n_cu, c->side != nullptr, Bn, sa.data(), sl.data());
  PredCall p{c, in, out, ch, Bn, A, Ltot, c->stream, c->side ? c->side : c->stream};
  int rc;
  if ((rc = pred_tables(p, sa.data(), sl.data()))) return rc;
  if ((rc = pred_workspaces(p))) return rc;
  if ((rc = pred_encoders(p))) return rc;
  if ((rc = pred_fusion(p))) return rc;
  if ((rc = pred_decoder(p))) return rc;
  return pred_finish(p);
}
```

mind_amd/csrc/token_mfma_kernels.hip:

```cpp
#define TM_TOK 16
#define TM_THREADS 256
#define TM_LDX 132
#define TM_LDT 260
#define TM_HP 8

struct TokWeightsM {
  const float *Wv, *Wo, *W1a, *W1b, *W2a, *W2b;
  const float *Ws, *Wt, *Wq, *Wkf;
  const float *Wpa, *Wpl;
};

typedef float tm_f4 __attribute__((ext_vector_type(4)));

struct TmFrag { tm_f4 a0[8], a1[8]; };
__device__ __forceinline__ void tm_load(TmFrag &F, const float *__restrict__ Wf, int ob0, int lane) {
  const tm_f4 *A = reinterpret_cast<const tm_f4 *>(Wf) + (size_t)ob0 * 8 * 64 + lane;
#pragma unroll
  for (int s4 = 0; s4 < 8; ++s4) { F.a0[s4] = A[s4 * 64]; F.a1[s4] = A[(8 + s4) * 64]; }
}
template <int BF>
__device__ __forceinline__ void tm_mma(tm_f4 (&acc)[2], const TmFrag &F, int ob0, const float *xb, int ob_stride, int lane) {
  if (BF) {
    const float *b0p = xb + 8 * (lane >> 4) + (size_t)ob0 * ob_stride;
    const float *b1p = b0p + ob_stride;
#pragma unroll
    for (int g = 0; g < 4; ++g) {
      u32x4 bh[2], bl[2];
#pragma unroll
      for (int t = 0; t < 2; ++t) {
        if (t == 1 && !ob_stride) { bh[1] = bh[0]; bl[1] = bl[0]; break; }
        const float *bp = (t ? b1p : b0p) + 32 * g;
        const tm_f4 x0 = *reinterpret_cast<const tm_f4 *>(bp), x1 = *reinterpret_cast<const tm_f4 *>(bp + 4);
        const float v[8] = {x0[0], x0[1], x0[2], x0[3], x1[0], x1[1], x1[2], x1[3]};
#pragma unroll
        for (int d = 0; d < 4; ++d) {
          const u32 h = pk_bf16(v[2 * d], v[2 * d + 1]);
          bh[t][d] = h;
          bl[t][d] = pk_bf16(v[2 * d] - bf_lo_f32(h), v[2 * d + 1] - bf_hi_f32(h));
        }
      }
      const u32x4 a0h = __builtin_bit_cast(u32x4, F.a0[g]), a0l = __builtin_bit_cast(u32x4, F.a0[4 + g]);
      const u32x4 a1h = __builtin_bit_cast(u32x4, F.a1[g]), a1l = __builtin_bit_cast(u32x4, F.a1[4 + g]);
      acc[0] = MFMA_BF(a0l, bh[0], acc[0]);
      acc[1] = MFMA_BF(a1l, bh[1], acc[1]);
      acc[0] = MFMA_BF(a0h, bl[0], acc[0]);
      acc[1] = MFMA_BF(a1h, bl[1], acc[1]);
      acc[0] = MFMA_BF(a0h, bh[0], acc[0]);
      acc[1] = MFMA_BF(a1h, bh[1], acc[1]);
    }
    return;
  }
  const float *b0p = xb + 4 * (lane >> 4) + (size_t)ob0 * ob_stride;
  const float *b1p = b0p + ob_stride;
#pragma unroll
  for (int s4 = 0; s4 < 8; ++s4) {
    const tm_f4 b0 = *reinterpret_cast<const tm_f4 *>(b0p + 16 * s4);
    const tm_f4 b1 = ob_stride ? *reinterpret_cast<const tm_f4 *>(b1p + 16 * s4) : b0;
#pragma unroll
    for (int w = 0; w < 4; ++w) {
      acc[0] = __builtin_amdgcn_mfma_f32_16x16x4f32(F.a0[s4][w], b0[w], acc[0], 0, 0, 0);
      acc[1] = __builtin_amdgcn_mfma_f32_16x16x4f32(F.a1[s4][w], b1[w], acc[1], 0, 0, 0);
    }
  }
}
template <int BF>
__device__ __forceinline__ void tm_gemm(tm_f4 (&acc)[2], const float *__restrict__ Wf, int ob0, const float *xb, int ob_stride, int lane) {
  TmFrag F;
  tm_load(F, Wf, ob0, lane);
  tm_mma<BF>(acc, F, ob0, xb, ob_stride, lane);
}

#define TM_FEAT(ob, i) (16 * (ob) + 4 * (lane >> 4) + (i))

__device__ __forceinline__ void tm_layernorm(float *tile, int ld, const float *__restrict__ g, const float *__restrict__ be, bool relu, int tid) {
  const int row = tid >> 4, part = tid & 15;
  float *p = tile + row * ld + part * 8;
  float v[8], s = 0.f;
#pragma unroll
  for (int k = 0; k < 8; ++k) { v[k] = p[k]; s += v[k]; }
#pragma unroll
  for (int o = 8; o > 0; o >>= 1) s += __shfl_xor(s, o, 64);
  const float mean = s * (1.0f / 128.0f);
  float q = 0.f;
#pragma unroll
  for (int k = 0; k < 8; ++k) { v[k] -= mean; q += v[k] * v[k]; }
#pragma unroll
  for (int o = 8; o > 0; o >>= 1) q += __shfl_xor(q, o, 64);
  const float inv = 1.0f / sqrtf(q * (1.0f / 128.0f) + 1e-5f);
#pragma unroll
  for (int k = 0; k < 8; ++k) {
    float y = v[k] * inv * g[part * 8 + k] + be[part * 8 + k];
    p[k] = relu ? fmaxf(y, 0.f) : y;
  }
}

template <int BF>
__global__ __launch_bounds__(TM_THREADS) void k_token_mfma(const TokMeta *__restrict__ meta, int n_tok, int mode, const float *__restrict__ actor_feat,
                                                           const float *__restrict__ lane_feat, float *__restrict__ x, const float *__restrict__ part,
                                                           float *__restrict__ ST, float *__restrict__ QK, TokWeights W, TokWeightsM WM) {
  extern __shared__ __attribute__((aligned(16))) float tm_sm[];
  float *xs = tm_sm;
  float *tmp = xs + TM_TOK * TM_LDX;
  float *mb = tmp + TM_TOK * TM_LDT;
  float *cw = mb + TM_TOK * TM_HP * TM_LDX;
  const int tid = threadIdx.x, lane = tid & 63, wave = tid >> 6;
  const int tok0 = blockIdx.x * TM_TOK;
  const int nt = min(TM_TOK, n_tok - tok0);
  const int ob0 = 2 * wave;
  const int tk = lane & 15;
  const bool tk_ok = tk < nt;
  TmFrag Fv, Fo;
  bool pre = false;

  if (mode & 1) {
    for (int e = tid; e < TM_TOK * 128; e += TM_THREADS) {
      const int t = e >> 7, col = e & 127;
      float f = 0.f;
      if (t < nt) {
        const TokMeta m = meta[tok0 + t];
        if (m.type == 0) f = actor_feat[(size_t)m.src * 128 + col];
        else if (m.type == 1) f = lane_feat[(size_t)m.src * 128 + col];
      }
      tmp[t * TM_LDT + col] = f;
    }
    __syncthreads();
    const int ty = tk_ok ? meta[tok0 + tk].type : 2;
    tm_f4 aa[2] = {{0, 0, 0, 0}, {0, 0, 0, 0}}, al[2] = {{0, 0, 0, 0}, {0, 0, 0, 0}};
    tm_gemm<BF>(aa, WM.Wpa, ob0, tmp + tk * TM_LDT, 0, lane);
    tm_gemm<BF>(al, WM.Wpl, ob0, tmp + tk * TM_LDT, 0, lane);
#pragma unroll
    for (int t = 0; t < 2; ++t)
#pragma unroll
      for (int i = 0; i < 4; ++i) {
        const int f = TM_FEAT(ob0 + t, i);
        xs[tk * TM_LDX + f] = ty == 0 ? aa[t][i] + W.bpa[f] : al[t][i] + W.bpl[f];
      }
    __syncthreads();
    {
      const int row = tid >> 4, prt = tid & 15;
      const int tyr = row < nt ? meta[tok0 + row].type : 2;
      tm_layernorm(xs, TM_LDX, tyr == 0 ? W.gpa : W.gpl, tyr == 0 ? W.bepa : W.bepl, true, tid);
      if (tyr == 2) {
#pragma unroll
        for (int k = 0; k < 8; ++k) xs[row * TM_LDX + prt * 8 + k] = 0.f;
      }
    }
    __syncthreads();
  } else {
    for (int e = tid; e < TM_TOK * 128; e += TM_THREADS) {
      const int t = e >> 7, col = e & 127;
      xs[t * TM_LDX + col] = t < nt ? x[(size_t)(tok0 + t) * 128 + col] : 0.f;
    }
    __syncthreads();
  }
  if (mode & 2) {
    if (tid < TM_TOK * 8) {
      const int t = tid >> 3, hd = tid & 7;
      float wgt[8];
#pragma unroll
      for (int s = 0; s < 8; ++s) wgt[s] = 0.f;
      if (t < nt) {
        const TokMeta m = meta[tok0 + t];
        if (!((mode & 8) && !(m.flags & 1))) {
          float M = -INFINITY;
          for (int s = 0; s < m.nsplit; ++s) M = fmaxf(M, part[(size_t)(m.slot0 + s) * PART_STRIDE + hd]);
          float L = 0.f;
          for (int s = 0; s < m.nsplit; ++s) {
            const float *ps = part + (size_t)(m.slot0 + s) * PART_STRIDE;
            const float e = expf(ps[hd] - M);
            wgt[s] = e;
            L += e * ps[8 + hd];
          }
          const float inv = 1.0f / L;
          for (int s = 0; s < m.nsplit; ++s) wgt[s] *= inv;
        }
      }
#pragma unroll
      for (int s = 0; s < 8; ++s) cw[(t * 8 + hd) * 8 + s] = wgt[s];
    }
    __syncthreads();
    tm_load(Fv, WM.Wv, ob0, lane);
    TmFrag F1a, F1b;
    for (int h0_ = 0; h0_ < 8; h0_ += TM_HP) {
      {
        const int t = tid >> 4, c8 = (tid & 15) * 8;
        int ns = 0, slot0 = 0;
        if (t < nt) {
          const TokMeta m = meta[tok0 + t];
          ns = ((mode & 8) && !(m.flags & 1)) ? 0 : m.nsplit;
          slot0 = m.slot0;
        }
        tm_f4 v[TM_HP][2];
#pragma unroll
        for (int hd = 0; hd < TM_HP; ++hd) { v[hd][0] = tm_f4{0, 0, 0, 0}; v[hd][1] = tm_f4{0, 0, 0, 0}; }
        for (int sp = 0; sp < ns; ++sp) {
          const tm_f4 *ps = reinterpret_cast<const tm_f4 *>(part + (size_t)(slot0 + sp) * PART_STRIDE + 16 + (size_t)h0_ * 128 + c8);
          tm_f4 pv[TM_HP][2];
#pragma unroll
          for (int hd = 0; hd < TM_HP; ++hd) { pv[hd][0] = ps[hd * 32]; pv[hd][1] = ps[hd * 32 + 1]; }
#pragma unroll
          for (int hd = 0; hd < TM_HP; ++hd) {
            const float wgt = cw[(t * 8 + h0_ + hd) * 8 + sp];
#pragma unroll
            for (int k = 0; k < 4; ++k) { v[hd][0][k] = fmaf(wgt, pv[hd][0][k], v[hd][0][k]); v[hd][1][k] = fmaf(wgt, pv[hd][1][k], v[hd][1][k]); }
          }
        }
#pragma unroll
        for (int hd = 0; hd < TM_HP; ++hd) {
          *reinterpret_cast<tm_f4 *>(mb + (t * TM_HP + hd) * TM_LDX + c8) = v[hd][0];
          *reinterpret_cast<tm_f4 *>(mb + (t * TM_HP + hd) * TM_LDX + c8 + 4) = v[hd][1];
        }
      }
      __syncthreads();
      if (ob0 >= h0_ && ob0 < h0_ + TM_HP) {
        tm_f4 acc[2] = {{0, 0, 0, 0}, {0, 0, 0, 0}};
        tm_mma<BF>(acc, Fv, ob0 - h0_, mb + (size_t)tk * TM_HP * TM_LDX, TM_LDX, lane);
#pragma unroll
        for (int t = 0; t < 2; ++t)
#pragma unroll
          for (int i = 0; i < 4; ++i) { const int f = TM_FEAT(ob0 + t, i); tmp[tk * TM_LDT + f] = acc[t][i] + W.bv[f]; }
      }
      __syncthreads();
    }
    tm_load(Fo, WM.Wo, ob0, lane);
    {
      tm_f4 acc[2] = {{0, 0, 0, 0}, {0, 0, 0, 0}};
      tm_mma<BF>(acc, Fo, ob0, tmp + tk * TM_LDT, 0, lane);
      tm_load(F1a, WM.W1a, ob0, lane);
      tm_load(F1b, WM.W1b, ob0, lane);
#pragma unroll
      for (int t = 0; t < 2; ++t)
#pragma unroll
        for (int i = 0; i < 4; ++i) { const int f = TM_FEAT(ob0 + t, i); xs[tk * TM_LDX + f] += acc[t][i] + W.bo[f]; }
    }
    __syncthreads();
    tm_layernorm(xs, TM_LDX, W.g2, W.b2, false, tid);
    __syncthreads();
    {
      tm_f4 h0[2] = {{0, 0, 0, 0}, {0, 0, 0, 0}}, h1[2] = {{0, 0, 0, 0}, {0, 0, 0, 0}};
      tm_mma<BF>(h0, F1a, ob0, xs + tk * TM_LDX, 0, lane);
// ... 91 lines not shown
```

Measured before the change: 1774.

## Use DPP/permlane wave reductions and optionally fuse cls head into actor decoder

Result: faster. 1804 (median of 4 runs) (+1.7%).

```diff
diff --git a/include/mind_hip.h b/include/mind_hip.h
--- a/include/mind_hip.h
+++ b/include/mind_hip.h
@@ -96,6 +96,8 @@
 int mind_debug_pack_conv_frag(const float *w, int co, int ci, int ksz, uint32_t *out, size_t cap);
 
 int mind_debug_trig(mind_ctx *ctx, const double *x, int n, double *out);
+
+int mind_debug_xlane(mind_ctx *ctx, const float *in, int n_waves, float *out_new, float *out_old);
 
 int mind_debug_set_layers(mind_ctx *ctx, int n);
 int64_t mind_debug_read(mind_ctx *ctx, const char *name, float *host, int64_t max_floats);
diff --git a/mind_amd/_lib.py b/mind_amd/_lib.py
--- a/mind_amd/_lib.py
+++ b/mind_amd/_lib.py
@@ -157,7 +157,7 @@
 EXPORTS = ["mind_ctx_create", "mind_ctx_destroy", "mind_last_error_string", "mind_ctx_synchronize",
            "mind_weights_load", "mind_predict_batch", "mind_last_fusion_stats", "mind_last_actor_stats", "mind_debug_actor_lw_plan", "mind_last_token_stats", "mind_last_token_stage_ms", "mind_debug_token_lw_plan", "mind_set_profiling",
            "mind_ilqr_solve_trees", "mind_ilqr_contingency", "mind_ilqr_solve_fields", "mind_cost_eval", "mind_lane_dist_field", "mind_aime_world", "mind_aime_rebase", "mind_debug_set_layers",
-           "mind_debug_read", "mind_set_pair_precision", "mind_get_pair_precision", "mind_debug_pack_bfrag", "mind_debug_pack_conv_frag", "mind_debug_pair_schedule", "mind_debug_predict_choice", "mind_debug_ilqr_plan", "mind_debug_aime_book", "mind_set_tuning", "mind_last_ilqr_stats", "mind_aime_plan", "mind_last_ilqr_profile", "mind_eval_traj_trees", "mind_last_ilqr_trace", "mind_ilqr_contingency_begin", "mind_ilqr_finish", "mind_fill_tracks", "mind_ilqr_contingency_begin_plan", "mind_debug_trig", "mind_aime_plan_begin", "mind_aime_plan_poll", "mind_aime_plan_finish", "mind_ctx_busy", "mind_ilqr_finish_plan",
+           "mind_debug_read", "mind_set_pair_precision", "mind_get_pair_precision", "mind_debug_pack_bfrag", "mind_debug_pack_conv_frag", "mind_debug_pair_schedule", "mind_debug_predict_choice", "mind_debug_ilqr_plan", "mind_debug_aime_book", "mind_debug_xlane", "mind_set_tuning", "mind_last_ilqr_stats", "mind_aime_plan", "mind_last_ilqr_profile", "mind_eval_traj_trees", "mind_last_ilqr_trace", "mind_ilqr_contingency_begin", "mind_ilqr_finish", "mind_fill_tracks", "mind_ilqr_contingency_begin_plan", "mind_debug_trig", "mind_aime_plan_begin", "mind_aime_plan_poll", "mind_aime_plan_finish", "mind_ctx_busy", "mind_ilqr_finish_plan",
            "mind_set_exchange", "mind_last_exchange_stats",
            "mind_loop_create", "mind_loop_destroy", "mind_loop_reset", "mind_loop_advance", "mind_loop_state", "mind_loop_last_plan", "mind_loop_export",
            "mind_planner_create", "mind_planner_destroy", "mind_planner_reset", "mind_planner_observe", "mind_planner_set_lanes", "mind_planner_set_target_lane",
@@ -236,6 +236,7 @@
     lib.mind_debug_ilqr_plan.argtypes = [C.POINTER(C.c_char_p), C.POINTER(C.c_int), C.c_int, C.c_int, C.c_int, C.c_int, C.POINTER(C.c_int), C.POINTER(C.c_int32),
                                          C.POINTER(C.c_longlong), C.c_int, C.POINTER(C.c_int)]
     lib.mind_debug_aime_book.argtypes = [C.c_int] * 8 + [C.POINTER(C.c_int), C.POINTER(C.c_float)] + [C.c_int] * 4 + [C.POINTER(C.c_longlong), C.c_int, C.c_char_p, C.c_int]
+    lib.mind_debug_xlane.argtypes = [C.c_void_p, C.POINTER(C.c_float), C.c_int, C.POINTER(C.c_float), C.POINTER(C.c_float)]
     lib.mind_debug_trig.argtypes = [C.c_void_p, C.POINTER(C.c_double), C.c_int, C.POINTER(C.c_double)]
     lib.mind_debug_pack_conv_frag.argtypes = [C.POINTER(C.c_float), C.c_int, C.c_int, C.c_int, C.POINTER(C.c_uint32), C.c_size_t]
     lib.mind_debug_set_layers.argtypes = [C.c_void_p, C.c_int]
@@ -271,7 +272,7 @@
 
 PRED_CHOICE_FIELDS = ("header", "n_runs", "np", "actor_form", "actor_arg", "actor_grid", "actor_chunk", "actor_chunks", "actor_launches", "qsplit", "qk_stride",
                       "tiled", "edge_bf16", "edge_pair_bytes", "tok_chunk", "tok_lw", "tok_chunks", "pair_family", "pair_np", "l5_jobs5", "xcd_lanes",
-                      "xcd_lanes5", "dec_actor", "dec_np", "fp32_dec", "split_dec", "want_mw", "mw_blocks", "cls_on_side", "tgt_wait_first")
+                      "xcd_lanes5", "dec_actor", "dec_np", "fp32_dec", "split_dec", "want_mw", "mw_blocks", "cls_on_side", "tgt_wait_first", "cls_blocks")
 PAIR_PREC = ("f32", "bf16x3", "bf16", "bf16x6")
 
 
@@ -288,7 +289,7 @@
     if n == MIND_EINVAL:
         return None
     assert 0 < n <= cap and out[0] == 32 and n == 32 + 6 * out[1], n
-    d = dict(zip(PRED_CHOICE_FIELDS, out[:30]))
+    d = dict(zip(PRED_CHOICE_FIELDS, out[:31]))
     d["runs"] = [tuple(out[32 + 6 * i:38 + 6 * i]) for i in range(out[1])]
     return d
 
diff --git a/mind_amd/csrc/encdec_kernels.hip b/mind_amd/csrc/encdec_kernels.hip
--- a/mind_amd/csrc/encdec_kernels.hip
+++ b/mind_amd/csrc/encdec_kernels.hip
@@ -1,19 +1,11 @@
 #include <hip/hip_runtime.h>
 #include <stdint.h>
 
+#include "xlane.h"
+
 typedef float f32x4 __attribute__((ext_vector_type(4)));
 
 #define NT 256
-
-__device__ __forceinline__ float wave_sum(float v) {
-  v += __shfl_xor(v, 32, 64);
-  v += __shfl_xor(v, 16, 64);
-  v += __shfl_xor(v, 8, 64);
-  v += __shfl_xor(v, 4, 64);
-  v += __shfl_xor(v, 2, 64);
-  v += __shfl_xor(v, 1, 64);
-  return v;
-}
 
 __device__ __forceinline__ float block_sum(float v, float *red) {
   v = wave_sum(v);
@@ -878,12 +870,12 @@
 #define RA 4
 #define DEC_ACTOR_LDS_FLOATS (512 + 1536 + 3072 + 3072 + 3072 + 960 + 6144)
 template <int PART>
-__global__ __launch_bounds__(DT) void k_dec_actor(const float *__restrict__ x ,
-                                                  const int *__restrict__ actor_row ,
-                                                  const int *__restrict__ actor_scene , int n_actors,
-                                                  const float *__restrict__ Cmode ,
-                                                  const float *__restrict__ tgt ,
-                                                  float *__restrict__ reg, float *__restrict__ vel, DecW W, float *__restrict__ h2g) {
+__device__ __forceinline__ void k_dec_actor_body(const float *__restrict__ x ,
+                                                 const int *__restrict__ actor_row ,
+                                                 const int *__restrict__ actor_scene , int n_actors,
+                                                 const float *__restrict__ Cmode ,
+                                                 const float *__restrict__ tgt ,
+                                                 float *__restrict__ reg, float *__restrict__ vel, const DecW &W, float *__restrict__ h2g) {
   extern __shared__ __attribute__((aligned(16))) float dsm[];
   float (*xin)[128] = (float (*)[128])(dsm);
   float (*h1)[384] = (float (*)[384])(dsm + 512);
@@ -972,6 +964,26 @@
     vo[0] = v2[0] / 6.0f; vo[1] = v2[1] / 6.0f;
   }
 }
+template <int PART>
+__global__ __launch_bounds__(DT) void k_dec_actor(const float *__restrict__ x, const int *__restrict__ actor_row, const int *__restrict__ actor_scene,
+                                                  int n_actors, const float *__restrict__ Cmode, const float *__restrict__ tgt,
+                                                  float *__restrict__ reg, float *__restrict__ vel, DecW W, float *__restrict__ h2g) {
+  k_dec_actor_body<PART>(x, actor_row, actor_scene, n_actors, Cmode, tgt, reg, vel, W, h2g);
+}
+__global__ __launch_bounds__(DT) void k_dec_actor_cls(const float *__restrict__ x, const int *__restrict__ actor_row, const int *__restrict__ actor_scene,
+                                                      int n_actors, float *__restrict__ Cmode, const float *__restrict__ tgt,
+                                                      float *__restrict__ reg, float *__restrict__ vel, DecW W, float *__restrict__ h2g,
+                                                      float *__restrict__ cls_out) {
+  const int agrid = (n_actors + RA - 1) / RA;
+  if ((int)blockIdx.x >= agrid) {
+    k_dec_scene_body<false, 2>(nullptr, nullptr, Cmode, cls_out, W, (int)blockIdx.x - agrid, 0, 1, nullptr, nullptr, nullptr);
+    return;
+  }
+  k_dec_actor_body<2>(x, actor_row, actor_scene, n_actors, Cmode, tgt, reg, vel, W, h2g);
+}
 
 extern "C" size_t mind_dec_scene_lds_bytes() { return (size_t)DEC_SCENE_LDS_FLOATS * sizeof(float); }
 extern "C" size_t mind_dec_actor_lds_bytes() { return (size_t)DEC_ACTOR_LDS_FLOATS * sizeof(float); }
+static inline size_t mind_dec_actor_cls_lds_bytes() {
+  return (size_t)(DEC_SCENE_LDS_FLOATS > DEC_ACTOR_LDS_FLOATS ? DEC_SCENE_LDS_FLOATS : DEC_ACTOR_LDS_FLOATS) * sizeof(float);
+}
diff --git a/mind_amd/csrc/fusion_kernels.hip b/mind_amd/csrc/fusion_kernels.hip
--- a/mind_amd/csrc/fusion_kernels.hip
+++ b/mind_amd/csrc/fusion_kernels.hip
@@ -1,5 +1,7 @@
 #include <hip/hip_runtime.h>
 #include <stdint.h>
+
+#include "xlane.h"
 
 typedef float f32x4 __attribute__((ext_vector_type(4)));
 typedef float f32x16 __attribute__((ext_vector_type(16)));
@@ -568,8 +570,7 @@
 }
 
 __device__ __forceinline__ void gsum2(float &a, float &b, float *rd, int kg, int tid) {
-#pragma unroll
-  for (int o = 32; o > 0; o >>= 1) { a += __shfl_xor(a, o, 64); b += __shfl_xor(b, o, 64); }
+  wave_sum2_bperm(a, b);
   const int wv = (tid >> 6) & 1;
   __syncthreads();
   if ((tid & 63) == 0) { rd[(kg * 2 + wv) * 2] = a; rd[(kg * 2 + wv) * 2 + 1] = b; }
diff --git a/mind_amd/csrc/mind_hip.hip b/mind_amd/csrc/mind_hip.hip
--- a/mind_amd/csrc/mind_hip.hip
+++ b/mind_amd/csrc/mind_hip.hip
@@ -297,6 +297,7 @@
   if (const char *te = getenv("MIND_TOK_MERGE")) c->pt.tok_merge = !(te[0] == '0');
   if (const char *te = getenv("MIND_DEC_MW")) c->pt.dec_mw = !(te[0] == '0');
   if (const char *te = getenv("MIND_DEC_CLS_SIDE")) c->pt.dec_cls_side = !(te[0] == '0');
+  if (const char *te = getenv("MIND_DEC_CLS_BLOCKS")) c->pt.dec_cls_blocks = !(te[0] == '0');
   if (const char *te = getenv("MIND_TOK_BF_MIN_N")) c->pt.tok_bf_min_n = atoi(te);
   if (const char *te = getenv("MIND_TOK_LW_MIN_N")) c->pt.tok_lw_min_n = atoi(te);
   if (const char *te = getenv("MIND_TOK_LW_MIN")) c->pt.tok_lw_min = atoi(te);
@@ -323,6 +324,7 @@
   (void)hipFuncSetAttribute((const void *)k_dec_actor<0>, hipFuncAttributeMaxDynamicSharedMemorySize, (int)mind_dec_actor_lds_bytes());
   (void)hipFuncSetAttribute((const void *)k_dec_actor<1>, hipFuncAttributeMaxDynamicSharedMemorySize, (int)mind_dec_actor_lds_bytes());
   (void)hipFuncSetAttribute((const void *)k_dec_actor<2>, hipFuncAttributeMaxDynamicSharedMemorySize, (int)mind_dec_actor_lds_bytes());
+  (void)hipFuncSetAttribute((const void *)k_dec_actor_cls, hipFuncAttributeMaxDynamicSharedMemorySize, (int)mind_dec_actor_cls_lds_bytes());
   *out = c;
   return MIND_OK;
 }
@@ -1423,6 +1425,36 @@
   return MIND_OK;
 }
 
+__global__ __launch_bounds__(256) void k_debug_xlane(const float *__restrict__ in, int n_waves, float *__restrict__ out_new, float *__restrict__ out_old) {
+  const int wave = blockIdx.x * 4 + (threadIdx.x >> 6), lane = threadIdx.x & 63;
+  if (wave >= n_waves) return;
+  const size_t n = (size_t)n_waves * 64, i = (size_t)wave * 64 + lane;
+  const float a = in[i], b = in[(size_t)wave * 64 + (63 - lane)];
+  float a2 = a, b2 = b;
+  wave_sum2_dpp(a2, b2);
+  out_new[i] = wave_sum_dpp(a); out_new[n + i] = row16_sum_dpp(a); out_new[2 * n + i] = a2; out_new[3 * n + i] = b2;
+  a2 = a; b2 = b;
+  wave_sum2_bperm(a2, b2);
+  out_old[i] = wave_sum_bperm(a); out_old[n + i] = row16_sum_bperm(a); out_old[2 * n + i] = a2; out_old[3 * n + i] = b2;
+}
+extern "C" int mind_debug_xlane(mind_ctx *c, const float *in, int n_waves, float *out_new, float *out_old) {
+  if (!c || !in || !out_new || !out_old || n_waves <= 0 || n_waves > (1 << 20)) return MIND_EINVAL;
+  HIPCHK(c, hipSetDevice(c->device));
+  const size_t n = (size_t)n_waves * 64;
+  float *d = nullptr;
+  HIPCHK(c, hipMalloc((void **)&d, n * 9 * sizeof(float)));
+  hipError_t e = hipMemcpy(d, in, n * sizeof(float), hipMemcpyHostToDevice);
+  if (e == hipSuccess) {
+    hipLaunchKernelGGL(k_debug_xlane, dim3((n_waves + 3) / 4), dim3(256), 0, c->stream, d, n_waves, d + n, d + 5 * n);
+    e = hipStreamSynchronize(c->stream);
+  }
+  if (e == hipSuccess) e = hipMemcpy(out_new, d + n, n * 4 * sizeof(float), hipMemcpyDeviceToHost);
+  if (e == hipSuccess) e = hipMemcpy(out_old, d + 5 * n, n * 4 * sizeof(float), hipMemcpyDeviceToHost);
+  (void)hipFree(d);
+  if (e != hipSuccess) return fail(c, MIND_EHIP, "mind_debug_xlane: %s", hipGetErrorString(e));
+  return MIND_OK;
+}
+
 extern "C" int mind_debug_set_layers(mind_ctx *c, int n) {
   if (!c || n < 0 || n > 6) return MIND_EINVAL;
   c->debug_layers = n;
diff --git a/mind_amd/csrc/pred_choice.h b/mind_amd/csrc/pred_choice.h
--- a/mind_amd/csrc/pred_choice.h
+++ b/mind_amd/csrc/pred_choice.h
@@ -19,6 +19,7 @@
   bool dec_overlap = true;
   bool dec_mw = false;
   bool dec_cls_side = false;
+  bool dec_cls_blocks = false;
   bool tgt_side = true;
 };
 
@@ -40,6 +41,7 @@
   else if (is("tok_merge")) t.tok_merge = value != 0;
   else if (is("dec_mw")) t.dec_mw = value != 0;
   else if (is("dec_cls_side")) t.dec_cls_side = value != 0;
+  else if (is("dec_cls_blocks")) t.dec_cls_blocks = value != 0;
   else if (is("tok_bf_min_n")) t.tok_bf_min_n = value;
   else if (is("tok_lw_min_n")) t.tok_lw_min_n = value;
   else if (is("tok_lw_min")) t.tok_lw_min = value;
@@ -80,7 +82,7 @@
   bool l5_jobs5 = false;
   int xcd_lanes = 1, xcd_lanes5 = 1;
   int dec_actor = PRED_DEC_ONE;
-  bool fp32_dec = true, split_dec = false, want_mw = false, cls_side = false;
+  bool fp32_dec = true, split_dec = false, want_mw = false, cls_side = false, cls_blocks = false;
   int mw_blocks = 0;
   bool tgt_wait_first = false;
 };
@@ -146,7 +148,8 @@
   ch.dec_actor = ch.split_dec ? PRED_DEC_SPLIT : ch.fp32_dec ? PRED_DEC_ONE : PRED_DEC_MFMA;
   ch.mw_blocks = ((n_scenes + 7) / 8) * 8 * DEC_MW_G;
   ch.want_mw = t.dec_mw && ch.mw_blocks <= n_cu;
-  ch.cls_side = ch.split_dec && t.dec_cls_side;
+  ch.cls_blocks = ch.split_dec && t.dec_cls_blocks;
+  ch.cls_side = ch.split_dec && t.dec_cls_side && !ch.cls_blocks;
   ch.tgt_wait_first = have_side && !t.tgt_side;
   return ch;
 }
diff --git a/mind_amd/csrc/predict.hip b/mind_amd/csrc/predict.hip
--- a/mind_amd/csrc/predict.hip
+++ b/mind_amd/csrc/predict.hip
@@ -116,7 +116,7 @@
       PRED_CHOICE_HEADER, (long long)ch.tok_runs.size(), ch.np, ch.actor_form, ch.actor_arg, ch.actor_grid, ch.actor_chunk, ch.actor_chunks,
       ch.actor_launches, ch.qsplit, ch.qk_stride, ch.tiled, ch.edge_bf16, pred_edge_pair_bytes(t, pair_prec), ch.tok_chunk, ch.tok_lw,
       ch.last_tok_chunks, ch.pair_family, ch.pair_np, ch.l5_jobs5, ch.xcd_lanes, ch.xcd_lanes5, ch.dec_actor, mfma_dec ? ch.np : 0,
-      ch.fp32_dec, ch.split_dec, ch.want_mw, ch.mw_blocks, ch.cls_side && !ch.want_mw, ch.tgt_wait_first, 0, 0};
+      ch.fp32_dec, ch.split_dec, ch.want_mw, ch.mw_blocks, ch.cls_side && !ch.want_mw, ch.tgt_wait_first, ch.cls_blocks && !ch.want_mw, 0};
   std::vector<long long> rec(head, head + PRED_CHOICE_HEADER);
   for (const PredTokRun &r : ch.tok_runs) rec.insert(rec.end(), {r.t0, r.n, r.kind, r.layerwise, r.small, r.merged});
   for (size_t i = 0; i < rec.size() && (int)i < cap; ++i) out[i] = rec[i];
@@ -437,7 +437,7 @@
                        (const float *)nullptr, (const float *)nullptr, (float *)nullptr, (float *)nullptr, c->decW, (float *)c->dec_h2.p);
     HIPCHK(c, hipEventRecord(c->ev_side, c->side));
   }
-  bool cls_on_side = false;
+  bool cls_on_side = false, cls_in_head = false;
   bool mw = ch.want_mw;
   if (mw) {
     if (c->dec_abort && *(volatile unsigned *)c->dec_abort) return fail(c, MIND_EHIP, "k_dec_scene_mw: a barrier of an earlier launch timed out (launch not resident)");
@@ -457,7 +457,10 @@
   if (mw)
     hipLaunchKernelGGL(k_dec_scene_mw, dim3(ch.mw_blocks), dim3(DT), mind_dec_scene_lds_bytes(), st, x, d_cls_row, (float *)c->cmode.p, out->cls, c->decW, Bn,
                        (float *)c->dec_xbuf.p, (unsigned *)c->dec_bars.p, c->dec_abort);
-  else if (ch.cls_side) {
+  else if (ch.cls_blocks) {
+    hipLaunchKernelGGL(k_dec_scene_c, dim3(Bn), dim3(DT), mind_dec_scene_lds_bytes(), st, x, d_cls_row, (float *)c->cmode.p, c->decW);
+    cls_in_head = true;
+  } else if (ch.cls_side) {
     hipLaunchKernelGGL(k_dec_scene_c, dim3(Bn), dim3(DT), mind_dec_scene_lds_bytes(), st, x, d_cls_row, (float *)c->cmode.p, c->decW);
     HIPCHK(c, hipEventRecord(c->ev_main, st));
     HIPCHK(c, hipStreamWaitEvent(c->side, c->ev_main, 0));
@@ -471,6 +474,11 @@
   switch (ch.dec_actor) {
   case PRED_DEC_SPLIT:
     HIPCHK(c, hipStreamWaitEvent(st, c->ev_side, 0));
+    if (cls_in_head) {
+      hipLaunchKernelGGL(k_dec_actor_cls, dim3(agrid.x + Bn), dim3(DT), mind_dec_actor_cls_lds_bytes(), st, x, d_actor_row, d_actor_scene, A,
+                         (float *)c->cmode.p, tgt_emb, out->reg, out->vel, c->decW, (float *)c->dec_h2.p, out->cls);
+      break;
+    }
     hipLaunchKernelGGL(k_dec_actor<2>, agrid, dim3(DT), mind_dec_actor_lds_bytes(), st, x, d_actor_row, d_actor_scene, A, cmode, tgt_emb, out->reg,
                        out->vel, c->decW, (float *)c->dec_h2.p);
     break;
diff --git a/mind_amd/csrc/token_mfma_kernels.hip b/mind_amd/csrc/token_mfma_kernels.hip
--- a/mind_amd/csrc/token_mfma_kernels.hip
+++ b/mind_amd/csrc/token_mfma_kernels.hip
@@ -78,14 +78,12 @@
   float v[8], s = 0.f;
 #pragma unroll
   for (int k = 0; k < 8; ++k) { v[k] = p[k]; s += v[k]; }
-#pragma unroll
-  for (int o = 8; o > 0; o >>= 1) s += __shfl_xor(s, o, 64);
+  s = row16_sum(s);
   const float mean = s * (1.0f / 128.0f);
   float q = 0.f;
 #pragma unroll
   for (int k = 0; k < 8; ++k) { v[k] -= mean; q += v[k] * v[k]; }
-#pragma unroll
-  for (int o = 8; o > 0; o >>= 1) q += __shfl_xor(q, o, 64);
+  q = row16_sum(q);
   const float inv = 1.0f / sqrtf(q * (1.0f / 128.0f) + 1e-5f);
 #pragma unroll
   for (int k = 0; k < 8; ++k) {
diff --git a/mind_amd/csrc/xlane.h b/mind_amd/csrc/xlane.h
--- /dev/null
+++ b/mind_amd/csrc/xlane.h
@@ -0,0 +1,48 @@
+#pragma once
+#include <hip/hip_runtime.h>
+
+__device__ __forceinline__ float row16_sum_bperm(float v) {
+  v += __shfl_xor(v, 8, 64);
+  v += __shfl_xor(v, 4, 64);
+  v += __shfl_xor(v, 2, 64);
+  v += __shfl_xor(v, 1, 64);
+  return v;
+}
+__device__ __forceinline__ float wave_sum_bperm(float v) {
+  v += __shfl_xor(v, 32, 64);
+  v += __shfl_xor(v, 16, 64);
+  return row16_sum_bperm(v);
+}
+
+__device__ __forceinline__ void wave_sum2_bperm(float &a, float &b) {
+#pragma unroll
+  for (int o = 32; o > 0; o >>= 1) { a += __shfl_xor(a, o, 64); b += __shfl_xor(b, o, 64); }
+}
+
+template <int CTRL>
+__device__ __forceinline__ float xl_dpp(float v) {
+  return __int_as_float(__builtin_amdgcn_update_dpp(0, __float_as_int(v), CTRL, 0xf, 0xf, true));
+}
+__device__ __forceinline__ float row16_sum_dpp(float v) {
+  v += xl_dpp<0x128>(v);
+  v += xl_dpp<0x124>(v);
+  v += xl_dpp<0x4e>(v);
+  v += xl_dpp<0xb1>(v);
+  return v;
+}
+__device__ __forceinline__ float wave_sum_dpp(float v) {
+  const uint32_t u = __float_as_uint(v);
+  const auto h = __builtin_amdgcn_permlane32_swap(u, u, false, false);
+  const uint32_t w = __float_as_uint(__uint_as_float(h[0]) + __uint_as_float(h[1]));
+  const auto q = __builtin_amdgcn_permlane16_swap(w, w, false, false);
+  return row16_sum_dpp(__uint_as_float(q[0]) + __uint_as_float(q[1]));
+}
+__device__ __forceinline__ void wave_sum2_dpp(float &a, float &b) { a = wave_sum_dpp(a); b = wave_sum_dpp(b); }
+
+#ifdef MIND_XLANE_BPERMUTE
+__device__ __forceinline__ float wave_sum(float v) { return wave_sum_bperm(v); }
+__device__ __forceinline__ float row16_sum(float v) { return row16_sum_bperm(v); }
+#else
+__device__ __forceinline__ float wave_sum(float v) { return wave_sum_dpp(v); }
+__device__ __forceinline__ float row16_sum(float v) { return row16_sum_dpp(v); }
+#endif
```
